# poke1024/vectorian

Measured on AMD Instinct MI355X. Metric: sentence-alignments/sec at d=300, |q|=10, |s|<=64; 1/2/4/8 GPU + %HBM roofline, higher is better.
Workload: dtype bf16

## Files before the change

### vectorian_amd/csrc/vk_common.hip.h

```cpp

#ifndef VK_COMMON_HIP_H
#define VK_COMMON_HIP_H

#include <hip/hip_runtime.h>
#include <stdint.h>
#include <stdlib.h>

#include "vk_device.h"

typedef __attribute__((ext_vector_type(8))) short bf16x8;
typedef __attribute__((ext_vector_type(4))) short bf16x4;
typedef __attribute__((ext_vector_type(4))) float f32x4;
typedef __attribute__((ext_vector_type(4))) int i32x4;
typedef __attribute__((ext_vector_type(2))) float f32x2;

#define VK_NEG_INF (-__builtin_inff())
#define VK_RUN 4
#ifdef VK_DBG_NOINLINE
#define VK_DP_INLINE __attribute__((noinline))
#else
#define VK_DP_INLINE __forceinline__
#endif


// ... 510 lines not shown

__device__ __forceinline__ const uint8_t *canon_row_ptr(const uint8_t *__restrict__ tile, int lane) { return tile + (lane & 15) * 16; }
__device__ __forceinline__ const uint8_t *canon_row_ptr_static(const uint8_t *__restrict__ etiles, int tile_bytes, int id) {
	return etiles + (int64_t)(id >> 4) * tile_bytes + (id & 15) * 16;
}

__device__ __forceinline__ float static_cell(float cosine, bool own, bool in_query, const vk_host::sim_ops &ops) {
	if (ops.n > 0 && in_query) cosine = vk_host::sim_ops_apply(cosine, ops);
	return own ? 1.0f : clip01(cosine);
}

__device__ __forceinline__ float static_table_cell(const float *__restrict__ table, int64_t table_stride, int id, int j) {
	return table[(int64_t)(j >> 4) * table_stride + (int64_t)id * 16 + (j & 15)];
}
__device__ __forceinline__ float static_cell(float cosine, bool own, bool in_query, const vk_host::sim_ops &ops, int sim_src,
	const float *__restrict__ table, int64_t table_stride, int id, int j) {
	if (sim_src != VK_SIMSRC_COSINE) return static_table_cell(table, table_stride, id, j);
	return static_cell(cosine, own, in_query, ops);
}

template <int NC>
__device__ __forceinline__ void static_sim_canon(const uint8_t *__restrict__ etiles, int tile_bytes, int id, const uint8_t *__restrict__ qtiles,
	int c0, int d, int prec, const int32_t *__restrict__ q_ids, int len_t, const vk_host::sim_ops &ops, int sim_src,
	const float *__restrict__ table, int64_t table_stride, float (&out)[NC]) {
	if (sim_src != VK_SIMSRC_COSINE) {
#pragma unroll
		for (int c = 0; c < NC; c++) out[c] = static_table_cell(table, table_stride, id, c0 + c);
		return;
	}
	sim_canon<NC>(etiles + (int64_t)(id >> 4) * tile_bytes, id & 15, qtiles + (int64_t)(c0 >> 4) * tile_bytes, c0 & 15, d, prec, out);
#pragma unroll
	for (int c = 0; c < NC; c++) out[c] = static_cell(out[c], q_ids && q_ids[c0 + c] == id, c0 + c < len_t, ops);
}

__device__ __forceinline__ float tag_weighted(float s, float w, int pos_s, int pos_t, float keep, float thr) {
	float wgt = w;
	if (pos_s != pos_t) wgt *= keep;
	const float sc = s * wgt;
	return sc <= thr ? 0.0f : sc;
}


__device__ __forceinline__ unsigned long long static_vocab_shared(int len_s, int len_t, const int32_t *__restrict__ tok,
	const int8_t *__restrict__ tag, const uint32_t *__restrict__ bits, const int32_t *qkey) {
	unsigned long long mask = 0;
	for (int u = 0; u < len_s; u++) {
		const int id = tok[u];
		if (!((bits[id >> 5] >> (id & 31)) & 1u)) continue;
		const int key = id * 256 + (tag[u] & 255);
		for (int j = 0; j < len_t; j++) mask |= qkey[j] == key ? 1ull << j : 0ull;
	}
	return (mask & (mask - 1)) ? mask : 0ull;
}

template <int NL, bool CANON = false, bool RESTORE = false>
__device__ __forceinline__ void static_vocab_fixup(float *__restrict__ S, int stride, int len_s, int len_t,
	const int32_t *__restrict__ tok, const int8_t *__restrict__ tag, const int8_t *__restrict__ pos,
	const float *__restrict__ table, int64_t table_stride, const uint32_t *__restrict__ bits, const int32_t *qkey,
	const float *tw, const int32_t *tpos, float keep, float thr, int l,
	const uint8_t *__restrict__ etiles = nullptr, int tile_bytes = 0, const uint8_t *__restrict__ qtiles = nullptr, int d = 0, int prec = 0,
	const int32_t *__restrict__ q_ids = nullptr, const vk_host::sim_ops &ops = vk_host::sim_ops{}, int sim_src = VK_SIMSRC_COSINE) {
	const unsigned long long mask = static_vocab_shared(len_s, len_t, tok, tag, bits, qkey);
	if (!mask) return;
	for (int u = l; u < len_s; u += NL) {
		const int id = tok[u];
		if (!((bits[id >> 5] >> (id & 31)) & 1u)) continue;
		const int key = id * 256 + (tag[u] & 255);
		int ft = -1;
		for (int j = len_t - 1; j >= 0; j--) ft = qkey[j] == key ? j : ft;
		if (ft < 0) continue;
		for (int j = 0; j < len_t; j++)
			if (((mask >> j) & 1ull) && qkey[j] > key) {
				float raw;
				if constexpr (CANON) {
					float v1[1];
					static_sim_canon<1>(etiles, tile_bytes, id, qtiles, j, d, prec, q_ids, len_t, ops, sim_src, table, table_stride, v1);
					raw = v1[0];
				} else raw = table[(int64_t)(j >> 4) * table_stride + (int64_t)id * 16 + (j & 15)];
				S[u * stride + j] = tag_weighted(raw, tw[RESTORE ? j : ft], pos[u], tpos[j], keep, thr);
			}
	}
}



struct DpArgs {
	int32_t locality;
	int32_t len_t;
	float gs, gt;
	float a_s, a_t;
	float open_s, open_t;
	const float *ws;
	const float *wt;
	const float *wt0;
	int32_t rwmd_symmetric, rwmd_normalize_bow, wmd_bound;
	float wrd_raw_total;
};

struct DecaySteps { float g1, g2, g4, g8; };

__device__ __forceinline__ DecaySteps decay_steps(float g, int v) {
	const float inf = __builtin_inff();
	return {v >= 1 ? g : inf, v >= 2 ? 2.0f * g : inf, v >= 4 ? 4.0f * g : inf, v >= 8 ? 8.0f * g : inf};
}

template <int LT>
__device__ __forceinline__ float decay_scan(float x, const DecaySteps &d) {
	x = fmaxf(x, dpp_zero<0x111>(x) - d.g1);
	if (LT > 2) x = fmaxf(x, dpp_zero<0x112>(x) - d.g2);
	if (LT > 4) x = fmaxf(x, dpp_zero<0x114>(x) - d.g4);
	if (LT > 8) x = fmaxf(x, dpp_zero<0x118>(x) - d.g8);
	return x;
}

template <int LT>
__device__ __forceinline__ float dp_linear(const float *__restrict__ S, int rowbase, int len, int maxlen, int v, const DpArgs &a) {
	const bool is_local = a.locality == VK_DEV_LOCAL;
	const bool is_global = a.locality == VK_DEV_GLOBAL;
	const float floor0 = is_local ? 0.0f : VK_NEG_INF;
	const float gsb = is_global ? a.gs : 0.0f;
	const float gs = a.gs, gt = a.gt;
	const bool last_col = v == a.len_t - 1;
	const float gt_v1 = gt * (float)(v + 1);

	const DecaySteps dt = decay_steps(gt, v);

	float h = is_global ? -gt_v1 : 0.0f;
	float best = 0.0f;
	for (int u = 1; u <= maxlen; u++) {
		const bool act = u <= len;
		const float s = S[(rowbase + (act ? u - 1 : 0)) * LT + v];
		const float bprev = -(gsb * (float)(u - 1));
		const float bcur = -(gsb * (float)u);
		const float diag = dpp_f<DPP_ROW_SHR1>(bprev, h);
		float c = fmaxf(diag + s, floor0);
		c = fmaxf(c, h - gs);
		float hn = decay_scan<LT>(c, dt);
		if (!is_local) hn = fmaxf(hn, bcur - gt_v1);
		h = act ? hn : h;
		if (is_local || last_col) best = fmaxf(best, h);
	}
	float m;
	if (is_local) m = v < a.len_t ? best : 0.0f;
	else if (is_global) m = last_col ? h : VK_NEG_INF;
	else m = v < a.len_t ? fmaxf(h, last_col ? best : 0.0f) : 0.0f;
	m = row_max_to_lane15(m);
	return (is_global) ? m : fmaxf(m, 0.0f);
}

template <int LT>
__device__ VK_DP_INLINE float dp_affine(const float *__restrict__ S, int rowbase, int len, int maxlen, int v, const DpArgs &a) {
	const bool is_local = a.locality == VK_DEV_LOCAL;
	const bool is_global = a.locality == VK_DEV_GLOBAL;
	const float floor0 = is_local ? 0.0f : VK_NEG_INF;
	const float bs = a.gs, bt = a.gt, open_s = a.open_s, open_t = a.open_t;
	const float a_s = a.a_s, a_t = a.a_t;
	const bool last_col = v == a.len_t - 1;

	float h = is_global ? -(a_t + bt * (float)(v + 1)) : 0.0f;
	float e = VK_NEG_INF;
	float best = 0.0f;
	const DecaySteps dt = decay_steps(bt, v);
	for (int u = 1; u <= maxlen; u++) {
		const bool act = u <= len;
		const float s = S[(rowbase + (act ? u - 1 : 0)) * LT + v];
		const float bprev = (is_global && u > 1) ? -(a_s + bs * (float)(u - 1)) : 0.0f;
		const float bcur = is_global ? -(a_s + bs * (float)u) : 0.0f;
		const float diag = dpp_f<DPP_ROW_SHR1>(bprev, h);
		const float en = fmaxf(h - open_s, e - bs);
		float c = fmaxf(fmaxf(diag + s, floor0), en);
		float f = VK_NEG_INF;
		float hc = c;
		if (a_t >= 0.0f) {
			f = decay_scan<LT>(dpp_f<DPP_ROW_SHR1>(bcur, c) - open_t, dt);
			hc = fmaxf(c, f);
		} else {
#pragma unroll
			for (int i = 0; i < LT; i++) {
				const float fl = fmaxf(dpp_f<DPP_ROW_SHR1>(bcur, hc) - open_t, dpp_f<DPP_ROW_SHR1>(VK_NEG_INF, f) - bt);
				f = fl;
				hc = fmaxf(c, f);
			}
		}
		if (act) { h = hc; e = en; }
		if (is_local || last_col) best = fmaxf(best, h);
	}
	float m;
	if (is_local) m = v < a.len_t ? best : 0.0f;
	else if (is_global) m = last_col ? h : VK_NEG_INF;
	else m = v < a.len_t ? fmaxf(h, last_col ? best : 0.0f) : 0.0f;
	m = row_max_to_lane15(m);
	return (is_global) ? m : fmaxf(m, 0.0f);
}

template <int LT>
__device__ __forceinline__ float dp_general(const float *__restrict__ S, float *__restrict__ Hh, int hstride,
	int rowbase, int len, int maxlen, int lane, const DpArgs &a) {

	const int v = lane & 15, sigma = lane >> 4;
	const bool is_local = a.locality == VK_DEV_LOCAL;
	const bool is_global = a.locality == VK_DEV_GLOBAL;
	const float floor0 = is_local ? 0.0f : VK_NEG_INF;
	const bool last_col = v == a.len_t - 1;
	float *hist = Hh + sigma * hstride * 16 + v;

	float wtl[LT];
#pragma unroll
	for (int p = 0; p < LT; p++) wtl[p] = (p <= v) ? a.wt[v + 1 - p] : __builtin_inff();

	float h = is_global ? -a.wt0[v + 1] : 0.0f;
	hist[0] = h;
	float best = 0.0f;
	for (int u = 1; u <= maxlen; u++) {
		const bool act = u <= len;
		const float s = S[(rowbase + (act ? u - 1 : 0)) * LT + v];
		const float bprev = is_global ? -a.ws[u - 1] : 0.0f;
		const float bcur = is_global ? -a.ws[u] : 0.0f;
		const float diag = dpp_f<DPP_ROW_SHR1>(bprev, h);
		float c = fmaxf(diag + s, floor0);
		for (int k = 1; k <= u; k++) c = fmaxf(c, hist[(u - k) * 16] - a.ws[k]);
		c = fmaxf(c, bcur - wtl[0]);
#pragma unroll
		for (int p = 1; p < LT; p++) {
			const float hp = __builtin_bit_cast(float,
				__builtin_amdgcn_ds_bpermute((sigma * 16 + p - 1) * 4, __builtin_bit_cast(int, c)));
			c = fmaxf(c, hp - wtl[p]);
		}
		if (act) { h = c; hist[u * 16] = c; }
		if (is_local || last_col) best = fmaxf(best, h);
	}
	float m;
	if (is_local) m = v < a.len_t ? best : 0.0f;
	else if (is_global) m = last_col ? h : VK_NEG_INF;
	else m = v < a.len_t ? fmaxf(h, last_col ? best : 0.0f) : 0.0f;
	m = row_max_to_lane15(m);
	return (is_global) ? m : fmaxf(m, 0.0f);
}

template <int LT, int MAXLEN, bool FRESH = true>
__device__ __forceinline__ float dp_general_reg(const float *__restrict__ S, int rowbase, int len, int maxlen, int v,
	const DpArgs &a, const float (&wsr)[MAXLEN + 1], const float (&wtr)[LT]) {

	int loc = a.locality, vsel = v;
	if constexpr (FRESH) {
		asm volatile("" : "+v"(loc));
		asm volatile("" : "+v"(vsel));
		loc = __builtin_amdgcn_readfirstlane(loc);
	}
	const bool is_local = loc == VK_DEV_LOCAL;
	const bool is_global = loc == VK_DEV_GLOBAL;
	const float floor0 = is_local ? 0.0f : VK_NEG_INF;
	const bool last_col = v == a.len_t - 1;
	const float wt_border = a.wt[v + 1];
	const float wt_border0 = a.wt0[v + 1];

	float wtv[16];
#pragma unroll
	for (int k = 1; k < LT; k++) wtv[k] = vsel >= k ? wtr[k] : __builtin_inff();

	float hreg[MAXLEN + 1];
	float h = is_global ? -wt_border0 : 0.0f;
	hreg[0] = h;
	float best = 0.0f;
#pragma unroll
	for (int u = 1; u <= MAXLEN; u++) {
		if (u <= maxlen) {
			const bool act = u <= len;
			const float s = S[(rowbase + (act ? u - 1 : 0)) * LT + v];
			const float bprev = is_global ? -wsr[u - 1] : 0.0f;
			const float bcur = is_global ? -wsr[u] : 0.0f;
			const float diag = dpp_f<DPP_ROW_SHR1>(bprev, hreg[u - 1]);
			float c = fmaxf(diag + s, floor0);
#pragma unroll
			for (int k = 1; k <= u; k++) c = fmaxf(c, hreg[u - k] - wsr[k]);
			float hc = fmaxf(c, bcur - wt_border);
			if (LT > 1) hc = fmaxf(hc, dpp_zero<0x111>(c) - wtv[1]);
			if (LT > 2) hc = fmaxf(hc, dpp_zero<0x112>(c) - wtv[2]);
			if (LT > 3) hc = fmaxf(hc, dpp_zero<0x113>(c) - wtv[3]);
			if (LT > 4) hc = fmaxf(hc, dpp_zero<0x114>(c) - wtv[4]);
			if (LT > 5) hc = fmaxf(hc, dpp_zero<0x115>(c) - wtv[5]);
			if (LT > 6) hc = fmaxf(hc, dpp_zero<0x116>(c) - wtv[6]);
			if (LT > 7) hc = fmaxf(hc, dpp_zero<0x117>(c) - wtv[7]);
			if (LT > 8) hc = fmaxf(hc, dpp_zero<0x118>(c) - wtv[8]);
			if (LT > 9) hc = fmaxf(hc, dpp_zero<0x119>(c) - wtv[9]);
			if (LT > 10) hc = fmaxf(hc, dpp_zero<0x11a>(c) - wtv[10]);
			if (LT > 11) hc = fmaxf(hc, dpp_zero<0x11b>(c) - wtv[11]);
			if (LT > 12) hc = fmaxf(hc, dpp_zero<0x11c>(c) - wtv[12]);
			if (LT > 13) hc = fmaxf(hc, dpp_zero<0x11d>(c) - wtv[13]);
			if (LT > 14) hc = fmaxf(hc, dpp_zero<0x11e>(c) - wtv[14]);
			if (LT > 15) hc = fmaxf(hc, dpp_zero<0x11f>(c) - wtv[15]);
			hreg[u] = hc;
			h = act ? hc : h;
			if (is_local || last_col) best = fmaxf(best, h);
		}
	}
	float m;
	if (is_local) m = v < a.len_t ? best : 0.0f;
	else if (is_global) m = last_col ? h : VK_NEG_INF;
	else m = v < a.len_t ? fmaxf(h, last_col ? best : 0.0f) : 0.0f;
	m = row_max_to_lane15(m);
	return (is_global) ? m : fmaxf(m, 0.0f);
}

template <int LT, int MAXLEN, int KT, bool FRESH = true>
__device__ __forceinline__ float dp_general_tail_reg(const float *__restrict__ S, int rowbase, int len, int maxlen, int v,
	const DpArgs &a, const float (&wsr)[KT + 2], const float (&wtr)[LT]) {
	static_assert(KT >= 1 && KT < MAXLEN, "the tail begins inside the table");
	int loc = a.locality, vsel = v;
	if constexpr (FRESH) {
		asm volatile("" : "+v"(loc));
		asm volatile("" : "+v"(vsel));
		loc = __builtin_amdgcn_readfirstlane(loc);
	}
	const bool is_local = loc == VK_DEV_LOCAL;
	const bool is_global = loc == VK_DEV_GLOBAL;
	const float floor0 = is_local ? 0.0f : VK_NEG_INF;
	const bool last_col = v == a.len_t - 1;
	const float wt_border = a.wt[v + 1];
	const float wt_border0 = a.wt0[v + 1];
	const float c_tail = wsr[KT + 1];

	float wtv[16];
#pragma unroll
	for (int k = 1; k < LT; k++) wtv[k] = vsel >= k ? wtr[k] : __builtin_inff();

	float hreg[MAXLEN + 1];
	float h = is_global ? -wt_border0 : 0.0f;
	hreg[0] = h;
	float R = h;
	float best = 0.0f;
#pragma unroll
	for (int u = 1; u <= MAXLEN; u++) {
		if (u <= maxlen) {
			const bool act = u <= len;
			const float s = S[(rowbase + (act ? u - 1 : 0)) * LT + v];
			const float bprev = is_global ? -wsr[u - 1 <= KT ? u - 1 : KT + 1] : 0.0f;
			const float bcur = is_global ? -wsr[u <= KT ? u : KT + 1] : 0.0f;
			const float diag = dpp_f<DPP_ROW_SHR1>(bprev, hreg[u - 1]);
			float c = fmaxf(diag + s, floor0);
#pragma unroll
			for (int k = 1; k <= (u < KT ? u : KT); k++) c = fmaxf(c, hreg[u - k] - wsr[k]);
			if (u > KT) {
				if (u > KT + 1) R = fmaxf(R, hreg[u - KT - 1]);
				c = fmaxf(c, R - c_tail);
			}
			float hc = fmaxf(c, bcur - wt_border);
			if (LT > 1) hc = fmaxf(hc, dpp_zero<0x111>(c) - wtv[1]);
			if (LT > 2) hc = fmaxf(hc, dpp_zero<0x112>(c) - wtv[2]);
			if (LT > 3) hc = fmaxf(hc, dpp_zero<0x113>(c) - wtv[3]);
			if (LT > 4) hc = fmaxf(hc, dpp_zero<0x114>(c) - wtv[4]);
			if (LT > 5) hc = fmaxf(hc, dpp_zero<0x115>(c) - wtv[5]);
			if (LT > 6) hc = fmaxf(hc, dpp_zero<0x116>(c) - wtv[6]);
			if (LT > 7) hc = fmaxf(hc, dpp_zero<0x117>(c) - wtv[7]);
			if (LT > 8) hc = fmaxf(hc, dpp_zero<0x118>(c) - wtv[8]);
			if (LT > 9) hc = fmaxf(hc, dpp_zero<0x119>(c) - wtv[9]);
			if (LT > 10) hc = fmaxf(hc, dpp_zero<0x11a>(c) - wtv[10]);
			if (LT > 11) hc = fmaxf(hc, dpp_zero<0x11b>(c) - wtv[11]);
			if (LT > 12) hc = fmaxf(hc, dpp_zero<0x11c>(c) - wtv[12]);
			if (LT > 13) hc = fmaxf(hc, dpp_zero<0x11d>(c) - wtv[13]);
			if (LT > 14) hc = fmaxf(hc, dpp_zero<0x11e>(c) - wtv[14]);
			if (LT > 15) hc = fmaxf(hc, dpp_zero<0x11f>(c) - wtv[15]);
			hreg[u] = hc;
			h = act ? hc : h;
			if (is_local || last_col) best = fmaxf(best, h);
		}
	}
	float m;
	if (is_local) m = v < a.len_t ? best : 0.0f;
	else if (is_global) m = last_col ? h : VK_NEG_INF;
	else m = v < a.len_t ? fmaxf(h, last_col ? best : 0.0f) : 0.0f;
	m = row_max_to_lane15(m);
	return (is_global) ? m : fmaxf(m, 0.0f);
}

template <int LT>
__device__ __forceinline__ float rwmd_rows(const float *__restrict__ S, int rowbase, int len, int maxlen, int v, const DpArgs &a) {
	const int len_t = a.len_t;
	const bool nbow = a.rwmd_normalize_bow != 0;
	const float w_t = nbow ? 1.0f / (float)len_t : 1.0f;
	const float w_s = nbow ? 1.0f / (float)(len > 0 ? len : 1) : 1.0f;
	const bool col_ok = v < len_t;
	float colmin = 3.402823466e+38F;
	float acc1 = 0.0f;
	for (int u = 1; u <= maxlen; u++) {
		const bool act = u <= len;
		const float s = S[(rowbase + (act ? u - 1 : 0)) * LT + v];
		const float dist = fmaxf(1.0f - s, 0.0f);
		if (act) colmin = fminf(colmin, dist);
		float m = col_ok ? dist : 3.402823466e+38F;
		m = fminf(m, dpp_f<DPP_ROW_SHR1>(m, m));
		m = fminf(m, dpp_f<DPP_ROW_SHR2>(m, m));
		m = fminf(m, dpp_f<DPP_ROW_SHR4>(m, m));
		m = fminf(m, dpp_f<DPP_ROW_SHR8>(m, m));
		if (act) acc1 += w_s * m;
	}
	const float x = col_ok ? w_t * colmin : 0.0f;
	float sum = x;
#pragma unroll
	for (int i = 1; i < LT; i++) {
		const float t = dpp_f<DPP_ROW_SHR1>(0.0f, sum);
		if (v == i) sum = t + x;
	}
	float acc0 = (v == len_t - 1) ? sum : VK_NEG_INF;
	acc0 = row_max_to_lane15(acc0);
	if (!nbow) {
		acc0 = acc0 / (float)len_t;
		acc1 = acc1 / (float)(len > 0 ? len : 1);
	}
	if (a.wmd_bound) {
		float lb;
		if (a.wmd_bound == 1) lb = fmaxf(acc0, acc1);
		else lb = len_t <= len ? acc0 : acc1;
		return fminf(1.0f - lb + 3e-5f, 1.0f);
	}
	float cost = 0.0f;
	if (a.rwmd_symmetric) {
		if (acc0 > cost) cost = acc0;
		if (acc1 > cost) cost = acc1;
	} else {
		cost = acc0;
	}
	const float max_cost = nbow ? 1.0f : (float)len_t;
	return (max_cost - cost) / max_cost;
}

template <int LT>
__device__ __forceinline__ float rwmd_fill_rows(const float *__restrict__ S, const float *__restrict__ smass, int rowbase, int len, int maxlen,
	int lane, const DpArgs &a, float q_mass) {
	const int v = lane & 15, sigma = lane >> 4;
	const int len_t = a.len_t;
	const bool nbow = a.rwmd_normalize_bow != 0;
	const bool col_ok = v < len_t;
	const float cap_s = nbow ? 1.0f / (float)(len > 0 ? len : 1) : 1.0f;
	const float INF = __builtin_inff();

	float rem = col_ok ? q_mass : 0.0f, cost0 = 0.0f, last_d = -1.0f;
	int last_i = -1;
	bool fin = !(rem > 0.0f) || len < 1;
	for (int round = 0; round < maxlen && __any(!fin); round++) {
		float bd = INF;
		int bi = -1;
		for (int u = 1; u <= maxlen; u++) {
			const bool act = u <= len;
			const float dist = fmaxf(1.0f - S[(rowbase + (act ? u - 1 : 0)) * LT + v], 0.0f);
			const bool later = dist > last_d || (dist == last_d && u - 1 > last_i);
			if (act && later && dist < bd) { bd = dist; bi = u - 1; }
		}
		if (!fin) {
			const float cap = (smass && bi >= 0) ? smass[bi] : cap_s;
			if (bi < 0) fin = true;
			else if (rem <= cap) { cost0 += rem * bd; fin = true; }
			else { rem -= cap; cost0 += cap * bd; last_d = bd; last_i = bi; }
		}
	}
	if (rem > 0.0f) cost0 += rem;
	float sum = cost0;
#pragma unroll
	for (int i = 1; i < LT; i++) {
		const float t = dpp_f<DPP_ROW_SHR1>(0.0f, sum);
		if (v == i) sum = t + cost0;
	}
	float acc0 = (v == len_t - 1) ? sum : VK_NEG_INF;
	acc0 = row_max_to_lane15(acc0);

	float acc1 = 0.0f;
	if (a.rwmd_symmetric) {
		for (int u = 1; u <= maxlen; u++) {
			const bool act = u <= len;
			const float dist = fmaxf(1.0f - S[(rowbase + (act ? u - 1 : 0)) * LT + v], 0.0f);
			float r1 = act ? (smass ? smass[u - 1] : cap_s) : 0.0f;
			float cost = 0.0f;
			bool used = !col_ok, done = !(r1 > 0.0f);
			for (int r = 0; r < LT && __any(!done); r++) {
				int key = used ? 0x7fffffff : ((__builtin_bit_cast(int, dist) & ~15) | v);
				key = min(key, __builtin_amdgcn_update_dpp(key, key, 0xB1, 0xf, 0xf, false));
				key = min(key, __builtin_amdgcn_update_dpp(key, key, 0x4E, 0xf, 0xf, false));
				key = min(key, __builtin_amdgcn_update_dpp(key, key, 0x141, 0xf, 0xf, false));
				key = min(key, __builtin_amdgcn_update_dpp(key, key, 0x140, 0xf, 0xf, false));
				const int tl = key & 15;
				const float td = __builtin_bit_cast(float, __builtin_amdgcn_ds_bpermute((sigma * 16 + tl) * 4, __builtin_bit_cast(int, dist)));
				const float tc = __builtin_bit_cast(float, __builtin_amdgcn_ds_bpermute((sigma * 16 + tl) * 4, __builtin_bit_cast(int, q_mass)));
				if (!done) {
					if (key == 0x7fffffff) done = true;
					else if (r1 <= tc) { cost += r1 * td; done = true; }
					else { r1 -= tc; cost += tc * td; }
				}
				if (v == tl) used = true;
			}
			if (r1 > 0.0f) cost += r1;
			acc1 += cost;
		}
	}
	if (!nbow) {
		acc0 = acc0 / (float)len_t;
		acc1 = acc1 / (float)(len > 0 ? len : 1);
	}
	float cost = acc0;
	if (a.rwmd_symmetric) { cost = 0.0f; if (acc0 > cost) cost = acc0; if (acc1 > cost) cost = acc1; }
	const float max_cost = nbow ? 1.0f : (float)len_t;
	return (max_cost - cost) / max_cost;
}

template <int LT>
__device__ __forceinline__ float wrd_bound_rows(const float *__restrict__ S, int rowbase, int len, int maxlen, int v,
	const DpArgs &a, const float *__restrict__ mag, const int32_t *__restrict__ ids, float q_mass) {
	const int len_t = a.len_t;
	const bool col_ok = v < len_t;
	float sum_s = 0.0f;
	float lb1n = 0.0f;
	const float BIG = 3.402823466e+38F;
	float d1 = BIG, d2 = BIG, d3 = BIG, d4 = BIG, c1 = 0.0f, c2 = 0.0f, c3 = 0.0f, c4 = 0.0f;
	const int lane_row = (int)(threadIdx.x & 48);
	for (int base = 0; base < maxlen; base += 64) {
		float mreg[4];
#pragma unroll
		for (int c = 0; c < 4; c++) {
			const int u0 = base + c * 16 + v;
			float mg = 0.0f;
			if (u0 < len) mg = mag ? (ids ? mag[ids[u0]] : mag[u0]) : 1.0f;
			mreg[c] = mg;
		}
#pragma unroll
		for (int c = 0; c < 4; c++) {
			const int u_end = maxlen < base + c * 16 + 16 ? maxlen : base + c * 16 + 16;
			for (int u = base + c * 16 + 1; u <= u_end; u++) {
				const bool act = u <= len;
				const float s = S[(rowbase + (act ? u - 1 : 0)) * LT + v];
				const float dist = fmaxf(1.0f - s, 0.0f);
				int mi = __builtin_bit_cast(int, col_ok ? dist : BIG);
				mi = min(mi, __builtin_amdgcn_update_dpp(mi, mi, DPP_ROW_SHR1, 0xf, 0xf, false));
				mi = min(mi, __builtin_amdgcn_update_dpp(mi, mi, DPP_ROW_SHR2, 0xf, 0xf, false));
				mi = min(mi, __builtin_amdgcn_update_dpp(mi, mi, DPP_ROW_SHR4, 0xf, 0xf, false));
				mi = min(mi, __builtin_amdgcn_update_dpp(mi, mi, DPP_ROW_SHR8, 0xf, 0xf, false));
				const float m = __builtin_bit_cast(float, mi);
				const float mg = __builtin_bit_cast(float, __builtin_amdgcn_ds_bpermute((lane_row | ((u - 1) & 15)) * 4, __builtin_bit_cast(int, mreg[c])));
				sum_s += mg;
				lb1n += mg * m;
				float nd = act ? dist : BIG, nc = mg;
				bool sw;
				sw = nd < d4; d4 = sw ? nd : d4; c4 = sw ? nc : c4;
				sw = d4 < d3; nd = d3; nc = c3; d3 = sw ? d4 : d3; c3 = sw ? c4 : c3; d4 = sw ? nd : d4; c4 = sw ? nc : c4;
				sw = d3 < d2; nd = d2; nc = c2; d2 = sw ? d3 : d2; c2 = sw ? c3 : c2; d3 = sw ? nd : d3; c3 = sw ? nc : c3;
				sw = d2 < d1; nd = d1; nc = c1; d1 = sw ? d2 : d1; c1 = sw ? c2 : c1; d2 = sw ? nd : d2; c2 = sw ? nc : c2;
			}
		}
	}
	const float lb1 = lb1n / sum_s * (1.0f - 2e-6f);
	const float scale = a.wrd_raw_total > 0.0f ? 1.0f : 1.0f / sum_s;
	float rem = col_ok ? q_mass : 0.0f, x = 0.0f, last = 0.0f;
	{
		float amt;
		if (d1 < BIG) { amt = fminf(rem, c1 * scale * (1.0f + 2e-6f)); x += amt * d1; rem -= amt; last = d1; }
		if (d2 < BIG) { amt = fminf(rem, c2 * scale * (1.0f + 2e-6f)); x += amt * d2; rem -= amt; last = d2; }
		if (d3 < BIG) { amt = fminf(rem, c3 * scale * (1.0f + 2e-6f)); x += amt * d3; rem -= amt; last = d3; }
		if (d4 < BIG) { amt = fminf(rem, c4 * scale * (1.0f + 2e-6f)); x += amt * d4; rem -= amt; last = d4; }
		x += fmaxf(rem, 0.0f) * last;
	}
	x += dpp_f<DPP_ROW_SHR1>(0.0f, x);
	x += dpp_f<DPP_ROW_SHR2>(0.0f, x);
	x += dpp_f<DPP_ROW_SHR4>(0.0f, x);
	x += dpp_f<DPP_ROW_SHR8>(0.0f, x);
	float lb;
	if (a.wrd_raw_total > 0.0f) {
		const float sum_t = a.wrd_raw_total;
		lb = (sum_t <= sum_s ? x / sum_t : lb1) * (1.0f - 2e-6f);
		if (!(sum_s > 0.0f)) lb = 0.0f;
	} else lb = fmaxf(x, lb1);
	return fminf(1.0f - lb + 3e-5f, 1.0f);
}

#endif
```

### vectorian_amd/csrc/vk_corpus.cpp

```cpp

#include "vk_internal.h"

std::string &vk_error_slot() {
	static thread_local std::string err;
	return err;
}

std::mutex &vk_ring_mutex() {
	static std::mutex mu;
	return mu;
}

void vk_devblock::release(void *p) {
	if (!p) return;
	{
		std::lock_guard<std::mutex> g(mu);
		ptrs.erase(std::remove(ptrs.begin(), ptrs.end(), p), ptrs.end());
	}
	(void)hipFree(p);
}

vk_devblock::~vk_devblock() {
	(void)hipSetDevice(device);
	for (void *p : ptrs) if (p) (void)hipFree(p);
// ... 314 lines not shown
	c->h_start = std::make_shared<std::vector<int32_t>>(st32);
	c->h_end = std::make_shared<std::vector<int32_t>>(en32);
	c->n_entries = n_entries;
	c->d_wide_order.reset(); c->d_xlong_order.reset(); c->d_apart_order.reset();
	c->n_wide_order = c->n_xlong_order = c->n_apart_order = -1;
	c->lq.order.reset(); c->lq.n_order = -1;
	c->n_long_groups = (int)long_groups.size();
	c->max_len = max_len;
	c->max_short_len = max_short;
	c->max_long_len = max_long;
	c->h_xlong = xlong_entries;
	c->h_apart = apart_entries;
	c->contiguous = contiguous;
	c->overlapping = false;
	for (int64_t s = 1; s < n_sentences && !c->overlapping; s++) c->overlapping = start[s] < end[s - 1] && end[s] > start[s];
	c->uniform_len = 0;
	if (n_sentences > 0 && contiguous) {
		const int64_t l0 = end[0] - start[0];
		bool uni = l0 > 0;
		for (int64_t s = 1; s < n_sentences && uni; s++) uni = (end[s] - start[s]) == l0;
		if (uni) c->uniform_len = (int)l0;
	}
	int mt = 1, mtok = 1, lt = 1, ltok = 1;
	size_t li = 0;
	for (int64_t g = 0; g * 4 < n_entries; g++) {
		const int64_t a = st32[(size_t)(g * 4)], b = en32[(size_t)std::min<int64_t>(g * 4 + 3, n_entries - 1)];
		const int tiles = (int)(((b + 15) >> 4) - (a >> 4));
		if (li < apart_groups.size() && apart_groups[li] == g) {
			li++;
			if (b - a <= VK_MAX_SENT_LEN) {
				lt = std::max(lt, tiles);
				ltok = std::max(ltok, (int)(b - a));
			}
		} else {
			mt = std::max(mt, tiles);
			mtok = std::max(mtok, (int)(b - a));
		}
	}
	int pt = 1, spt = 1;
	li = 0;
	for (int64_t g = 0; g * 2 < n_entries; g++) {
		const int64_t a = st32[(size_t)(g * 2)], b = en32[(size_t)std::min<int64_t>(g * 2 + 1, n_entries - 1)];
		const int tiles = (int)(((b + 15) >> 4) - (a >> 4));
		pt = std::max(pt, tiles);
		while (li < apart_groups.size() && apart_groups[li] < g / 2) li++;
		if (!(li < apart_groups.size() && apart_groups[li] == g / 2)) spt = std::max(spt, tiles);
	}
	c->max_pair_tiles = pt;
	c->max_short_pair_tiles = spt;
	c->max_group_tiles = mt;
	c->max_group_tokens = mtok;
	c->long_group_tiles = lt;
	c->long_group_tokens = ltok;
	c->have_sent = true;
	return VK_OK;
}

int vk_corpus_set_sentences(vk_corpus_t *c, const int64_t *sent_off, int64_t n_sentences) {
	if (!c || !sent_off) return fail(VK_ERR_INVALID, "null argument");
	if (c->finalized) return fail(VK_ERR_STATE, "corpus already finalized");
	if (n_sentences != c->desc.n_sentences) return fail(VK_ERR_INVALID, "sentence count differs from n_sentences");
	if (sent_off[0] != 0) return fail(VK_ERR_INVALID, "sentence spans must start at token 0 (document.h:151-168)");
	if (sent_off[n_sentences] != c->desc.n_tokens) return fail(VK_ERR_INVALID, "sentence spans must cover exactly n_tokens");
	for (int64_t s = 0; s < n_sentences; s++)
		if (sent_off[s + 1] < sent_off[s]) return fail(VK_ERR_INVALID, "sentence offsets must be non-decreasing");
	return set_slices_impl(c, sent_off, sent_off + 1, n_sentences, true);
}

int vk_corpus_set_slices(vk_corpus_t *c, const int64_t *start, const int64_t *end, int64_t n_sentences) {
	if (!c || !start || !end) return fail(VK_ERR_INVALID, "null argument");
	if (c->finalized) return fail(VK_ERR_STATE, "corpus already finalized");
	if (n_sentences != c->desc.n_sentences) return fail(VK_ERR_INVALID, "slice count differs from n_sentences");
	return set_slices_impl(c, start, end, n_sentences, false);
}

static void build_shadow(vk_corpus *c) {
	const int mode = bound_pass_mode();
	if (mode < 0 || (mode == 0 && c->desc.n_sentences < kBoundPassMinSentences)) return;
	if (c->max_len > VK_FAST_SENT_LEN || c->n_entries < 1) return;
	const vk_host::shadow_format f = vk_host::shadow_format_of(c->desc.d, c->nk32, c->tail, c->prec, c->desc.layout, bound_bits_wanted(mode));
	if (f.bits == 0) return;
	const size_t bytes = (size_t)c->n_tiles * f.tile_bytes();
	uint8_t *sh = nullptr;
	if (c->d_counter.reserve(4, &c->device_bytes) || alloc_shared(c, &sh, bytes)) { (void)hipGetLastError(); return; }
	uint32_t stats[4] = {0, 0, 1, 0};
	const bool ran = vk_launch_shadow(c->d_tiles, c->n_tiles, c->rows_total, c->tile_bytes, &f, sh, c->d_counter, c->stream) == hipSuccess
		&& hipMemcpyAsync(stats, c->d_counter, 16, hipMemcpyDeviceToHost, c->stream) == hipSuccess && hipStreamSynchronize(c->stream) == hipSuccess;
	if (!ran || stats[2] != 0) {
		(void)hipGetLastError();
		c->shared->release(sh);
		c->device_bytes -= (int64_t)bytes;
		return;
	}
	c->shadow = sh; c->shadow_format = f;
	memcpy(&c->shadow_n, &stats[0], 4);
	memcpy(&c->shadow_x, &stats[1], 4);
}

int vk_corpus_finalize(vk_corpus_t *c) {
	if (!c) return fail(VK_ERR_INVALID, "null argument");
	if (c->rows_appended != c->rows_total) return fail(VK_ERR_STATE, "not all vectors were appended");
	if (!c->have_sent) return fail(VK_ERR_STATE, "sentence spans were not set");
	if (c->desc.layout == VK_LAYOUT_STATIC && !c->have_ids) return fail(VK_ERR_STATE, "token ids were not set");
	VK_HIP(hipSetDevice(c->device));
	c->d_stage.reset();
	VK_HIP(hipStreamSynchronize(c->stream));
	build_shadow(c);
	c->finalized = true;
	return VK_OK;
}

int vk_corpus_set_sim_ops(vk_corpus_t *c, const int32_t *kinds, const float *args, int32_t n_ops) {
	if (!c || (n_ops > 0 && (!kinds || !args))) return fail(VK_ERR_INVALID, "null argument");
	int bad = -1;
	if (vk_host::sim_ops_check(kinds, args, n_ops, &bad) != VK_OK) {
		if (bad < 0) return fail(VK_ERR_INVALID, "n_ops must be 0 .. VK_MAX_SIM_OPS (8), got " + std::to_string(n_ops));
		return fail(VK_ERR_INVALID, "similarity operator " + std::to_string(bad) + ": unknown kind or an argument that is not finite");
	}
	if (n_ops > 0 && c->desc.layout != VK_LAYOUT_STATIC)
		return fail(VK_ERR_UNSUPPORTED, "similarity operators run over VK_LAYOUT_STATIC only: this corpus is VK_LAYOUT_CONTEXTUAL");
	vk_host::sim_ops ops{};
	ops.n = n_ops;
	for (int i = 0; i < n_ops; i++) { ops.kind[i] = kinds[i]; ops.arg[i] = args[i]; }
	c->sim_ops = ops;
	return VK_OK;
}

int vk_corpus_set_sim_source(vk_corpus_t *c, int32_t kind, float arg) {
	if (!c) return fail(VK_ERR_INVALID, "null argument");
	if (vk_host::sim_src_check(kind, arg) != VK_OK)
		return fail(VK_ERR_INVALID, kind == VK_SIMSRC_PNORM ? "VK_SIMSRC_PNORM: p must be finite and > 0" : "unknown similarity source " + std::to_string(kind));
	if (kind == VK_SIMSRC_COSINE) { c->sim_src = vk_host::sim_src{VK_SIMSRC_COSINE, 0.0f}; return VK_OK; }
	if (c->desc.layout != VK_LAYOUT_STATIC)
		return fail(VK_ERR_UNSUPPORTED, "similarity sources beside the cosine run over VK_LAYOUT_STATIC only: this corpus is VK_LAYOUT_CONTEXTUAL");
	if (c->desc.d > vk_host::kSimSrcMaxD)
		return fail(VK_ERR_UNSUPPORTED, "similarity sources beside the cosine: rows of at most " + std::to_string(vk_host::kSimSrcMaxD) + " features (the table kernel keeps a query tile in LDS)");
	if (!c->raw_rows) {
		if (c->rows_appended > 0 || c->finalized || c->is_view || c->shares_vectors)
			return fail(VK_ERR_STATE, "a similarity source beside the cosine is set before the first vk_corpus_append_vectors: it reads the unmodified rows, and they are gone");
		VK_HIP(hipSetDevice(c->device));
		const int raw_tile_bytes = (c->desc.d + 15) / 16 * 1024;
		const size_t bytes = (size_t)c->n_tiles * (size_t)raw_tile_bytes;
		auto rows = std::make_shared<vk_devbuf<uint8_t>>();
		if (int rc = rows->reserve(bytes, nullptr)) return rc;
		VK_HIP(hipMemsetAsync(*rows, 0, bytes, c->stream));
		VK_HIP(hipStreamSynchronize(c->stream));
		c->raw_rows = rows; c->raw_tile_bytes = raw_tile_bytes;
		c->device_bytes += (int64_t)bytes;
	}
	c->sim_src = vk_host::sim_src{kind, kind == VK_SIMSRC_PNORM ? arg : 0.0f};
	return VK_OK;
}

int vk_corpus_filter(vk_corpus_t *src, uint64_t pos_mask, uint64_t tag_mask, vk_corpus_t **out) {
	if (!src || !out) return fail(VK_ERR_INVALID, "null argument");
	if (!src->finalized) return fail(VK_ERR_STATE, "corpus not finalized");
	if (pos_mask && !src->d_pos) return fail(VK_ERR_STATE, "pos filter needs vk_corpus_set_token_pos");
	if (tag_mask && !src->d_tag) return fail(VK_ERR_STATE, "tag filter needs vk_corpus_set_token_tags");
	VK_HIP(hipSetDevice(src->device));
	hipStream_t st = src->stream;
	const int64_t n = src->desc.n_tokens, ne = src->n_entries, ns = src->desc.n_sentences;
	const bool is_static = src->desc.layout == VK_LAYOUT_STATIC;

	int32_t *keep = nullptr, *new_index = nullptr, *src_of = nullptr, *fs = nullptr, *fe = nullptr;
	void *temp = nullptr;
	vk_corpus *c = nullptr;
	int rc = VK_OK;
	auto body = [&]() -> int {
		VK_HIP(hipMalloc((void **)&keep, ((size_t)n + 1) * 4));
		VK_HIP(hipMalloc((void **)&new_index, ((size_t)n + 1) * 4));
		VK_HIP(hipMalloc((void **)&src_of, ((size_t)n + 1) * 4));
		VK_HIP(hipMalloc((void **)&fs, ((size_t)ne + 1) * 4));
		VK_HIP(hipMalloc((void **)&fe, ((size_t)ne + 1) * 4));
		size_t temp_bytes = 0;
		VK_HIP(vk_launch_filter_scan(nullptr, nullptr, 0, 0, n, keep, new_index, nullptr, &temp_bytes, st));
		VK_HIP(hipMalloc(&temp, temp_bytes ? temp_bytes : 16));
		VK_HIP(vk_launch_filter_scan(src->d_pos, src->d_tag, pos_mask, tag_mask, n, keep, new_index, temp, &temp_bytes, st));
		VK_HIP(vk_launch_filter_maps(keep, new_index, n, src_of, src->d_sent_start, src->d_sent_end, ne, fs, fe, st));
		int32_t n_kept32 = 0;
		std::vector<int32_t> hs((size_t)ne), he((size_t)ne);
		VK_HIP(hipMemcpyAsync(&n_kept32, new_index + n, 4, hipMemcpyDeviceToHost, st));
		if (ne > 0) {
			VK_HIP(hipMemcpyAsync(hs.data(), fs, (size_t)ne * 4, hipMemcpyDeviceToHost, st));
			VK_HIP(hipMemcpyAsync(he.data(), fe, (size_t)ne * 4, hipMemcpyDeviceToHost, st));
		}
		VK_HIP(hipStreamSynchronize(st));
		const int64_t n_kept = n_kept32;

		std::vector<int64_t> start((size_t)ns), end((size_t)ns);
		for (int64_t e = 0; e < ne; e++) {
			const int64_t sent = src->entry_sent.empty() ? e : src->entry_sent[(size_t)e];
			if (sent >= 0 && sent < ns) { start[(size_t)sent] = hs[(size_t)e]; end[(size_t)sent] = he[(size_t)e]; }
		}

		vk_corpus_desc desc = src->desc;
		desc.n_tokens = n_kept;
		if (is_static) {
			c = new vk_corpus();
			c->desc = desc; c->device = src->device;
			c->shared = std::make_shared<vk_devblock>();
			c->shared->device = src->device;
			c->d_pad = src->d_pad; c->nk32 = src->nk32; c->tail = src->tail; c->tile_bytes = src->tile_bytes; c->prec = src->prec;
			c->rows_total = c->rows_appended = src->rows_total; c->n_tiles = src->n_tiles;
			c->d_tiles = src->d_tiles; c->d_mag = src->d_mag; c->shares_vectors = true;
			c->vectors_of = src->shares_vectors ? src->vectors_of : src->shared;
			c->sim_ops = src->sim_ops;
			c->sim_src = src->sim_src; c->raw_rows = src->raw_rows; c->raw_tile_bytes = src->raw_tile_bytes;
			if (hipStreamCreateWithFlags(&c->stream, hipStreamNonBlocking) != hipSuccess) return fail(VK_ERR_HIP, "hipStreamCreate failed");
			for (auto &e : c->ev) if (hipEventCreate(&e) != hipSuccess) return fail(VK_ERR_HIP, "hipEventCreate failed");
			int r;
			if ((r = alloc_shared(c, &c->d_tok_id, (size_t)n_kept + 64))) return r;
			if ((r = reserve_query_workspaces(c))) return r;
			VK_HIP(hipMemsetAsync(c->d_tok_id, 0, ((size_t)n_kept + 64) * 4, st));
			VK_HIP(vk_launch_filter_gather(src->d_tok_id, c->d_tok_id, 4, src_of, n_kept, st));
			c->have_ids = true;
		} else {
			int r = vk_corpus_create(&desc, &c);
			if (r) return r;
			VK_HIP(hipStreamSynchronize(c->stream));
			VK_HIP(vk_launch_filter_rows(src->d_tiles, c->d_tiles, src_of, n_kept, src->tile_bytes, st));
			if (src->d_mag && c->d_mag) VK_HIP(vk_launch_filter_gather(src->d_mag, c->d_mag, 4, src_of, n_kept, st));
			c->rows_appended = c->rows_total;
		}
		for (int which = 0; which < 2; which++) {
			int8_t *from = which ? src->d_tag : src->d_pos;
			int8_t **to = which ? &c->d_tag : &c->d_pos;
			if (!from) continue;
			int r = alloc_shared(c, to, (size_t)n_kept + 64);
			if (r) return r;
			VK_HIP(hipMemsetAsync(*to, 0, (size_t)n_kept + 64, st));
			VK_HIP(vk_launch_filter_gather(from, *to, 1, src_of, n_kept, st));
		}
		VK_HIP(hipStreamSynchronize(st));
		if (is_static) {
			c->h_tok = std::make_shared<std::vector<int32_t>>((size_t)n_kept);
			if (n_kept > 0) VK_HIP(hipMemcpy(c->h_tok->data(), c->d_tok_id, (size_t)n_kept * 4, hipMemcpyDeviceToHost));
		}
		if (c->d_tag) {
			c->h_tag = std::make_shared<std::vector<int8_t>>((size_t)n_kept);
			if (n_kept > 0) VK_HIP(hipMemcpy(c->h_tag->data(), c->d_tag, (size_t)n_kept, hipMemcpyDeviceToHost));
		}
		int r = set_slices_impl(c, start.data(), end.data(), ns, src->contiguous);
		if (r) return r;
		c->finalized = true;
		return VK_OK;
	};
	rc = body();
	for (void *p : {(void *)keep, (void *)new_index, (void *)src_of, (void *)fs, (void *)fe, temp}) if (p) (void)hipFree(p);
	if (rc) { if (c) vk_corpus_free(c); return rc; }
	*out = c;
	return VK_OK;
}

int vk_last_scores(vk_corpus_t *c, float *scores, int64_t n) {
	if (!c || !scores) return fail(VK_ERR_INVALID, "null argument");
	if (!c->have_scores) return fail(VK_ERR_STATE, "no query has run on this corpus");
	if (n != c->desc.n_sentences) return fail(VK_ERR_INVALID, "n differs from n_sentences");
	VK_HIP(hipSetDevice(c->device));
	if (c->bp.pruned) {
		VK_HIP(vk_launch_score(&c->bp.full, c->bp.full_grid, c->bp.full_smem, c->stream));
		VK_HIP(hipStreamSynchronize(c->stream));
		c->bp.pruned = false;
	}
	if (c->entry_sent.empty()) {
		VK_HIP(hipMemcpy(scores, c->d_scores, (size_t)n * 4, hipMemcpyDeviceToHost));
		return VK_OK;
	}
	std::vector<float> rows((size_t)c->n_entries);
	VK_HIP(hipMemcpy(rows.data(), c->d_scores, rows.size() * 4, hipMemcpyDeviceToHost));
	for (int64_t e = 0; e < c->n_entries; e++)
		if (c->entry_sent[(size_t)e] >= 0) scores[c->entry_sent[(size_t)e]] = rows[(size_t)e];
	return VK_OK;
}

int vk_bound_pass_state(vk_corpus_t *c, float *bounds, int64_t n, int64_t *counters) {
	if (!c || !counters) return fail(VK_ERR_INVALID, "null argument");
	const int64_t v[7] = {c->bp.ran, c->bp.round1, c->bp.round2, c->bp.fell_back, c->bp.queries, c->bp.fallbacks, c->bp.survivors};
	memcpy(counters, v, sizeof v);
	if (!bounds) return VK_OK;
	if (!c->bp.ran) return fail(VK_ERR_STATE, "the last query ran no bound pass");
	if (n != c->desc.n_sentences) return fail(VK_ERR_INVALID, "n differs from n_sentences");
	VK_HIP(hipSetDevice(c->device));
	std::vector<float> rows((size_t)c->n_entries);
	VK_HIP(hipMemcpy(rows.data(), c->d_ub, rows.size() * 4, hipMemcpyDeviceToHost));
	for (int64_t e = 0; e < c->n_entries; e++) {
		const int64_t sent = c->entry_sent.empty() ? e : (int64_t)c->entry_sent[(size_t)e];
		if (sent >= 0) bounds[sent] = rows[(size_t)e];
	}
	return VK_OK;
}

int vk_bound_pass_bits(vk_corpus_t *c, int64_t *bits) {
	if (!c || !bits) return fail(VK_ERR_INVALID, "null argument");
	*bits = c->shadow ? c->shadow_format.bits : 0;
	return VK_OK;
}

int vk_bound_pass_tail(vk_corpus_t *c, int32_t *k) {
	if (!c || !k) return fail(VK_ERR_INVALID, "null argument");
	*k = c->bp.ran ? (int32_t)c->bp.tail_k : 0;
	return VK_OK;
}

int vk_bound_pass_shadow(vk_corpus_t *c, int64_t *format, float *nx, int64_t tile0, int64_t n, uint8_t *out) {
	if (!c || !format || !nx) return fail(VK_ERR_INVALID, "null argument");
	const vk_host::shadow_format &sf = c->shadow_format;
	const int64_t f[5] = {sf.bits, sf.steps, sf.live, sf.tile_bytes(), c->n_tiles};
	memset(format, 0, sizeof f);
	nx[0] = nx[1] = 0.0f;
	if (!c->shadow) return out ? fail(VK_ERR_STATE, "the corpus has no shadow") : VK_OK;
	memcpy(format, f, sizeof f);
	nx[0] = c->shadow_n; nx[1] = c->shadow_x;
	if (!out) return VK_OK;
	if (tile0 < 0 || n < 0 || tile0 > c->n_tiles || n > c->n_tiles - tile0) return fail(VK_ERR_INVALID, "tiles out of range");
	VK_HIP(hipSetDevice(c->device));
	VK_HIP(hipStreamSynchronize(c->stream));
	if (n > 0) VK_HIP(hipMemcpy(out, c->shadow + tile0 * sf.tile_bytes(), (size_t)n * sf.tile_bytes(), hipMemcpyDeviceToHost));
	return VK_OK;
}

int vk_batch_state(vk_corpus_t *c, int64_t *state) {
	if (!c || !state) return fail(VK_ERR_INVALID, "null argument");
	memcpy(state, c->batch_state, sizeof c->batch_state);
	return VK_OK;
}

int vk_query_route(vk_corpus_t *c, int64_t *state) {
	if (!c || !state) return fail(VK_ERR_INVALID, "null argument");
	memcpy(state, c->query_route, sizeof c->query_route);
	return VK_OK;
}

int vk_i8_tile_probe(const int8_t *q, const int8_t *x, int32_t *out) {
	if (!q || !x || !out) return fail(VK_ERR_INVALID, "null argument");
	vk_devbuf<uint8_t> buf;
	if (int rc = buf.reserve(4096, nullptr)) return rc;
	uint8_t *d = buf;
	VK_HIP(hipMemcpy(d, q, 1024, hipMemcpyHostToDevice));
	VK_HIP(hipMemcpy(d + 1024, x, 1024, hipMemcpyHostToDevice));
	VK_HIP(vk_launch_i8_probe((const int8_t *)d, (const int8_t *)d + 1024, (int32_t *)(d + 2048), nullptr));
	VK_HIP(hipDeviceSynchronize());
	VK_HIP(hipMemcpy(out, d + 2048, 1024, hipMemcpyDeviceToHost));
	return VK_OK;
}

int vk_i8_bound_tile_probe(const int8_t *q, const int8_t *x, int32_t nk64, int32_t live, int32_t *out) {
	if (!q || !x || !out) return fail(VK_ERR_INVALID, "null argument");
	if ((nk64 != 5 && nk64 != 12) || live < 1 || live > 4) return fail(VK_ERR_INVALID, "nk64 is 5 or 12, live 1 .. 4");
	const size_t tb = (size_t)nk64 * 1024;
	vk_devbuf<uint8_t> buf;
	if (int rc = buf.reserve(2 * tb + 1024, nullptr)) return rc;
	uint8_t *d = buf;
	std::vector<uint8_t> pk(2 * tb);
	for (int side = 0; side < 2; side++)
		for (int i = 0; i < 16; i++)
			vk_host::i8_put_row(pk.data() + side * tb, i, (const uint8_t *)(side ? x : q) + (size_t)i * nk64 * 64, nk64 * 64);
	VK_HIP(hipMemcpy(d, pk.data(), 2 * tb, hipMemcpyHostToDevice));
	VK_HIP(vk_launch_i8_bound_probe(d, d + tb, nk64, live, (int32_t *)(d + 2 * tb), nullptr));
	VK_HIP(hipDeviceSynchronize());
	VK_HIP(hipMemcpy(out, d + 2 * tb, 1024, hipMemcpyDeviceToHost));
	return VK_OK;
}

int vk_fp6_bound_tile_probe(const uint8_t *q, const uint8_t *x, int32_t live6, float *out) {
	if (!q || !x || !out) return fail(VK_ERR_INVALID, "null argument");
	if (live6 < 1 || live6 > 4) return fail(VK_ERR_INVALID, "live6 is 1 .. 4");
	const size_t xoff = VK_DEV_FP6_QTILE_BYTES, ooff = xoff + 5120;
	vk_devbuf<uint8_t> buf;
	if (int rc = buf.reserve(ooff + 1024, nullptr)) return rc;
	uint8_t *d = buf;
	std::vector<uint8_t> pk(ooff, 0);
	for (int i = 0; i < 16; i++) {
		vk_host::fp6_put_row(pk.data(), 4, i, q + (size_t)i * 384, 384);
		vk_host::fp6_put_row(pk.data() + xoff, live6, i, x + (size_t)i * 384, 256 + 32 * live6);
	}
	static_assert(VK_DEV_FP6_QTILE_BYTES % 128 == 0 && VK_DEV_FP6_TILE_BYTES(4) <= 5120, "the probe's buffer");
	VK_HIP(hipMemcpy(d, pk.data(), ooff, hipMemcpyHostToDevice));
	VK_HIP(vk_launch_fp6_bound_probe(d, d + xoff, live6, (float *)(d + ooff), nullptr));
	VK_HIP(hipDeviceSynchronize());
	VK_HIP(hipMemcpy(out, d + ooff, 1024, hipMemcpyDeviceToHost));
	return VK_OK;
}

int vk_fp6c_bound_tile_probe(const uint8_t *q, const uint8_t *x, int32_t d, int32_t fill, float *out) {
	if (!q || !x || !out) return fail(VK_ERR_INVALID, "null argument");
	if (d < 0 || d > 304) return fail(VK_ERR_INVALID, "d is 0 .. 304");
	const size_t xoff = VK_DEV_FP6_QTILE_BYTES, ooff = xoff + 5120;
	vk_devbuf<uint8_t> buf;
	if (int rc = buf.reserve(ooff + 1024, nullptr)) return rc;
	uint8_t *dv = buf;
	std::vector<uint8_t> pk(ooff, 0);
	for (int i = 0; i < 16; i++) {
		vk_host::fp6_put_row(pk.data(), 4, i, q + (size_t)i * 384, 384);
		vk_host::fp6c_put_row(pk.data() + xoff, i, x + (size_t)i * 384, d);
	}
	memset(pk.data() + xoff + VK_DEV_FP6C_TILE_BYTES, fill, 5120 - VK_DEV_FP6C_TILE_BYTES);
	VK_HIP(hipMemcpy(dv, pk.data(), ooff, hipMemcpyHostToDevice));
	VK_HIP(vk_launch_fp6c_bound_probe(dv, dv + xoff, (float *)(dv + ooff), nullptr));
	VK_HIP(hipDeviceSynchronize());
	VK_HIP(hipMemcpy(out, dv + ooff, 1024, hipMemcpyDeviceToHost));
	return VK_OK;
}

int vk_last_timings(const vk_corpus_t *c, vk_timings *t) {
	if (!c || !t) return fail(VK_ERR_INVALID, "null argument");
	*t = c->last;
	return VK_OK;
}

}
```

### vectorian_amd/csrc/vk_device.h

```cpp
#ifndef VK_DEVICE_H
#define VK_DEVICE_H

#include <hip/hip_runtime.h>
#include <stdint.h>

#include "vk_sim_ops_host.h"
#include "vk_sim_src_host.h"

#define VK_DEV_LOCAL 0
#define VK_DEV_GLOBAL 1
#define VK_DEV_SEMIGLOBAL 2

#define VK_DEV_LAYOUT_CONTEXTUAL 0
#define VK_DEV_LAYOUT_STATIC 1

#define VK_DEV_MAX_SENT_LEN 64
#define VK_DEV_MAX_LONG_LEN 512
#define VK_DEV_MAX_QUERY_LEN 16
#define VK_DEV_MAX_WIDE_QUERY_LEN 64
#define VK_DEV_BOUND_CONST_BYTES 256
#define VK_DEV_FP6_STEPS 3
#define VK_DEV_FP6_STEP_BYTES 1536
#define VK_DEV_FP6_QTILE_BYTES (VK_DEV_FP6_STEPS * VK_DEV_FP6_STEP_BYTES)
#define VK_DEV_FP6_TILE_BYTES(live6) ((VK_DEV_FP6_STEPS - 1) * VK_DEV_FP6_STEP_BYTES + 384 * (live6) + 128)
// ... 60 lines not shown

struct VkRwmdBatchParams {
	const uint8_t *tiles;
	int64_t n_tiles;
	int32_t tile_bytes, nk, half;
	const uint8_t *qtiles;
	int32_t n_qtiles, qpt;
	int32_t dense;
	int32_t late_mask;
	const int32_t *q_len;
	const float *q_inv_len;
	const float *q_param;
	int32_t n_queries;
	int32_t n_sent;
	int32_t tiles_per_sent;
	int32_t symmetric, nbow;
	const float *boost;
	float *scores;
	const int32_t *sent_len;
	const int32_t *sent_id;
	int64_t score_stride;
	const int32_t *tok_id;
	const int32_t *sent_start, *sent_end;
	const uint16_t *table;
	int64_t table_row;
	int32_t zero_row;
};

struct VkWrdParams {
	const uint8_t *tiles;
	const int32_t *tok_id;
	const float *table;
	int64_t table_stride;
	const int32_t *sent_start;
	const int32_t *sent_end;
	int32_t layout;
	int32_t nk32, tail, tile_bytes;
	int32_t prec;
	const uint8_t *qtile;
	int32_t nq;
	int32_t len_t;
	const float *mag;
	float qmass[VK_DEV_MAX_WIDE_QUERY_LEN];
	int32_t mass_mode;
	int32_t raw_masses;
	const int8_t *pos_s;
	float tw[VK_DEV_MAX_WIDE_QUERY_LEN];
	int32_t tpos[VK_DEV_MAX_WIDE_QUERY_LEN];
	float tw_keep, tw_threshold;
	float ref_total;
	const float *boost;
	const uint64_t *keys;
	float *raw_out;
	float *val_out;
	float *plan_out;
	float *rows_out;
	int32_t rows_len;
	const int8_t *tag_s;
	const uint32_t *qid_bits;
	int32_t qkey[VK_DEV_MAX_WIDE_QUERY_LEN];
	const int32_t *cand_query;
	int64_t qtile_stride;
	int32_t q_ids_stride;
	const int32_t *cand_len_t;
	const int32_t *group_list;
	int32_t n_list;
	int32_t n_entries;
	float *scores, *raw;
	float wrd_raw_total;
	int32_t wmd_bound;
	int32_t d;
	const int32_t *q_ids;
	uint8_t *scratch;
	int64_t scratch_stride;
	int32_t n_cand;
	vk_host::sim_ops sim_ops;
	int32_t sim_src;
};

struct VkFlowParams {
	const uint8_t *tiles;
	const int32_t *tok_id;
	const float *table;
	const int32_t *sent_start;
	const int32_t *sent_end;
	int32_t layout;
	int32_t nk32, tail, tile_bytes;
	int32_t prec;
	const uint8_t *qtile;
	int32_t len_t;
	int32_t locality;
	int32_t gap_mode;
	int32_t max_len;
	float gs, gt, a_s, a_t, open_s, open_t;
	const float *ws;
	const float *wt;
	const int8_t *pos_s;
	float tw[VK_DEV_MAX_QUERY_LEN];
	int32_t tpos[VK_DEV_MAX_QUERY_LEN];
	float tw_keep, tw_threshold;
	int32_t d;
	const int32_t *q_ids;
	const uint64_t *keys;
	float *raw_out;
	int16_t *mapping;
	float *edge_sim;
	vk_host::sim_ops sim_ops;
	int32_t sim_src;
};

struct VkScoreBatchParams {
	const uint8_t *tiles;
	const int32_t *sent_start;
	const int32_t *sent_end;
	int32_t n_sent;
	int32_t nk32, tail, tile_bytes;
	const uint8_t *qtiles;
	int32_t n_queries;
	int32_t n_strips;
	int32_t len_t[4];
	int32_t locality;
	int32_t gap_mode;
	int32_t rwmd_symmetric, rwmd_normalize_bow;
	float gs, gt, a_s, a_t, open_s, open_t;
	const float *ws;
	const float *wt;
	const float *wt0;
	const float *boost;
	float *scores;
	float *raw;
	int32_t lds_floats_per_wave;
	int32_t s_rows_per_wave;
	int32_t h_rows;
};

struct VkWideParams {
	const uint8_t *tiles;
	const int32_t *tok_id;
	const float *table;
	int64_t table_stride;
	const int32_t *sent_start;
	const int32_t *sent_end;
	int32_t n_sent;
	int32_t layout;
	int32_t nk32, tail, tile_bytes;
	int32_t prec;
	const uint8_t *qtile;
	int32_t nq, len_t;
	int32_t locality;
	int32_t gap_mode;
	int32_t max_len;
	int32_t rwmd_symmetric, rwmd_normalize_bow;
	float gs, gt, a_s, a_t, open_s, open_t;
	const float *ws;
	const float *wt;
	const float *wt0;
	const int8_t *pos_s;
	const int8_t *tag_s;
	const uint32_t *qid_bits;
	int32_t slices_overlap;
	int32_t qkey[VK_DEV_MAX_WIDE_QUERY_LEN];
	float tw[VK_DEV_MAX_WIDE_QUERY_LEN];
	int32_t tpos[VK_DEV_MAX_WIDE_QUERY_LEN];
	float tw_keep, tw_threshold;
	float ref_total;
	const float *mag;
	float qmass[VK_DEV_MAX_WIDE_QUERY_LEN];
	float wrd_raw_total;
	int32_t wmd_bound;
	const float *boost;
	float *scores;
	float *raw;
	int32_t d;
	const int32_t *q_ids;
	const uint64_t *keys;
	float *raw_out;
	int16_t *mapping;
	float *edge_sim;
	uint8_t *scratch;
	int64_t scratch_stride;
	const int32_t *order;
	int32_t n_order;
	const float *dp_rows;
	int32_t dp_rows_len;
	int32_t h_ring;
	int32_t ws_tail;
	vk_host::sim_ops sim_ops;
	int32_t sim_src;
};

struct VkLongqParams {
	const uint8_t *tiles;
	const int32_t *tok_id;
	const float *table;
	int64_t table_stride;
	const int32_t *sent_start;
	const int32_t *sent_end;
	int32_t n_sent;
	int32_t layout;
	int32_t nk32, tail, tile_bytes;
	int32_t prec;
	const uint8_t *qtile;
	int32_t nq, len_t;
	int32_t s_stride;
	int32_t locality;
	int32_t gap_mode;
	float gs, gt, a_s, a_t, open_s, open_t;
	const float *ws;
	const float *wt;
	int32_t wt_tail;
	const int8_t *pos_s;
	const float *tw;
	const int32_t *tpos;
	float tw_keep, tw_threshold;
	float ref_total;
	const float *boost;
	float *scores;
	float *raw;
	int32_t d;
	const int32_t *q_ids;
	const uint64_t *keys;
	int32_t n_keys;
	float *raw_out;
	int16_t *mapping;
	float *edge_sim;
	int32_t out_stride;
	uint8_t *scratch;
	int64_t scratch_stride;
	const int32_t *order;
	int32_t n_order;
	int64_t dm_off, su_off;
	vk_host::sim_ops sim_ops;
	int32_t sim_src;
};

struct VkSimSrcArgs {
	vk_host::sim_src src;
	const uint8_t *raw_tiles;
	int32_t raw_tile_bytes;
	int32_t d;
	const float *q_rows;
	const float *q_abs_sums;
};

#ifdef __cplusplus
namespace vk_host { struct shadow_format; }

extern "C" {
#endif
size_t vk_longq_scratch_bytes(int32_t len_t, int32_t gap_mode, int32_t flow, int32_t tagged);
size_t vk_longq_lds_bytes(int32_t len_t, int32_t max_len, int32_t flow);
int32_t vk_longq_blocks(int32_t len_t, int32_t max_len, int64_t n_sent, int32_t hm_in_lds);
int32_t vk_longq_hm_in_lds(int32_t len_t, int32_t max_len);
int32_t vk_longq_stride(int32_t max_len);
hipError_t vk_launch_longq(const VkLongqParams *p, int32_t flow_k, hipStream_t stream);
hipError_t vk_launch_longq_blocks(const VkLongqParams *p, int32_t max_len, int32_t flow_k, hipStream_t stream);
int32_t vk_longq_blocks_grid(int32_t len_t, int32_t max_len, int32_t gap_mode, int32_t flow_k, int64_t n_items);
hipError_t vk_launch_wide(const VkWideParams *p, int32_t flow_k, hipStream_t stream);
hipError_t vk_launch_doc(const VkWideParams *p, int32_t flow_k, hipStream_t stream);
size_t vk_doc_scratch_bytes(int32_t max_len, int32_t gap_mode);
hipError_t vk_launch_docw(const VkWideParams *p, int32_t flow_k, hipStream_t stream);
size_t vk_docw_scratch_bytes(int32_t max_len, int32_t nq);
hipError_t vk_launch_docg(const VkWideParams *p, int32_t flow_k, hipStream_t stream);
size_t vk_docg_scratch_bytes(int32_t max_len);
hipError_t vk_launch_submatch_bound(const float *raw, const float *boost, int64_t n, float total, float w, float m_star,
	float *scores, hipStream_t stream);
hipError_t vk_launch_mark(const uint64_t *keys, int32_t n, float *scores, hipStream_t stream);
hipError_t vk_launch_select_ge(const float *scores, int64_t n, float theta, float floor_excl, uint64_t *keys_out,
	uint32_t *counter, uint32_t cap, hipStream_t stream);
size_t vk_wide_lds_demand(int32_t max_len, int32_t nq, int32_t gap_mode, int32_t tagged, int32_t flow);
size_t vk_wide_scratch_bytes(int32_t max_len, int32_t nq, int32_t gap_mode, int32_t flow, int32_t ring);
int32_t vk_wide_gs_blocks(int32_t max_len, int32_t nq, int32_t gap_mode, int32_t flow_k, int64_t n_sent, int32_t ring);
int32_t vk_wide_ring_rows(int32_t nq, int32_t gap_mode, int32_t ws_tail);
hipError_t vk_launch_shadow(const uint8_t *tiles, int64_t n_tiles, int64_t rows_total, int32_t tile_bytes, const vk_host::shadow_format *f,
	uint8_t *shadow, uint32_t *stats, hipStream_t stream);
hipError_t vk_launch_i8_bound_probe(const uint8_t *qtile8, const uint8_t *tile8, int32_t nk64, int32_t live, int32_t *out, hipStream_t stream);
hipError_t vk_launch_i8_probe(const int8_t *q, const int8_t *x, int32_t *out, hipStream_t stream);
hipError_t vk_launch_fp6_bound_probe(const uint8_t *qtile6, const uint8_t *tile6, int32_t live6, float *out, hipStream_t stream);
hipError_t vk_launch_fp6c_bound_probe(const uint8_t *qtile6, const uint8_t *tile6c, float *out, hipStream_t stream);
hipError_t vk_launch_select_ge_key(const float *scores, int64_t n, const uint64_t *theta_key, float floor_excl, uint64_t *keys_out,
	uint32_t *counter, uint32_t cap, hipStream_t stream);
hipError_t vk_launch_rekey(const uint64_t *keys, int32_t n, const float *scores, float floor_excl, uint64_t *out, hipStream_t stream);
hipError_t vk_launch_topk_unsorted(const uint64_t *in, int32_t n, int32_t k, uint64_t *out, hipStream_t stream);
hipError_t vk_launch_key_groups(const uint64_t *keys, int32_t n, int32_t *groups, hipStream_t stream);
hipError_t vk_launch_pack(const void *in, int32_t dtype_bf16, int64_t n_rows, int32_t d, int32_t d_pad, int64_t row0,
	uint8_t *tiles, float *mag_out, int32_t normalize, int32_t prec, hipStream_t stream);
size_t vk_score32_lds_bytes(int32_t nk32, int32_t tail, int32_t max_pair_tiles, int32_t len_t, int32_t gap_mode, int32_t waves);
int32_t vk_score32_waves(int32_t nk32, int32_t tail, int32_t max_pair_tiles, int32_t len_t, int32_t gap_mode);
hipError_t vk_launch_score32(const VkWideParams *p, int32_t max_pair_tiles, hipStream_t stream);
hipError_t vk_launch_filter_scan(const int8_t *pos, const int8_t *tag, uint64_t pos_mask, uint64_t tag_mask, int64_t n,
	int32_t *keep, int32_t *new_index, void *temp, size_t *temp_bytes, hipStream_t stream);
hipError_t vk_launch_filter_maps(const int32_t *keep, const int32_t *new_index, int64_t n, int32_t *src_of,
	const int32_t *start, const int32_t *end, int64_t n_entries, int32_t *out_start, int32_t *out_end, hipStream_t stream);
hipError_t vk_launch_filter_rows(const uint8_t *src, uint8_t *dst, const int32_t *src_of, int64_t n_kept, int32_t tile_bytes,
	hipStream_t stream);
hipError_t vk_launch_filter_gather(const void *src, void *dst, int32_t elem_bytes, const int32_t *src_of, int64_t n_kept,
	hipStream_t stream);
hipError_t vk_launch_table(const uint8_t *etiles, const uint8_t *qtile, int32_t n_tiles, int32_t nk32, int32_t tail,
	int32_t tile_bytes, float *table, const int32_t *q_ids, int32_t len_t, int32_t V, int32_t prec, const vk_host::sim_ops *ops,
	const VkSimSrcArgs *src, hipStream_t stream);
hipError_t vk_launch_score(const VkScoreParams *p, int32_t grid, size_t smem_bytes, hipStream_t stream);
int32_t vk_score_m8t_tail_k(void);
int32_t vk_score_m7t_tail_k(void);
hipError_t vk_launch_span(const VkScoreParams *p, hipStream_t stream);
hipError_t vk_launch_score_batch(const VkScoreBatchParams *p, int32_t lt, size_t smem, hipStream_t stream);
hipError_t vk_launch_topk_scores(const float *scores, int64_t n, float min_score, int32_t k, uint64_t *out,
	int32_t *n_blocks_out, hipStream_t stream);
hipError_t vk_launch_topk_keys(const uint64_t *in, int64_t n, int32_t k, uint64_t *out, int32_t *n_blocks_out,
	hipStream_t stream);
hipError_t vk_launch_topk_wave(const float *scores, const uint64_t *keys_in, int64_t n, float min_score, int32_t k,
	int64_t per_wave, uint64_t *out, int64_t *n_waves_out, hipStream_t stream);
hipError_t vk_launch_flow(const VkFlowParams *p, int32_t k, hipStream_t stream);
hipError_t vk_launch_sort_all(const float *scores, int64_t n, float min_score, uint64_t *keys_a, uint64_t *keys_b, void *temp, size_t *temp_bytes,
	uint64_t **sorted_out, hipStream_t stream);
hipError_t vk_launch_rwmd_batch(const VkRwmdBatchParams *p, hipStream_t stream);
hipError_t vk_launch_rwmd_batch32(const VkRwmdBatchParams *p, hipStream_t stream);
hipError_t vk_launch_batch_pack(const uint8_t *src_tiles, uint8_t *dst_tiles, const int32_t *ids, const int32_t *sent_start, const int32_t *sent_end,
	int64_t n, int32_t tps, int32_t tile_bytes, hipStream_t stream);
int vk_rwmd_batch_supported(int32_t nk, int32_t half);
hipError_t vk_launch_table_batch(const uint8_t *etiles, int64_t n_vtiles, int32_t tile_bytes, int32_t nk16, const uint8_t *qtiles, int32_t n_qtiles,
	uint16_t *table, int32_t V, const vk_host::sim_ops *ops, const uint32_t *live, hipStream_t stream);
hipError_t vk_launch_table_batch_fix(uint16_t *table, const int64_t *offsets, int32_t n, hipStream_t stream);
hipError_t vk_launch_rwmd_static32(const VkRwmdBatchParams *p, int32_t w64, hipStream_t stream);
hipError_t vk_launch_topk_wave_batch(const float *scores, const uint64_t *keys_in, int64_t n, float min_score, int32_t k,
	int64_t per_wave, int32_t n_queries, int64_t in_stride, int64_t out_stride, uint64_t *out, int64_t *n_waves_out, hipStream_t stream);
hipError_t vk_launch_wrd_exact(const VkWrdParams *p, int32_t n_cand, float *scores_to_mark, hipStream_t stream);
hipError_t vk_launch_rows(const VkWrdParams *p, int32_t n_cand, hipStream_t stream);
hipError_t vk_launch_canon_rows(const VkWrdParams *p, int32_t n_cand, int32_t max_tiles, hipStream_t stream);
hipError_t vk_launch_wrd_exact_long(const VkWrdParams *p, int32_t n_cand, hipStream_t stream);
int vk_wrd_long_blocks(void);
size_t vk_wrd_long_scratch_bytes(void);
hipError_t vk_launch_long_rwmd_fill(const VkWideParams *p, const int32_t *group_list, int32_t n_list, int32_t n_entries, hipStream_t stream);
hipError_t vk_launch_long_bound(const VkWrdParams *p, hipStream_t stream);
#ifdef __cplusplus
}
#endif

#endif
```

### vectorian_amd/csrc/vk_internal.h

```cpp
#ifndef VK_INTERNAL_H
#define VK_INTERNAL_H

#include "../../include/vectorian_hip.h"
#include "vk_device.h"
#include "vk_devbuf.h"
#include "vk_guard.h"
#include "vk_result_host.h"
#include "vk_bound_host.h"
#include "vk_route_host.h"
#include "vk_sim_ops_host.h"

#include <algorithm>
#include <atomic>
#include <cmath>
#include <cstdio>
#include <cstring>
#include <memory>
#include <mutex>
#include <string>
#include <vector>

std::string &vk_error_slot();

namespace {

int fail(int code, const std::string &msg) {
	vk_error_slot() = msg;
	return code;
}

#define VK_HIP(call) \
	do { \
		hipError_t e_ = (call); \
		if (e_ != hipSuccess) { \
			char buf_[512]; \
			snprintf(buf_, sizeof buf_, "%s failed: %s (%s:%d)", #call, hipGetErrorString(e_), __FILE__, __LINE__); \
			return fail(VK_ERR_HIP, buf_); \
		} \
	} while (0)

uint16_t f32_to_bf16(float x) {
	uint32_t u;
	memcpy(&u, &x, 4);
	if ((u & 0x7fffffffu) > 0x7f800000u) return (uint16_t)((u >> 16) | 0x0040u);
	u += 0x7fffu + ((u >> 16) & 1u);
	return (uint16_t)(u >> 16);
}

float bf16_to_f32(uint16_t b) {
	uint32_t u = ((uint32_t)b) << 16;
	float f;
	memcpy(&f, &u, 4);
	return f;
}

using vk_host::gap_cost;

constexpr int kTopkChunk = 2048;
constexpr int kGapTable = 640;
constexpr int64_t kStageBytes = 64ll << 20;
constexpr int64_t kBoundPassMinSentences = 1000000;
constexpr int64_t kBoundRound2Floor = 1024;
inline int bound_pass_mode() {
	const char *e = getenv("VK_BOUND_PASS");
	return !e ? 0 : !strcmp(e, "off") ? -1 : !strcmp(e, "force") ? 1 : 0;
}
inline int bound_bits_wanted(int mode) {
	const char *e = getenv("VK_BOUND_BITS");
	if (e && !strcmp(e, "6c")) return vk_host::bits6_compact;
	if (e && !strcmp(e, "6")) return 6;
	if (e && !strcmp(e, "8")) return 8;
	return mode > 0 ? 8 : vk_host::bits6_compact;
}
inline bool bound_tail_wanted(int mode) { return vk_host::bound_tail_choice(getenv("VK_BOUND_TAIL"), mode); }

}

struct vk_devblock {
	int device = 0;
	std::mutex mu;
	std::vector<void *> ptrs;
	void add(void *p) { std::lock_guard<std::mutex> g(mu); ptrs.push_back(p); }
	void release(void *p);
	~vk_devblock();
};

std::mutex &vk_ring_mutex();

struct vk_corpus_shape {
	vk_corpus_desc desc{};
	int device = 0;
	int d_pad = 0, nk32 = 0, tail = 0, tile_bytes = 0;
	int prec = 0;
	int64_t rows_total = 0, rows_appended = 0, n_tiles = 0;
	uint8_t *d_tiles = nullptr;
	float *d_mag = nullptr;
	int32_t *d_tok_id = nullptr;
	int8_t *d_pos = nullptr;
	int8_t *d_tag = nullptr;
	int32_t *d_sent_start = nullptr, *d_sent_end = nullptr;
	std::shared_ptr<std::vector<int32_t>> h_start, h_end, h_tok;
	std::shared_ptr<std::vector<int8_t>> h_tag;
	bool contiguous = false;
	bool overlapping = false;
	bool have_ids = false, have_sent = false;
	int max_len = 0, max_group_tiles = 0, max_group_tokens = 0;
	int max_pair_tiles = 0;
	int max_short_pair_tiles = 0;
	int64_t n_entries = 0;
	std::vector<int32_t> entry_sent;
	int32_t *d_long_groups = nullptr;
	int n_long_groups = 0, max_short_len = 0, long_group_tiles = 0, long_group_tokens = 0;
	int max_long_len = 0;
	std::shared_ptr<std::vector<int32_t>> h_apart;
	std::shared_ptr<std::vector<int32_t>> h_xlong;
	int uniform_len = 0;
	bool shares_vectors = false;
	std::shared_ptr<vk_devblock> shared, vectors_of;
	const uint8_t *shadow = nullptr;
	vk_host::shadow_format shadow_format;
	float shadow_n = 0.0f, shadow_x = 0.0f;
	vk_host::sim_ops sim_ops{};
	vk_host::sim_src sim_src{};
	std::shared_ptr<vk_devbuf<uint8_t>> raw_rows;
	int raw_tile_bytes = 0;
};

enum vk_batch_state_index {
	VK_BS_ROUTE,
	VK_BS_QB_MAX, VK_BS_LT, VK_BS_GAP_MODE,
	VK_BS_STAT, VK_BS_STAT_UNIFORM32, VK_BS_UNIFORM16, VK_BS_B32, VK_BS_R32, VK_BS_GRAN,
	VK_BS_WIDE32, VK_BS_DENSE, VK_BS_QPT, VK_BS_N_QTILES, VK_BS_UNIFORM_LEN, VK_BS_LATE_MASK,
	VK_BS_COUNT
};

enum vk_query_route_index {
	VK_QR_PLAN, VK_QR_GAP_MODE, VK_QR_WIDE_GAP_MODE, VK_QR_SCORE32_GAP_MODE, VK_QR_WAVE_TILES,
	VK_QR_PASS_SHORT, VK_QR_PASS_MID, VK_QR_PASS_XLONG, VK_QR_LIST, VK_QR_RING_ROWS, VK_QR_FLOW, VK_QR_OSTRIDE, VK_QR_RAW, VK_QR_SPAN_SKIP_RAW,
	VK_QR_COUNT
};

struct vk_corpus : vk_corpus_shape {
	hipStream_t stream = nullptr;
	bool finalized = false;
	std::vector<int32_t> sent_entry;
	int64_t device_bytes = 0;
	vk_devbuf<uint8_t> d_bq; vk_devbuf<int32_t> d_bqlen; vk_devbuf<float> d_bscores; vk_devbuf<uint64_t> d_bkeys[2];
	vk_devbuf<float> d_braw;
	vk_devbuf<uint8_t> d_stage;
	vk_devbuf<uint8_t> d_qtile;
	vk_devbuf<float> d_ws, d_wt;
	vk_devbuf<int32_t> d_qids;
	vk_devbuf<float> d_table;
	vk_devbuf<float> d_qraw;
	vk_devbuf<float> d_scores, d_raw, d_boost;
	vk_devbuf<uint64_t> d_keys[2];
	vk_devbuf<float> d_out_raw, d_out_sim;
	vk_devbuf<int16_t> d_out_map;
	vk_devbuf<float> d_wrd_raw, d_wrd_val;
	vk_devbuf<uint32_t> d_counter;
	vk_devbuf<float> d_rows_out, d_plan_out;
	vk_devbuf<uint8_t> d_bqt; vk_devbuf<uint64_t> d_bcand; vk_devbuf<int32_t> d_bcandq; vk_devbuf<float> d_brows;
	vk_devbuf<float, true> h_brows;
	vk_devbuf<uint32_t> d_qbits;
	vk_devbuf<uint8_t> d_wrdl_scratch;
	vk_devbuf<uint8_t> d_wide_scratch;
	vk_devbuf<int32_t> d_apart_order; int32_t n_apart_order = -1;
	vk_devbuf<int32_t> d_xlong_order; int32_t n_xlong_order = -1;
	vk_devbuf<int32_t> d_wide_order; int32_t n_wide_order = -1;
	int rows_w = 0;
	struct batch_bucket { vk_devbuf<uint8_t> tiles; vk_devbuf<int32_t> len, id; int64_t n = 0; };
	batch_bucket bl[4];
	bool bl_built = false;
	int64_t bl_empty = 0;
	vk_devbuf<uint8_t> d_qtile8; vk_devbuf<float> d_ub; vk_devbuf<int32_t> d_bound_groups; vk_devbuf<uint64_t> d_bound_keys;
	struct bound_state {
		bool pruned = false;
		VkScoreParams full{}; int full_grid = 0; size_t full_smem = 0;
		int64_t ran = 0, round1 = 0, round2 = 0, fell_back = 0;
		int64_t tail_k = 0;
		int64_t queries = 0, fallbacks = 0, survivors = 0;
		vk_host::bound_backoff backoff;
	} bp;
	vk_devbuf<int32_t> d_sb_id[2]; int64_t sb_n[2] = {0, 0}; bool sb_built = false; int64_t sb_empty = 0;
	vk_devbuf<uint16_t> d_btable;
	vk_devbuf<int64_t> d_bfix;
	vk_devbuf<uint32_t> d_blive;
	vk_devbuf<int32_t> d_bqids;
	vk_devbuf<uint64_t> d_sort[2]; vk_devbuf<uint8_t> d_sort_temp;
	int64_t batch_state[VK_BS_COUNT] = {};
	int64_t query_route[VK_QR_COUNT] = {};
	hipEvent_t ev[7] = {nullptr, nullptr, nullptr, nullptr, nullptr, nullptr, nullptr};
	vk_timings last{};
	bool have_scores = false;
	bool is_view = false;
	struct longq_bufs {
		vk_devbuf<uint8_t> qt;
		vk_devbuf<float> fl;
		vk_devbuf<int32_t> il;
		vk_devbuf<float> table;
		vk_devbuf<uint8_t> scratch, fscratch;
		vk_devbuf<uint8_t> bscratch;
		vk_devbuf<int32_t> order; int32_t n_order = -1;
		vk_devbuf<float> raw, sim;
		vk_devbuf<int16_t> map;
	} lq;
	vk_corpus *peer = nullptr;
	std::atomic<bool> ev2_recorded{false};
};

namespace {

template <typename T> int alloc_shared(vk_corpus *c, T **p, size_t n) {
	VK_HIP(hipMalloc((void **)p, n ? n * sizeof(T) : 16));
	c->device_bytes += (int64_t)(n * sizeof(T));
	c->shared->add((void *)*p);
	return VK_OK;
}

}

int vk_wait_peer_turn(vk_corpus *c, hipStream_t st);
int vk_validate_query(const vk_corpus *c, const vk_query_desc *q, const vk_topk_out *out);
int vk_longq_query(vk_corpus *c, const vk_query_desc *q, vk_topk_out *out, vk_host_keep &keep);
void vk_pack_query(const vk_corpus *c, const vk_query_desc *q, std::vector<uint8_t> &tile, float *mags, std::vector<uint8_t> *bound_tile = nullptr);

namespace {

template <typename P> void corpus_fields(P &p, const vk_corpus *c) {
	p.tiles = c->d_tiles; p.sent_start = c->d_sent_start; p.sent_end = c->d_sent_end;
	p.nk32 = c->nk32; p.tail = c->tail; p.tile_bytes = c->tile_bytes;
}
template <typename P> auto sim_ops_field(P &p, const vk_corpus *c, int) -> decltype((void)p.sim_ops) { p.sim_ops = c->sim_ops; p.sim_src = c->sim_src.kind; }
template <typename P> void sim_ops_field(P &, const vk_corpus *, long) {}
template <typename P> void corpus_fields_ids(P &p, const vk_corpus *c) {
	corpus_fields(p, c);
	sim_ops_field(p, c, 0);
	p.tok_id = c->d_tok_id; p.prec = c->prec;
	p.layout = c->desc.layout == VK_LAYOUT_STATIC ? VK_DEV_LAYOUT_STATIC : VK_DEV_LAYOUT_CONTEXTUAL;
}
template <typename P, typename G> void gap_fields(P &p, const G &g) {
	p.gs = g.gs; p.gt = g.gt; p.a_s = g.a_s; p.a_t = g.a_t; p.open_s = g.open_s; p.open_t = g.open_t;
}

inline float ref_total_of(const vk_query_desc *q) {
	if (!q->tag_weights) return (float)q->len_t;
	float total = 0.0f;
	for (int j = 0; j < q->len_t; j++) total += q->tag_weights[j];
	return total;
}
template <typename P> void tag_weight_fields(P &p, const vk_corpus *c, const vk_query_desc *q, int cols) {
	const bool tagged = q->tag_weights != nullptr;
	for (int j = 0; j < cols; j++) {
		p.tw[j] = (tagged && j < q->len_t) ? q->tag_weights[j] : 0.0f;
		p.tpos[j] = (tagged && j < q->len_t) ? (int32_t)q->q_pos[j] : -1;
	}
	p.ref_total = ref_total_of(q);
	if (!tagged) return;
	p.pos_s = c->d_pos; p.tw_keep = 1.0f - q->pos_mismatch_penalty; p.tw_threshold = q->similarity_threshold;
}

void state_timings(vk_corpus *c, bool flow, int scored = 2) {
	float ms = 0;
	vk_timings t{};
	if (hipEventElapsedTime(&ms, c->ev[0], c->ev[5]) == hipSuccess) t.prepare_ms = ms;
	if (hipEventElapsedTime(&ms, c->ev[5], c->ev[1]) == hipSuccess) t.queue_ms = ms;
	if (hipEventElapsedTime(&ms, c->ev[1], c->ev[scored]) == hipSuccess) t.score_ms = ms;
	if (hipEventElapsedTime(&ms, c->ev[scored], c->ev[3]) == hipSuccess) t.topk_ms = ms;
	if (flow && hipEventElapsedTime(&ms, c->ev[3], c->ev[4]) == hipSuccess) t.flow_ms = ms;
	if (hipEventElapsedTime(&ms, c->ev[0], c->ev[4]) == hipSuccess) t.total_ms = ms - t.queue_ms;
	c->last = t;
}

int select_waves(vk_corpus *c, float floor, int kk, hipStream_t st, const uint64_t **d_sel) {
	int64_t nw = 0;
	int cur = 0;
	VK_HIP(vk_launch_topk_wave(c->d_scores, nullptr, c->n_entries, floor, kk, 4096, c->d_keys[0], &nw, st));
	while (nw > 1) {
		const int64_t nkeys = nw * kk;
		const int64_t per_wave = nkeys <= 16384 ? nkeys : 4096;
		VK_HIP(vk_launch_topk_wave(nullptr, c->d_keys[cur], nkeys, 0.0f, kk, per_wave, c->d_keys[1 - cur], &nw, st));
		cur = 1 - cur;
	}
	*d_sel = c->d_keys[cur];
	return VK_OK;
}
int select_blocks(vk_corpus *c, float floor, int kk, hipStream_t st, const uint64_t **d_sel, const float *scores = nullptr) {
	int nb = 0, cur = 0;
	VK_HIP(vk_launch_topk_scores(scores ? scores : (const float *)c->d_scores, c->n_entries, floor, kk, c->d_keys[0], &nb, st));
	while (nb > 1) {
		VK_HIP(vk_launch_topk_keys(c->d_keys[cur], (int64_t)nb * kk, kk, c->d_keys[1 - cur], &nb, st));
		cur = 1 - cur;
	}
	*d_sel = c->d_keys[cur];
	return VK_OK;
}

int upload_boost(vk_corpus *c, const float *boost, vk_host_keep &keep, hipStream_t st, bool *nonneg = nullptr) {
	const int64_t n = c->n_entries;
	if (nonneg) {
		float least = 0.0f;
		bool nan = false;
		for (int64_t s = 0; s < c->desc.n_sentences; s++) { least = std::min(least, boost[s]); nan = nan || boost[s] != boost[s]; }
		*nonneg = !(least < 0.0f) && !nan;
	}
	if (int rc = c->d_boost.reserve((size_t)n + 8, &c->device_bytes)) return rc;
	if (!c->entry_sent.empty()) {
		std::vector<float> &rows = keep.vec<float>((size_t)n);
		for (int64_t e = 0; e < n; e++) rows[(size_t)e] = c->entry_sent[(size_t)e] >= 0 ? boost[c->entry_sent[(size_t)e]] : 1.0f;
		boost = rows.data();
	}
	VK_HIP(hipMemcpyAsync(c->d_boost, boost, (size_t)n * 4, hipMemcpyHostToDevice, st));
	return VK_OK;
}

constexpr size_t vk_source_tile_floats(int d) { return 16 * (size_t)d + 16; }
int upload_source_query(vk_corpus *c, const vk_query_desc *q, vk_host_keep &keep, hipStream_t st) {
	const int d = c->desc.d, nq = (q->len_t + 15) / 16;
	const size_t per = vk_source_tile_floats(d);
	std::vector<float> &rows = keep.vec<float>(per * (size_t)nq);
	std::fill(rows.begin(), rows.end(), 0.0f);
	for (int i = 0; i < q->len_t; i++) {
		float *row = rows.data() + (size_t)(i >> 4) * per + (size_t)(i & 15) * d;
		for (int k = 0; k < d; k++)
			row[k] = q->q_dtype == VK_F32 ? ((const float *)q->q_vectors)[(size_t)i * d + k] : bf16_to_f32(((const uint16_t *)q->q_vectors)[(size_t)i * d + k]);
		rows[(size_t)(i >> 4) * per + 16 * (size_t)d + (size_t)(i & 15)] = vk_host::sim_src_abs_sum(row, d);
	}
	if (int rc = c->d_qraw.reserve(rows.size(), &c->device_bytes)) return rc;
	VK_HIP(hipMemcpyAsync(c->d_qraw, rows.data(), rows.size() * 4, hipMemcpyHostToDevice, st));
	return VK_OK;
}
VkSimSrcArgs source_table_args(const vk_corpus *c, int t) {
	VkSimSrcArgs a{};
	a.src = c->sim_src; a.raw_tiles = c->raw_rows ? (const uint8_t *)*c->raw_rows : nullptr; a.raw_tile_bytes = c->raw_tile_bytes; a.d = c->desc.d;
	a.q_rows = (const float *)c->d_qraw + (size_t)t * vk_source_tile_floats(c->desc.d);
	a.q_abs_sums = a.q_rows + 16 * (size_t)c->desc.d;
	return a;
}

int64_t row_of_sentence(vk_corpus *c, int64_t s) {
	if (c->entry_sent.empty()) return s;
	if (c->sent_entry.empty()) {
		c->sent_entry.assign((size_t)c->desc.n_sentences, -1);
		for (int64_t e = 0; e < c->n_entries; e++) if (c->entry_sent[(size_t)e] >= 0) c->sent_entry[(size_t)c->entry_sent[(size_t)e]] = (int32_t)e;
	}
	return (int64_t)c->sent_entry[(size_t)s];
}

int launch_wrd_exact_both(vk_corpus *c, VkWrdParams &w, int count, float *scores_to_mark, bool long_too, hipStream_t st) {
	VK_HIP(vk_launch_wrd_exact(&w, count, scores_to_mark, st));
	if (long_too) {
		if (w.nq > 1)
			if (int rc = c->d_wrdl_scratch.reserve((size_t)vk_wrd_long_blocks() * vk_wrd_long_scratch_bytes(), &c->device_bytes)) return rc;
		w.scratch = c->d_wrdl_scratch; w.scratch_stride = (int64_t)vk_wrd_long_scratch_bytes();
		VK_HIP(vk_launch_wrd_exact_long(&w, count, st));
	}
	return VK_OK;
}

}

#endif
```

### vectorian_amd/csrc/vk_query.cpp

```cpp

#include "vk_internal.h"
#include "vk_guard.h"
#include "vk_transport_host.h"

static constexpr int kCanonMargin = 8;
static const vk_host::route_fits kRouteFits{vk_score32_waves, vk_wide_ring_rows, vk_wide_lds_demand};
static bool exact_transport(const vk_query_desc *q) { return vk_host::exact_transport(q->algorithm, q->wmd_full != 0); }
static vk_host::route_facts route_facts_of(const vk_corpus *c, const vk_query_desc *q, const vk_topk_out *out) {
	vk_host::route_facts f;
	f.layout = c->desc.layout; f.prec = c->prec; f.nk32 = c->nk32; f.tail = c->tail;
	f.max_len = c->max_len; f.max_short_len = c->max_short_len; f.n_long_groups = c->n_long_groups;
	f.has_apart = c->h_apart && !c->h_apart->empty(); f.has_xlong = c->h_xlong && !c->h_xlong->empty();
	f.max_pair_tiles = c->max_pair_tiles; f.max_short_pair_tiles = c->max_short_pair_tiles; f.uniform_len = c->uniform_len;
	f.has_pos = c->d_pos != nullptr; f.has_tags = c->d_tag != nullptr; f.n_sentences = c->desc.n_sentences;
	f.algorithm = q->algorithm; f.wmd_full = q->wmd_full != 0; f.rwmd_injective = q->rwmd_injective != 0; f.len_t = q->len_t;
	if (q->algorithm == VK_ALG_ALIGN) {
		f.gaps = vk_host::classify_gaps(q->gap_s, q->gap_t);
		if (f.gaps.gap_mode == 2 && q->gap_s.kind >= VK_GAP_LINEAR && q->gap_s.kind <= VK_GAP_TABLE) f.ws_tail = vk_host::ws_tail_of(q->gap_s, c->max_len);
	}
	f.submatch = q->submatch_weight > 0.0f; f.tagged = q->tag_weights != nullptr; f.has_q_tags = q->q_tags != nullptr; f.has_q_ids = q->q_token_ids != nullptr;
	f.only = q->only_slices != nullptr; f.want_flow = q->want_flow != 0; f.locality = q->locality;
	f.sim_rows = out->sim_rows != nullptr; f.raw_score = out->raw_score != nullptr; f.boost = q->boost != nullptr;
	const int k = q->max_matches;
	const bool restated = (q->want_flow && q->algorithm == VK_ALG_ALIGN) || (q->algorithm == VK_ALG_RWMD && !q->wmd_full && q->want_flow && out->sim_rows);
	f.kk = f.only ? q->n_only : (int)std::min<int64_t>(!restated ? k : (k <= VK_MAX_MATCHES ? std::min(k + kCanonMargin, VK_MAX_MATCHES) : k + kCanonMargin), std::max<int64_t>(c->n_entries, 1));
	return f;
}

int vk_validate_query(const vk_corpus *c, const vk_query_desc *q, const vk_topk_out *out) {
	if (!c || !q || !out) return fail(VK_ERR_INVALID, "null argument");
	if (!c->finalized) return fail(VK_ERR_STATE, "corpus not finalized");
	if (q->len_t < 1) return fail(VK_ERR_INVALID, "empty query");
	if (q->len_t > VK_MAX_LONG_QUERY_LEN) return fail(VK_ERR_UNSUPPORTED, "query longer than VK_MAX_LONG_QUERY_LEN (512) tokens");
	if (q->len_t > VK_MAX_QUERY_LEN) {
		if (q->algorithm != VK_ALG_ALIGN) return fail(VK_ERR_UNSUPPORTED, "queries of more than VK_MAX_QUERY_LEN (64) tokens: alignments only (the transports keep a lane per query token)");
		if (c->max_len > VK_MAX_SENT_LEN) return fail(VK_ERR_UNSUPPORTED, "queries of more than 64 tokens over a corpus that holds a slice of more than VK_MAX_SENT_LEN (512) tokens: the state of such a slice does not fit a workgroup's LDS");
		if (q->submatch_weight != 0.0f) return fail(VK_ERR_UNSUPPORTED, "queries of more than 64 tokens with a submatch weight");
		if (out->sim_rows) return fail(VK_ERR_UNSUPPORTED, "queries of more than 64 tokens: similarity rows of the winners are not returned");
		if (q->max_matches > VK_MAX_MATCHES) return fail(VK_ERR_UNSUPPORTED, "queries of more than 64 tokens: max_matches <= VK_MAX_MATCHES");
	}
	if (q->len_t <= VK_MAX_QUERY_LEN) {
		const vk_host::query_route r = vk_host::route_query(route_facts_of(c, q, out), vk_host::route_switches{}, kRouteFits);
		if (r.status != VK_OK && !r.fits32) return fail(r.status, r.message);
	}
	if (c->max_len > VK_MAX_SENT_LEN && q->algorithm != VK_ALG_ALIGN) {
		const bool relaxed_11 = q->algorithm == VK_ALG_RWMD && !q->wmd_full && q->rwmd_injective;
		if (!relaxed_11)
			return fail(VK_ERR_UNSUPPORTED, "slices of more than VK_MAX_SENT_LEN (512) tokens: alignments and the relaxed 1:1 word mover's distance only (the 1:n form and the exact transports keep a slice's bag of words in LDS)");
		if (c->desc.layout == VK_LAYOUT_STATIC && q->tag_weights && q->q_tags && q->q_token_ids && c->d_tag)
			return fail(VK_ERR_UNSUPPORTED, "slices of more than VK_MAX_SENT_LEN (512) tokens: tag-weighted vocabulary transports keyed by (id, tag) rewrite cells of a slice's rows in LDS");
	}
	if (!q->q_vectors) return fail(VK_ERR_INVALID, "q_vectors is null");
	if (q->q_dtype != VK_F32 && q->q_dtype != VK_BF16) return fail(VK_ERR_INVALID, "bad q_dtype");
	if (q->max_matches < 1 || q->max_matches > VK_MAX_MATCHES_SORTED) return fail(VK_ERR_INVALID, "max_matches out of range");
	if (q->max_matches > VK_MAX_MATCHES && !q->only_slices && (q->algorithm != VK_ALG_ALIGN || q->submatch_weight != 0.0f || out->sim_rows))
		return fail(VK_ERR_UNSUPPORTED, "max_matches beyond VK_MAX_MATCHES (1024): alignments without a submatch weight only");
	if (out->capacity < q->max_matches) return fail(VK_ERR_INVALID, "output capacity smaller than max_matches");
	if (!out->score || !out->sentence) return fail(VK_ERR_INVALID, "output arrays missing");
	if (out->sim_rows && out->rows_per_winner != 0 && (out->rows_per_winner < VK_FAST_SENT_LEN || out->rows_per_winner % 64 != 0 || out->rows_per_winner > VK_MAX_DOC_LEN + 1))
		return fail(VK_ERR_INVALID, "rows_per_winner must be 0 or a multiple of 64 (64 .. VK_MAX_DOC_LEN + 1)");
	if (!(q->submatch_weight >= 0.0f)) return fail(VK_ERR_INVALID, "submatch_weight must be >= 0 (pow of a zero base, metric/alignment.h:97-99)");
	if (q->only_slices) {
		if (q->n_only < 1 || q->n_only > VK_MAX_MATCHES || q->n_only > out->capacity) return fail(VK_ERR_INVALID, "only_slices: n_only out of range (1 .. min(VK_MAX_MATCHES, capacity))");
		const bool relaxed = q->algorithm == VK_ALG_RWMD && !q->wmd_full && out->sim_rows != nullptr;
		const bool exact = exact_transport(q);
		if (!(q->algorithm == VK_ALG_ALIGN || relaxed || exact) || !q->want_flow || (q->submatch_weight != 0.0f && q->algorithm != VK_ALG_ALIGN))
			return fail(VK_ERR_UNSUPPORTED, "only_slices states alignments, relaxed WMD with sim_rows, or exact transports, with want_flow (and submatch_weight = 0 for the transports)");
		for (int i = 0; i < q->n_only; i++)
			if (q->only_slices[i] < 0 || q->only_slices[i] >= c->desc.n_sentences) return fail(VK_ERR_INVALID, "only_slices: slice index out of range");
	}
	if (q->bidirectional) return fail(VK_ERR_UNSUPPORTED, "bidirectional is not implemented (unused upstream, query.cpp:81-83)");
	int rc = VK_OK;
	const auto tag_weights = [&]() -> int {
		if (!q->tag_weights) return VK_OK;
		if (!q->q_pos) return fail(VK_ERR_INVALID, "tag-weighted query without q_pos");
		if (!c->d_pos) return fail(VK_ERR_STATE, "tag-weighted query needs vk_corpus_set_token_pos");
		if (q->similarity_threshold < 0.0f) return fail(VK_ERR_INVALID, "similarity_threshold must be >= 0 (slice/static.h:209)");
		return VK_OK;
	};
	const auto flow_arrays = [&]() -> int {
		return (q->want_flow && (!out->mapping || !out->edge_sim)) ? fail(VK_ERR_INVALID, "want_flow needs mapping and edge_sim arrays") : VK_OK;
	};
	if (q->algorithm == VK_ALG_ALIGN) {
		if (q->locality < VK_LOCAL || q->locality > VK_SEMIGLOBAL) return fail(VK_ERR_INVALID, "bad locality");
		for (const vk_gap *g : {&q->gap_s, &q->gap_t}) {
			if (g->kind < VK_GAP_LINEAR || g->kind > VK_GAP_TABLE) return fail(VK_ERR_INVALID, "bad gap kind");
			if (g->kind == VK_GAP_TABLE && (!g->table || g->n_table < 1)) return fail(VK_ERR_INVALID, "gap table missing");
		}
		if (q->gap_s.kind == VK_GAP_TABLE && q->gap_s.n_table <= c->max_len) return fail(VK_ERR_INVALID, "gap_s table shorter than the longest sentence");
		if (q->gap_t.kind == VK_GAP_TABLE && q->gap_t.n_table <= q->len_t) return fail(VK_ERR_INVALID, "gap_t table shorter than the query");
		if ((rc = flow_arrays())) return rc;
		if ((rc = tag_weights())) return rc;
	} else if (q->algorithm == VK_ALG_RWMD) {
		if ((rc = tag_weights())) return rc;
		if (q->tag_weights) {
			if (q->q_tags && c->desc.layout == VK_LAYOUT_STATIC) {
				if (c->desc.vocab_size > (1 << 23)) return fail(VK_ERR_UNSUPPORTED, "tag-weighted transport with q_tags over the static layout: vocabularies of more than 2^23 entries overflow the (id, tag) keys");
				for (int j = 0; j < q->len_t; j++) {
					if (q->q_tags[j] < 0) return fail(VK_ERR_INVALID, "q_tags: tag codes must be 0 .. 127");
					if (q->q_token_ids && q->q_token_ids[j] >= (1 << 23)) return fail(VK_ERR_UNSUPPORTED, "q_token_ids: ids of 2^23 and more overflow the (id, tag) keys");
				}
			}
			if (q->q_tags && !q->rwmd_injective && !q->wmd_full && c->desc.layout == VK_LAYOUT_STATIC && !c->d_tag)
				return fail(VK_ERR_STATE, "tag-weighted 1:n RWMD over the static layout with q_tags needs vk_corpus_set_token_tags (its vocabulary is keyed by (token, tag), bow.h:150-176)");
		}
		if (q->rwmd_symmetric && !q->rwmd_normalize_bow)
			return fail(VK_ERR_INVALID, "cannot run symmetric mode WMD with bow (needs nbow)");
		if (q->wmd_full) {
			if (q->rwmd_injective) return fail(VK_ERR_INVALID, "non-relaxed WMD with injective mapping is not supported");
			if (q->rwmd_symmetric) return fail(VK_ERR_INVALID, "non-relaxed WMD with symmetric computation is not supported");
		}
		if ((rc = flow_arrays())) return rc;
	} else if (q->algorithm == VK_ALG_WRD) {
		if ((rc = tag_weights())) return rc;
		if (!c->d_mag) return fail(VK_ERR_STATE, "VK_ALG_WRD needs a corpus created with keep_magnitudes = 1");
		if ((rc = flow_arrays())) return rc;
	} else {
		return fail(VK_ERR_INVALID, "bad algorithm");
	}
	return VK_OK;
}

void vk_pack_query(const vk_corpus *c, const vk_query_desc *q, std::vector<uint8_t> &tile, float *mags, std::vector<uint8_t> *bound_tile) {
	const int d = c->desc.d;
	tile.assign((size_t)c->tile_bytes * (size_t)((q->len_t + 15) / 16), 0);
	std::vector<float> row((size_t)d);
	for (int i = 0; i < q->len_t; i++) {
		for (int k = 0; k < d; k++)
			row[(size_t)k] = q->q_dtype == VK_F32 ? ((const float *)q->q_vectors)[(size_t)i * d + k]
			                                       : bf16_to_f32(((const uint16_t *)q->q_vectors)[(size_t)i * d + k]);
		double acc = 0.0;
		for (int k = 0; k < d; k++) acc += (double)row[(size_t)k] * (double)row[(size_t)k];
		float m = (float)std::sqrt(acc);
		if (m != m) m = 0.0f;
		mags[i] = m;
		if (q->q_normalize) {
			for (int k = 0; k < d; k++) {
				float v = row[(size_t)k] / m;
				if (v != v) v = 0.0f;
				row[(size_t)k] = v;
			}
		}
		for (int k = 0; k < d; k++) {
			if (c->prec) {
				const size_t off = (size_t)(i >> 4) * c->tile_bytes + (size_t)(k >> 4) * 1024 + (size_t)((k & 3) * 16 + (i & 15)) * 16 + (size_t)((k & 15) >> 2) * 4;
				memcpy(&tile[off], &row[(size_t)k], 4);
				continue;
			}
			const uint16_t b = f32_to_bf16(row[(size_t)k]);
			const int t = k >> 5, g = (k & 31) >> 3, j = k & 7;
			const size_t off = (size_t)(i >> 4) * c->tile_bytes + (size_t)t * 1024 + (size_t)(g * 16 + (i & 15)) * 16 + (size_t)j * 2;
			memcpy(&tile[off], &b, 2);
		}
	}
	if (!bound_tile || !c->shadow || c->prec || q->len_t > VK_FAST_QUERY_LEN) return;
	std::vector<float> stored((size_t)q->len_t * d);
	for (int i = 0; i < q->len_t; i++)
		for (int k = 0; k < d; k++) {
			uint16_t b;
			memcpy(&b, &tile[(size_t)(k >> 5) * 1024 + (size_t)(((k & 31) >> 3) * 16 + i) * 16 + (size_t)(k & 7) * 2], 2);
			stored[(size_t)i * d + k] = bf16_to_f32(b);
		}
	vk_host::pack_bound_query(c->shadow_format, stored.data(), q->len_t, c->shadow_n, c->shadow_x, *bound_tile);
}

static int score_bounded(vk_corpus *c, const VkScoreParams &p, int grid, size_t smem, size_t smem_bound, size_t smem_list, int kk, float sel_floor,
	const vk_gap &gap_s, bool tail, vk_host_keep &keep, hipStream_t st, const uint64_t **d_sel) {
	*d_sel = nullptr;
	const int64_t n = c->n_entries;
	vk_corpus::bound_state &b = c->bp;
	const int64_t most = std::max<int64_t>(n / 16, kBoundRound2Floor);
	const int M = kk <= 32 ? 64 : kk <= 256 ? 512 : VK_MAX_MATCHES;
	int rc;
	if ((rc = c->d_ub.reserve((size_t)n + 8, &c->device_bytes))) return rc;
	if ((rc = c->d_bound_groups.reserve((size_t)std::max<int64_t>(most, kTopkChunk), &c->device_bytes))) return rc;
	if ((rc = c->d_bound_keys.reserve((size_t)2 * kTopkChunk, &c->device_bytes))) return rc;
	if ((rc = c->d_counter.reserve(4, &c->device_bytes))) return rc;
	VkScoreParams pb = p;
	const vk_host::shadow_format &sf = c->shadow_format;
	pb.tiles = c->shadow; pb.nk32 = sf.steps; pb.tail = 0; pb.tile_bytes = sf.tile_bytes(); pb.bound_bits = sf.bits; pb.bound_live = sf.live; pb.bound_compact = sf.compact;
	pb.q_mode3 = 0; pb.q_lds = 0; pb.qtile = c->d_qtile8; pb.scores = c->d_ub; pb.raw = nullptr;
	b.tail_k = 0;
	if (tail && (p.gap_mode == 3 || p.gap_mode == 6)) {
		const int rows = p.gap_mode == 3 ? 32 : 64, K = sf.bits == 6 ? vk_score_m8t_tail_k() : vk_score_m7t_tail_k();
		float w[65];
		for (int j = 0; j <= rows; j++) w[j] = gap_cost(gap_s, j);
		pb.gap_mode = p.gap_mode == 3 ? 8 : 9;
		pb.bound_tail_cost = vk_host::bound_tail_cost(w, K, rows);
		b.tail_k = K;
	}
	VK_HIP(vk_launch_score(&pb, grid, smem_bound, st));
	VK_HIP(hipEventRecord(c->ev[2], st));
	c->ev2_recorded = true;
	b.ran = 1; b.queries++;
	VK_HIP(hipMemsetD32Async(static_cast<hipDeviceptr_t>(c->d_scores), (int)0xff800000u, (size_t)n, st));
	if (p.raw) VK_HIP(hipMemsetD32Async(reinterpret_cast<hipDeviceptr_t>(p.raw), (int)0xff800000u, (size_t)n, st));
	VkScoreParams pl = p;
	pl.group_list = c->d_bound_groups;
	const uint64_t *d_first = nullptr;
	if ((rc = select_blocks(c, sel_floor, M, st, &d_first, c->d_ub))) return rc;
	VK_HIP(vk_launch_key_groups(d_first, M, c->d_bound_groups, st));
	pl.n_list = M;
	VK_HIP(vk_launch_score(&pl, M, smem_list, st));
	uint64_t *d_exact = c->d_bound_keys, *d_best = c->d_bound_keys + kTopkChunk;
	VK_HIP(vk_launch_rekey(d_first, M, c->d_scores, sel_floor, d_exact, st));
	VK_HIP(vk_launch_topk_unsorted(d_exact, M, kk, d_best, st));
	VK_HIP(vk_launch_select_ge_key(c->d_ub, n, d_best + (kk - 1), sel_floor, c->d_keys[0], c->d_counter, (uint32_t)most, st));
	uint32_t &count = *keep.array<uint32_t>(1);
	VK_HIP(hipMemcpyAsync(&count, c->d_counter, 4, hipMemcpyDeviceToHost, st));
	VK_HIP(hipStreamSynchronize(st));
	b.round1 = M;
	bool fell = false;
	if ((int64_t)count > most) {
		fell = true;
		VK_HIP(vk_launch_score(&p, grid, smem, st));
	} else if (count > 0) {
		VK_HIP(vk_launch_key_groups(c->d_keys[0], (int32_t)count, c->d_bound_groups, st));
		pl.n_list = (int32_t)count;
		VK_HIP(vk_launch_score(&pl, (int32_t)count, smem_list, st));
	}
	if (!fell && count <= (uint32_t)kTopkChunk) {
		VK_HIP(vk_launch_rekey(c->d_keys[0], (int32_t)count, c->d_scores, sel_floor, d_exact, st));
		VK_HIP(vk_launch_topk_unsorted(d_exact, (int32_t)count, kk, d_best, st));
		*d_sel = d_best;
	}
	b.round2 = count;
	if (!fell) b.survivors += count;
	b.fell_back = fell ? 1 : 0;
	if (fell) b.fallbacks++;
	if (bound_pass_mode() == 0) b.backoff.record(fell);
	b.pruned = !fell;
	b.full = p; b.full_grid = grid; b.full_smem = smem;
	return VK_OK;
}

static int query_body(vk_corpus_t *c, const vk_query_desc *q, vk_topk_out *out, vk_host_keep &keep) {
	int rc = VK_OK;
	VK_HIP(hipSetDevice(c->device));
	c->bp.pruned = false; c->bp.ran = c->bp.round1 = c->bp.round2 = c->bp.fell_back = c->bp.tail_k = 0;
	for (int64_t &x : c->query_route) x = -1;
	if (q->len_t > VK_MAX_QUERY_LEN) return vk_longq_query(c, q, out, keep);
	hipStream_t st = c->stream;
	const int64_t n = c->n_entries;
	const int k = q->max_matches;
	const bool only = q->only_slices != nullptr;
	out->n_out = 0;
	c->have_scores = false;
	if (n == 0) return VK_OK;
	const vk_host::route_switches sw = vk_host::read_route_switches();
	vk_host::route_facts facts = route_facts_of(c, q, out);
	const int bound_mode = bound_pass_mode();
	facts.bound_pass = c->shadow && bound_mode >= 0 && (bound_mode > 0 || c->desc.n_sentences >= kBoundPassMinSentences) && vk_host::bound_pass_takes(facts) &&
		(bound_mode != 0 || c->bp.backoff.take());
	const vk_host::query_route r = vk_host::route_query(facts, sw, kRouteFits);
	if (r.status != VK_OK) return fail(r.status, r.message);
	const int64_t route_state[VK_QR_COUNT] = {r.plan, r.gap_mode, r.wide_gap_mode, r.score32_gap_mode, r.wave_tiles, r.pass[vk_host::CLASS_SHORT],
		r.pass[vk_host::CLASS_MID], r.pass[vk_host::CLASS_XLONG], r.list, r.ring_rows, r.flow, r.ostride, r.raw, r.span_skip_raw};
	memcpy(c->query_route, route_state, sizeof route_state);
	const bool wide_query = q->len_t > VK_FAST_QUERY_LEN;
	const bool xlong = c->max_len > VK_MAX_SENT_LEN;
	const bool wide_family = r.flow != vk_host::FLOW_NARROW;
	auto sentence_of = [c](int64_t row) { return c->entry_sent.empty() ? row : (int64_t)c->entry_sent[(size_t)row]; };
	const bool is_static_l = c->desc.layout == VK_LAYOUT_STATIC;
	auto fill_transport = [&](VkWrdParams &w) {
		corpus_fields_ids(w, c);
		w.table = c->d_table; w.table_stride = (int64_t)c->n_tiles * 16 * 16;
		w.qtile = c->d_qtile; w.nq = (q->len_t + 15) / 16; w.len_t = q->len_t; w.mag = c->d_mag;
		w.d = c->desc.d; w.q_ids = is_static_l ? (int32_t *)c->d_qids : nullptr;
		tag_weight_fields(w, c, q, VK_MAX_QUERY_LEN);
		if (q->tag_weights) {
			if (is_static_l && q->algorithm == VK_ALG_RWMD && q->q_tags && q->q_token_ids && c->d_tag && c->d_qbits) {
				w.tag_s = c->d_tag; w.qid_bits = c->d_qbits;
				for (int j = 0; j < VK_MAX_QUERY_LEN; j++)
					w.qkey[j] = (j < q->len_t && q->q_token_ids[j] >= 0 && q->q_token_ids[j] < c->desc.vocab_size) ? q->q_token_ids[j] * 256 + ((int32_t)q->q_tags[j] & 255) : -1;
			}
		}
	};
	auto transport_flows = [&](const std::vector<int64_t> &rows_idx, bool exact, const float *qmass, int mass_mode, int raw_masses, float *rows_dst = nullptr) -> int {
		if (!q->want_flow || !out->sim_rows || rows_idx.empty()) return VK_OK;
		if (!rows_dst) rows_dst = out->sim_rows;
		const int nqw = (q->len_t + 15) / 16, W = 16 * nqw;
		const int R = out->rows_per_winner > 0 ? out->rows_per_winner : VK_FAST_SENT_LEN;
		if (R % 64 != 0 || R > VK_MAX_DOC_LEN + 1 || (exact && R > VK_MAX_SENT_LEN))
			return fail(VK_ERR_INVALID, "rows_per_winner must be a multiple of 64, at most VK_MAX_SENT_LEN (rows without plans: VK_MAX_DOC_LEN + 1)");
		int rc2;
		const int cnt = (int)rows_idx.size();
		const size_t need = (size_t)cnt * R * W;
		if ((rc2 = c->d_rows_out.reserve(need, &c->device_bytes))) return rc2;
		if ((rc2 = c->d_plan_out.reserve(need, &c->device_bytes))) return rc2;
		if ((rc2 = c->d_wrd_raw.reserve((size_t)VK_MAX_MATCHES, &c->device_bytes))) return rc2;
		if ((rc2 = c->d_wrd_val.reserve((size_t)VK_MAX_MATCHES, &c->device_bytes))) return rc2;
		std::vector<uint64_t> &hk = keep.vec<uint64_t>((size_t)cnt);
		for (int i = 0; i < cnt; i++) hk[(size_t)i] = vk_host::key_of_row(rows_idx[(size_t)i]);
		VK_HIP(hipMemcpyAsync(c->d_keys[1], hk.data(), hk.size() * 8, hipMemcpyHostToDevice, c->stream));
		VkWrdParams w{};
		fill_transport(w);
		w.keys = c->d_keys[1]; w.rows_out = c->d_rows_out; w.rows_len = R;
		if (R > VK_MAX_SENT_LEN) {
			VK_HIP(hipMemsetAsync(c->d_rows_out, 0, need * 4, c->stream));
			VK_HIP(vk_launch_canon_rows(&w, cnt, (c->max_len + 15) / 16 + 1, c->stream));
		} else VK_HIP(vk_launch_rows(&w, cnt, c->stream));
		VK_HIP(hipMemcpyAsync(rows_dst, c->d_rows_out, need * 4, hipMemcpyDeviceToHost, c->stream));
		if (exact && out->plan) {
			w.mass_mode = mass_mode; w.raw_masses = raw_masses;
			memcpy(w.qmass, qmass, sizeof w.qmass);
			w.raw_out = c->d_wrd_raw; w.val_out = c->d_wrd_val; w.plan_out = c->d_plan_out;
			VK_HIP(hipMemsetAsync(c->d_plan_out, 0, need * 4, c->stream));
			if ((rc2 = launch_wrd_exact_both(c, w, cnt, nullptr, R > VK_FAST_SENT_LEN && c->max_len > VK_FAST_SENT_LEN, c->stream))) return rc2;
			VK_HIP(hipMemcpyAsync(out->plan, c->d_plan_out, need * 4, hipMemcpyDeviceToHost, c->stream));
		}
		VK_HIP(hipStreamSynchronize(c->stream));
		return VK_OK;
	};

	VK_HIP(hipEventRecord(c->ev[0], st));
	std::vector<uint8_t> &qtile = keep.vec<uint8_t>();
	float qmags[VK_MAX_QUERY_LEN] = {0};
	const int nq = (q->len_t + 15) / 16;
	bool bound_ok = r.plan == vk_host::PLAN_BOUNDED;
	std::vector<uint8_t> &qtile8 = keep.vec<uint8_t>();
	vk_pack_query(c, q, qtile, qmags, bound_ok ? &qtile8 : nullptr);
	VK_HIP(hipMemcpyAsync(c->d_qtile, qtile.data(), qtile.size(), hipMemcpyHostToDevice, st));
	bound_ok = bound_ok && !qtile8.empty();
	if (bound_ok) {
		if ((rc = c->d_qtile8.reserve(qtile8.size(), &c->device_bytes))) return rc;
		VK_HIP(hipMemcpyAsync(c->d_qtile8, qtile8.data(), qtile8.size(), hipMemcpyHostToDevice, st));
	}

	VkScoreParams p{};
	float qmass_all[VK_MAX_QUERY_LEN] = {0};
	const size_t n_ws = std::max<size_t>((size_t)kGapTable, (size_t)c->max_len + 2);
	std::vector<float> &ws = keep.vec<float>(n_ws);
	float *wt = keep.array<float>(160);
	const bool is_align = q->algorithm == VK_ALG_ALIGN;
	if (q->algorithm == VK_ALG_WRD) {
		float sum_t = 0.0f;
		for (int j = 0; j < q->len_t; j++) sum_t += qmags[j];
		const bool rawm = !q->wrd_normalize_magnitudes;
		for (int j = 0; j < VK_MAX_QUERY_LEN; j++) qmass_all[j] = j < q->len_t ? (rawm ? qmags[j] : qmags[j] / sum_t) : 0.0f;
		memcpy(p.qmass, qmass_all, sizeof p.qmass);
		p.wrd_raw_total = rawm ? sum_t : 0.0f;
		p.mag = c->d_mag;
	} else if (q->algorithm == VK_ALG_RWMD) {
		p.rwmd_symmetric = q->rwmd_symmetric;
		p.rwmd_normalize_bow = q->rwmd_normalize_bow;
		if (q->wmd_full) {
			p.wmd_bound = q->rwmd_normalize_bow ? 1 : 2;
			for (int j = 0; j < q->len_t; j++) qmass_all[j] = q->rwmd_normalize_bow ? 1.0f / (float)q->len_t : 1.0f;
		}
		else if (!q->rwmd_injective) {
			const bool ids = c->desc.layout == VK_LAYOUT_STATIC && q->q_token_ids;
			for (int j = 0; j < VK_MAX_QUERY_LEN; j++) {
				float mass = 0.0f;
				if (j < q->len_t) {
					int cnt = 1;
					bool first = true;
					const bool tagged = q->tag_weights && q->q_tags;
					if (ids && q->q_token_ids[j] >= 0)
						for (int i = 0; i < q->len_t; i++)
							if (i != j && q->q_token_ids[i] == q->q_token_ids[j] && (!tagged || q->q_tags[i] == q->q_tags[j])) { cnt++; if (i < j) first = false; }
					mass = first ? (q->rwmd_normalize_bow ? (float)cnt / (float)q->len_t : (float)cnt) : 0.0f;
				}
				qmass_all[j] = mass;
			}
			memcpy(p.qmass, qmass_all, sizeof p.qmass);
			if (ids && q->tag_weights && q->q_tags) p.tag_s = c->d_tag;
		}
	} else gap_fields(p, facts.gaps);
	p.gap_mode = r.gap_mode;
	for (size_t i = 0; i < n_ws; i++) ws[i] = (is_align && (int64_t)i <= c->max_len) ? gap_cost(q->gap_s, (int)i) : 0.0f;
	if ((rc = c->d_ws.reserve(n_ws, &c->device_bytes))) return rc;
	vk_host::wt_with_closure(wt, q->gap_t, q->len_t, is_align);
	VK_HIP(hipMemcpyAsync(c->d_ws, ws.data(), n_ws * sizeof(float), hipMemcpyHostToDevice, st));
	VK_HIP(hipMemcpyAsync(c->d_wt, wt, 160 * sizeof(float), hipMemcpyHostToDevice, st));

	bool boost_nonneg = true;
	if (q->boost && (rc = upload_boost(c, q->boost, keep, st, bound_ok ? &boost_nonneg : nullptr))) return rc;
	bound_ok = bound_ok && boost_nonneg;

	const bool is_static = c->desc.layout == VK_LAYOUT_STATIC;
	const int64_t table_stride = (int64_t)c->n_tiles * 16 * 16;
	if (is_static) {
		int32_t *ids = keep.array<int32_t>(80);
		for (int j = 0; j < 80; j++) ids[j] = (q->q_token_ids && j < q->len_t) ? q->q_token_ids[j] : -1;
		VK_HIP(hipMemcpyAsync(c->d_qids, ids, 80 * sizeof(int32_t), hipMemcpyHostToDevice, st));
		const bool sourced = c->sim_src.kind != VK_SIMSRC_COSINE;
		if (sourced && (rc = upload_source_query(c, q, keep, st))) return rc;
		for (int t = 0; t < nq && (!only || sourced); t++) {
			const VkSimSrcArgs sa = source_table_args(c, t);
			VK_HIP(vk_launch_table(c->d_tiles, c->d_qtile + (size_t)t * c->tile_bytes, (int32_t)c->n_tiles, c->nk32, c->tail, c->tile_bytes,
				c->d_table + t * table_stride, q->q_token_ids ? c->d_qids + t * 16 : nullptr, std::min(16, q->len_t - t * 16), c->desc.vocab_size, c->prec, &c->sim_ops,
				sourced ? &sa : nullptr, st));
		}
	}

	const bool do_flow = q->want_flow && is_align;
	const bool canon_tr = q->algorithm == VK_ALG_RWMD && !q->wmd_full && q->want_flow && out->sim_rows != nullptr;
	const int kk = facts.kk;
	const float sel_floor = (do_flow || canon_tr) ? q->min_score - 1e-5f * std::max(1.0f, std::fabs(q->min_score)) : q->min_score;

	VK_HIP(hipEventRecord(c->ev[5], st));
	if ((rc = vk_wait_peer_turn(c, st))) return rc;
	VK_HIP(hipEventRecord(c->ev[1], st));
	corpus_fields_ids(p, c);
	p.table = c->d_table; p.n_sent = (int32_t)n;
	p.qtile = c->d_qtile; p.len_t = q->len_t; p.locality = q->locality;
	p.ws = c->d_ws; p.wt = c->d_wt + 80; p.wt0 = c->d_wt;
	p.boost = q->boost ? (float *)c->d_boost : nullptr;
	p.scores = c->d_scores; p.raw = c->d_raw;
	tag_weight_fields(p, c, q, VK_FAST_QUERY_LEN);
	int32_t qkey_all[VK_MAX_QUERY_LEN];
	for (int j = 0; j < VK_MAX_QUERY_LEN; j++) qkey_all[j] = -1;
	const bool vocab_fix = is_static && q->algorithm == VK_ALG_RWMD && q->tag_weights && q->q_tags && q->q_token_ids && c->d_tag && c->d_pos;
	if (vocab_fix) {
		const size_t words = ((size_t)c->desc.vocab_size + 31) / 32 + 1;
		if ((rc = c->d_qbits.reserve(words, &c->device_bytes))) return rc;
		std::vector<uint32_t> &bits = keep.vec<uint32_t>(words, 0u);
		for (int j = 0; j < q->len_t; j++) {
			const int32_t id = q->q_token_ids[j];
			if (id < 0 || id >= c->desc.vocab_size) continue;
			bits[(size_t)id >> 5] |= 1u << (id & 31);
			qkey_all[j] = id * 256 + ((int32_t)q->q_tags[j] & 255);
		}
		VK_HIP(hipMemcpyAsync(c->d_qbits, bits.data(), words * 4, hipMemcpyHostToDevice, st));
		VK_HIP(hipStreamSynchronize(st));
		p.qid_bits = c->d_qbits; p.tag_s = c->d_tag; p.slices_overlap = c->overlapping ? 1 : 0;
		for (int j = 0; j < VK_FAST_QUERY_LEN; j++) p.qkey[j] = qkey_all[j];
	}
	bool bounded = false;
	const uint64_t *d_sel_bounded = nullptr;
	VkWideParams wp{};
	auto wide_order = [&](vk_host::route_list list) -> int {
		const bool all = list == vk_host::LIST_ALL, apart = list == vk_host::LIST_APART;
		vk_devbuf<int32_t> &d_ord = all ? c->d_wide_order : apart ? c->d_apart_order : c->d_xlong_order;
		int32_t &n_ord = all ? c->n_wide_order : apart ? c->n_apart_order : c->n_xlong_order;
		if (n_ord < 0) {
			std::vector<int32_t> ord;
			if (all) { for (int64_t e = 0; e < n; e++) if ((*c->h_end)[(size_t)e] > (*c->h_start)[(size_t)e]) ord.push_back((int32_t)e); }
			else if (apart && c->h_apart) ord = *c->h_apart;
			else if (!apart && c->h_xlong) ord = *c->h_xlong;
			std::stable_sort(ord.begin(), ord.end(), [&](int32_t a, int32_t b) {
				return (*c->h_end)[(size_t)a] - (*c->h_start)[(size_t)a] > (*c->h_end)[(size_t)b] - (*c->h_start)[(size_t)b]; });
			int rcw;
			if ((rcw = d_ord.reserve(ord.size() + 1, &c->device_bytes))) return rcw;
			VK_HIP(hipMemcpy(d_ord, ord.data(), ord.size() * 4, hipMemcpyHostToDevice));
			n_ord = (int32_t)ord.size();
		}
		wp.order = d_ord; wp.n_order = n_ord;
		if (all) {
			VK_HIP(hipMemsetD32Async(static_cast<hipDeviceptr_t>(c->d_scores), (int)0xff800000u, (size_t)n, st));
			if (wp.raw) VK_HIP(hipMemsetD32Async(reinterpret_cast<hipDeviceptr_t>(wp.raw), (int)0xff800000u, (size_t)n, st));
		}
		return VK_OK;
	};
	auto wide_state = [&](int flow_k) -> int {
		const bool flow = flow_k > 0;
		const vk_host::route_list list = flow ? vk_host::LIST_NONE : r.list;
		wp.scratch = nullptr; wp.scratch_stride = 0; wp.h_ring = 0; wp.order = nullptr; wp.n_order = 0;
		if (flow ? r.wide_lds_flow : r.wide_lds_score)
			return list == vk_host::LIST_APART || list == vk_host::LIST_XLONG ? wide_order(list) : VK_OK;
		wp.h_ring = r.ring_rows;
		size_t per = vk_wide_scratch_bytes(c->max_len, nq, wp.gap_mode, flow, wp.h_ring);
		if (flow && r.flow == vk_host::FLOW_DOC) per = std::max(per, vk_doc_scratch_bytes(c->max_len, wp.gap_mode));
		if (flow && r.flow == vk_host::FLOW_DOCW) per = std::max(per, vk_docw_scratch_bytes(c->max_len, nq));
		if (flow && r.flow == vk_host::FLOW_DOCG) per = std::max(per, vk_docg_scratch_bytes(c->max_len));
		const size_t blocks = (size_t)vk_wide_gs_blocks(c->max_len, nq, wp.gap_mode, flow_k, n, wp.h_ring);
		const size_t need = per * blocks;
		if (need > ((size_t)16 << 30)) return fail(VK_ERR_UNSUPPORTED, "traceback state of this many slices this long exceeds 16 GiB of scratch");
		if (int rcw = c->d_wide_scratch.reserve(need, &c->device_bytes)) return rcw;
		wp.scratch = c->d_wide_scratch; wp.scratch_stride = (int64_t)per;
		return list != vk_host::LIST_NONE ? wide_order(list) : VK_OK;
	};
	auto list_pass = [&]() -> int {
		const vk_host::route_pass pass = r.wide_pass;
		if (int rcw = (pass == vk_host::PASS_WIDE || pass == vk_host::PASS_DOC) ? wide_state(0) : wide_order(r.list)) return rcw;
		if (wp.order && wp.n_order == 0) return VK_OK;
		if (pass == vk_host::PASS_DOCW) VK_HIP(vk_launch_docw(&wp, 0, st));
		else if (pass == vk_host::PASS_DOCG) VK_HIP(vk_launch_docg(&wp, 0, st));
		else if (pass == vk_host::PASS_DOC) VK_HIP(vk_launch_doc(&wp, 0, st));
		else VK_HIP(vk_launch_wide(&wp, 0, st));
		return VK_OK;
	};
	if (wide_family || r.list != vk_host::LIST_NONE) {
		corpus_fields_ids(wp, c);
		wp.table = c->d_table; wp.table_stride = table_stride; wp.n_sent = (int32_t)n;
		wp.qtile = c->d_qtile; wp.nq = nq; wp.len_t = q->len_t; wp.locality = q->locality; wp.max_len = c->max_len;
		wp.gap_mode = r.wide_gap_mode;
		wp.rwmd_symmetric = p.rwmd_symmetric; wp.rwmd_normalize_bow = p.rwmd_normalize_bow;
		gap_fields(wp, p);
		wp.ws = c->d_ws; wp.wt = c->d_wt; wp.wt0 = c->d_wt;
		wp.ws_tail = facts.ws_tail;
		tag_weight_fields(wp, c, q, VK_MAX_QUERY_LEN);
		wp.tag_s = p.tag_s; wp.qid_bits = p.qid_bits; wp.slices_overlap = p.slices_overlap; memcpy(wp.qkey, qkey_all, sizeof wp.qkey);
		wp.boost = p.boost; wp.scores = c->d_scores; wp.raw = r.raw ? (float *)c->d_raw : nullptr;
		wp.d = c->desc.d; wp.q_ids = is_static ? (int32_t *)c->d_qids : nullptr;
	}
	if (r.plan == vk_host::PLAN_MULTI_BLOCK) {
		const bool exact = exact_transport(q);
		if (exact || r.score32_gap_mode == 7) memcpy(wp.qmass, qmass_all, sizeof wp.qmass);
		if (exact) {
			wp.mag = q->algorithm == VK_ALG_WRD ? c->d_mag : nullptr;
			wp.wrd_raw_total = p.wrd_raw_total; wp.wmd_bound = q->algorithm == VK_ALG_WRD ? 0 : p.wmd_bound;
		}
		wp.gap_mode = r.score32_gap_mode;
		if (r.wide_gap_mode == 2) wp.wt = c->d_wt + 80;
		VK_HIP(vk_launch_score32(&wp, r.wave_tiles, st));
		if (r.pass[vk_host::CLASS_MID] == vk_host::PASS_LONG_RWMD_FILL) VK_HIP(vk_launch_long_rwmd_fill(&wp, c->d_long_groups, c->n_long_groups, (int32_t)n, st));
		else if (r.pass[vk_host::CLASS_MID] == vk_host::PASS_LONG_BOUND) {
			VkWrdParams lw{};
			fill_transport(lw);
			lw.mag = q->algorithm == VK_ALG_WRD ? c->d_mag : nullptr;
			memcpy(lw.qmass, qmass_all, sizeof lw.qmass);
			lw.wrd_raw_total = p.wrd_raw_total; lw.wmd_bound = wp.wmd_bound;
			lw.group_list = c->d_long_groups; lw.n_list = c->n_long_groups; lw.n_entries = (int32_t)n;
			lw.scores = c->d_scores; lw.raw = c->d_raw; lw.boost = p.boost;
			VK_HIP(vk_launch_long_bound(&lw, st));
		}
		wp.gap_mode = r.wide_gap_mode;
		wp.wt = c->d_wt;
		if (r.wide_pass != vk_host::PASS_NONE && (rc = list_pass())) return rc;
	} else if (r.plan == vk_host::PLAN_DOCW_ALL || r.plan == vk_host::PLAN_DOCG_ALL || r.plan == vk_host::PLAN_WIDE_ALL) {
		if ((rc = list_pass())) return rc;
	} else if (r.plan == vk_host::PLAN_SPAN) {
		VkScoreParams ps = p;
		if (r.span_skip_raw) ps.raw = nullptr;
		VK_HIP(vk_launch_span(&ps, st));
	} else if (!wide_query) {
	p.max_short_len = VK_FAST_SENT_LEN;
	if (!r.raw) p.raw = nullptr;
	p.s_rows_per_wave = is_static ? (c->max_group_tokens + 15) / 16 * 16 : c->max_group_tiles * 16;
	p.h_rows = c->max_short_len + 1;
	const int lt = q->len_t <= 4 ? 4 : q->len_t <= 8 ? 8 : q->len_t <= 12 ? 12 : 16;
	int lds_floats = p.s_rows_per_wave * lt + 16;
	if (p.gap_mode == 2) lds_floats += 4 * p.h_rows * 16;
	p.m_rows = (c->max_short_len + 4) / 4 * 4;
	if (p.gap_mode == 7) lds_floats += 4 * p.m_rows;
	p.lds_floats_per_wave = lds_floats;
	size_t smem = (size_t)lds_floats * 4 * 4;
	const bool reg_history = p.gap_mode == 3 || p.gap_mode == 6;
	if (!is_static && c->prec == 0 && c->nk32 == 10 && c->tail == 1)
		p.q_mode3 = sw.qlds ? 1 : sw.qreg ? 0 : (reg_history ? 1 : 0);
	if (!is_static && c->prec == 1 && c->nk32 == 19 && !sw.no_f32_special) p.q_mode3 = 1;
// ... 520 lines not shown
```

### vectorian_amd/csrc/vk_score.hip.h

```cpp
#ifndef VK_SCORE_HIP_H
#define VK_SCORE_HIP_H

#include <type_traits>
#include "vk_common.hip.h"


#ifdef VK_SCORE_VGPRS
#define VK_SCORE_KERNEL_ATTR __attribute__((amdgpu_num_vgpr(VK_SCORE_VGPRS)))
#else
#define VK_SCORE_KERNEL_ATTR
#endif

template <int MODE, int NK32, bool TAIL, int GAP, int LT>
__global__ __launch_bounds__(256) VK_SCORE_KERNEL_ATTR void vk_score_kernel(VkScoreParams p) {
	extern __shared__ float4 vk_smem4[];
	float *smem = reinterpret_cast<float *>(vk_smem4);
	const int lane = threadIdx.x & 63, wv = threadIdx.x >> 6;
	const int nwaves = blockDim.x >> 6;
	const uint8_t *qlds = reinterpret_cast<const uint8_t *>(smem);
	if constexpr (MODE == 3 || MODE == 4) {
		for (int i = threadIdx.x; i < NK32 * 64; i += blockDim.x)
			vk_smem4[i] = *reinterpret_cast<const float4 *>(p.qtile + i * 16);
		__syncthreads();
		smem += NK32 * 256;
	}
	if constexpr (MODE == 7) {
		for (int i = threadIdx.x; i < NK32 * 64 + 12; i += blockDim.x)
			vk_smem4[i] = *reinterpret_cast<const float4 *>(p.qtile + i * 16);
		__syncthreads();
		smem += NK32 * 256 + VK_DEV_BOUND_CONST_BYTES / 4;
	}
	if constexpr (MODE == 8 || MODE == 9) {
		for (int i = threadIdx.x; i < VK_DEV_FP6_QTILE_BYTES / 16 + 12; i += blockDim.x)
			vk_smem4[i] = *reinterpret_cast<const float4 *>(p.qtile + i * 16);
		__syncthreads();
		smem += (VK_DEV_FP6_QTILE_BYTES + VK_DEV_BOUND_CONST_BYTES) / 4;
	}
	if constexpr (MODE == 1 || MODE == 5 || MODE == 6) {
		if (p.q_lds > 0) {
			for (int i = threadIdx.x; i * 16 < p.q_lds; i += blockDim.x)
				vk_smem4[i] = i * 16 < p.tile_bytes ? *reinterpret_cast<const float4 *>(p.qtile + i * 16) : float4{0.0f, 0.0f, 0.0f, 0.0f};
			__syncthreads();
			smem += p.q_lds / 4;
		}
	}
	float *S = smem + wv * p.lds_floats_per_wave;
	float *Hh = S + p.s_rows_per_wave * LT + 16;
	const int sigma = lane >> 4, v = lane & 15;

	QFrag<NK32, TAIL> qf;
	if constexpr (MODE == 0) load_qfrag<NK32, TAIL>(qf, p.qtile, lane);

	DpArgs a;
	a.locality = p.locality; a.len_t = p.len_t;
	a.gs = p.gs; a.gt = p.gt; a.a_s = p.a_s; a.a_t = p.a_t; a.open_s = p.open_s; a.open_t = p.open_t;
	a.ws = p.ws; a.wt = p.wt; a.wt0 = p.wt0;
	a.rwmd_symmetric = p.rwmd_symmetric; a.rwmd_normalize_bow = p.rwmd_normalize_bow; a.wmd_bound = p.wmd_bound;
	a.wrd_raw_total = p.wrd_raw_total;
	const float inv_ref = p.ref_total;
	constexpr bool TAGS = MODE != 7 && MODE != 8 && MODE != 9;
	float twl[4] = {1.0f, 1.0f, 1.0f, 1.0f};
	int tposl[4] = {0, 0, 0, 0};
	if (TAGS && p.pos_s) {
		const int cbase = (MODE == 2) ? (lane & 3) * 4 : (lane >> 4) * 4;
#pragma unroll
		for (int r = 0; r < 4; r++) { twl[r] = p.tw[cbase + r]; tposl[r] = p.tpos[cbase + r]; }
	}

	constexpr bool FLAT = GAP == 8 || GAP == 9;
	static_assert(!FLAT || MODE == 7 || MODE == 8 || MODE == 9, "a flat-tailed table gives a bound, not a score");
	constexpr int WSN = FLAT ? VK_BOUND_TAIL_K + 2 : GAP == 6 ? 65 : 33;
	float wsr[WSN], wtr[LT];
	if (GAP == 3 || GAP == 6 || FLAT) {
#pragma unroll
		for (int k = 0; k < (FLAT ? WSN - 1 : WSN); k++) wsr[k] = p.ws[k];
		if (FLAT) wsr[WSN - 1] = p.bound_tail_cost;
#pragma unroll
		for (int k = 0; k < LT; k++) wtr[k] = p.wt[k];
	}

	const int n_groups = p.group_list ? p.n_list : (p.n_sent + 3) >> 2;
	const int run = p.group_list ? 1 : VK_RUN;
	const int n_runs = (n_groups + run - 1) / run;
	for (int ri = blockIdx.x * nwaves + wv; ri < n_runs; ri += gridDim.x * nwaves) {
	int prev_tile = -1, prev_row = 0;
	for (int gg = 0; gg < run; gg++) {
		const int gi = ri * run + gg;
		if (gi >= n_groups) break;
		const int grp = p.group_list ? p.group_list[gi] : gi;
		const int s_idx = grp * 4 + sigma;
		const int i0 = s_idx < p.n_sent ? s_idx : p.n_sent;
		const int t_a = p.sent_start[i0], t_b = p.sent_end[i0];
		const int len = t_b - t_a;
		const int g_a = __builtin_amdgcn_readlane(t_a, 0);
		const int g_b = __builtin_amdgcn_readlane(t_b, 48);
		int maxlen = __builtin_amdgcn_readlane(len, 0);
		maxlen = max(maxlen, __builtin_amdgcn_readlane(len, 16));
		maxlen = max(maxlen, __builtin_amdgcn_readlane(len, 32));
		maxlen = max(maxlen, __builtin_amdgcn_readlane(len, 48));
		if (!p.group_list && maxlen > p.max_short_len) { prev_tile = -1; continue; }

		int rowbase;
		if (MODE == 2) {
			const int ntok = g_b - g_a;
			for (int it0 = 0; it0 * 16 < ntok; it0 += 4) {
				int id[4];
				float4 val[4];
#pragma unroll
				for (int q4 = 0; q4 < 4; q4++) {
					const int tk = (it0 + q4) * 16 + (lane >> 2);
					id[q4] = p.tok_id[g_a + (tk < ntok ? tk : 0)];
				}
#pragma unroll
				for (int q4 = 0; q4 < 4; q4++)
					val[q4] = *reinterpret_cast<const float4 *>(p.table + (int64_t)id[q4] * 16 + (lane & 3) * 4);
#pragma unroll
				for (int q4 = 0; q4 < 4; q4++) {
					const int tk = (it0 + q4) * 16 + (lane >> 2);
					if (tk < ntok) {
						float4 vq = val[q4];
						if (p.pos_s) {
							const int ps = p.pos_s[g_a + tk];
							vq.x = tag_weighted(vq.x, twl[0], ps, tposl[0], p.tw_keep, p.tw_threshold);
							vq.y = tag_weighted(vq.y, twl[1], ps, tposl[1], p.tw_keep, p.tw_threshold);
							vq.z = tag_weighted(vq.z, twl[2], ps, tposl[2], p.tw_keep, p.tw_threshold);
							vq.w = tag_weighted(vq.w, twl[3], ps, tposl[3], p.tw_keep, p.tw_threshold);
						}
						if ((lane & 3) * 4 < LT) *reinterpret_cast<float4 *>(S + tk * LT + (lane & 3) * 4) = vq;
					}
				}
			}
			rowbase = t_a - g_a;
		} else {
			const int tile0 = g_a >> 4;
			const int ntiles = ((g_b + 15) >> 4) - tile0;
			const uint8_t *tp = p.tiles + (int64_t)tile0 * p.tile_bytes;
			int ti0 = 0;
			if (ntiles > 0 && tile0 == prev_tile) {
				if (prev_row != 0) {
					float4 keep = {0.0f, 0.0f, 0.0f, 0.0f};
					if (lane < 4 * LT) keep = reinterpret_cast<const float4 *>(S)[prev_row * 4 * LT + lane];
					wave_lds_fence();
					if (lane < 4 * LT) reinterpret_cast<float4 *>(S)[lane] = keep;
				}
				ti0 = 1;
				tp += p.tile_bytes;
			}
			if (ntiles > 0) { prev_tile = tile0 + ntiles - 1; prev_row = ntiles - 1; }
			if constexpr (MODE == 8 || MODE == 9) {
				constexpr int T = GAP == 6 ? 1 : GAP == 8 ? VK_FP6_TILES_TAIL : GAP == 9 ? VK_FP6_TILES_TAIL64 : VK_FP6_TILES;
				const auto tiles = [&](auto tc, int ti) {
					constexpr int N = decltype(tc)::value;
					f32x4 ub[N];
					sim_tiles_fp6<N, MODE == 9>(ub, qlds, tp, p.tile_bytes, lane, p.bound_live);
#pragma unroll
					for (int i = 0; i < N; i++)
						if ((lane >> 4) * 4 < LT) *reinterpret_cast<f32x4 *>(S + ((ti + i) * 16 + (lane & 15)) * LT + (lane >> 4) * 4) = ub[i];
					tp += (int64_t)N * p.tile_bytes;
				};
				int ti = ti0;
				for (; ti + T <= ntiles; ti += T) tiles(std::integral_constant<int, T>{}, ti);
				if constexpr (T > 1)
					for (; ti < ntiles; ti++) tiles(std::integral_constant<int, 1>{}, ti);
			} else
			for (int ti = ti0; ti < ntiles; ti++) {
				f32x4 acc;
				if constexpr (MODE == 0) acc = sim_tile<NK32, TAIL>(qf, tp, lane);
				else if constexpr (MODE == 3) acc = sim_tile_qlds<NK32, TAIL>(qlds, tp, lane);
				else if constexpr (MODE == 4) acc = sim_tile_f32_qlds<NK32>(qlds, tp, lane);
				else if constexpr (MODE == 7) acc = sim_tile_i8<NK32>(qlds, tp, lane, p.bound_live);
				else {
					constexpr bool DEEP = MODE == 5 || MODE == 6;
					constexpr int PREC = MODE == 6 ? 1 : 0;
					if (p.q_lds > 0) acc = sim_tile_generic<DEEP, PREC>(qlds, tp, p.nk32, p.tail, lane);
					else acc = sim_tile_generic<DEEP, PREC>(p.qtile, tp, p.nk32, p.tail, lane);
				}
				if (TAGS && p.pos_s) {
					const int ps = p.pos_s[(tile0 + ti) * 16 + (lane & 15)];
#pragma unroll
					for (int r = 0; r < 4; r++) acc[r] = tag_weighted(acc[r], twl[r], ps, tposl[r], p.tw_keep, p.tw_threshold);
				}
				if ((lane >> 4) * 4 < LT) *reinterpret_cast<f32x4 *>(S + (ti * 16 + (lane & 15)) * LT + (lane >> 4) * 4) = acc;
				tp += p.tile_bytes;
			}
			rowbase = t_a - tile0 * 16;
		}
		wave_lds_fence();
		int turns = 1;
		bool rewrite = false;
		if constexpr (MODE == 2 && (GAP == 4 || GAP == 7)) {
			if (p.qid_bits) {
				rewrite = len > 0 && static_vocab_shared(len, p.len_t, p.tok_id + t_a, p.tag_s + t_a, p.qid_bits, p.qkey) != 0;
				if (p.slices_overlap && __builtin_amdgcn_ballot_w64(rewrite) != 0) turns = 4;
				else if (rewrite) static_vocab_fixup<16>(S + rowbase * LT, LT, len, p.len_t, p.tok_id + t_a, p.tag_s + t_a, p.pos_s + t_a, p.table, 0,
					p.qid_bits, p.qkey, p.tw, p.tpos, p.tw_keep, p.tw_threshold, v);
				wave_lds_fence();
			}
		}

		const int lenc = len > 0 ? len : 0;
		const int rb = len > 0 ? rowbase : 0;
		auto evaluate = [&]() -> float {
		float raw;
		if constexpr (GAP == 0) raw = dp_linear<LT>(S, rb, lenc, maxlen, v, a);
		else if constexpr (GAP == 1) raw = dp_affine<LT>(S, rb, lenc, maxlen, v, a);
		else if constexpr (GAP == 2) raw = dp_general<LT>(S, Hh, p.h_rows, rb, lenc, maxlen, lane, a);
		else if constexpr (GAP == 3) raw = dp_general_reg<LT, 32>(S, rb, lenc, maxlen, v, a, wsr, wtr);
		else if constexpr (GAP == 6) raw = dp_general_reg<LT, 64, MODE != 7>(S, rb, lenc, maxlen, v, a, wsr, wtr);
		else if constexpr (GAP == 8) raw = dp_general_tail_reg<LT, 32, VK_BOUND_TAIL_K>(S, rb, lenc, maxlen, v, a, wsr, wtr);
		else if constexpr (GAP == 9) raw = dp_general_tail_reg<LT, 64, VK_BOUND_TAIL_K, MODE != 7>(S, rb, lenc, maxlen, v, a, wsr, wtr);
		else if constexpr (GAP == 4) {
			if (a.wmd_bound == 1) raw = wrd_bound_rows<LT>(S, rb, lenc, maxlen, v, a, nullptr, nullptr, 1.0f / (float)a.len_t);
			else raw = rwmd_rows<LT>(S, rb, lenc, maxlen, v, a);
		}
		else if constexpr (GAP == 7) {
			float *sm = nullptr;
			if (MODE == 2) {
				sm = Hh + sigma * p.m_rows;
				const float wsum = p.rwmd_normalize_bow ? (float)(lenc > 0 ? lenc : 1) : 1.0f;
				for (int u = v; u < lenc; u += 16) {
					const int id = p.tok_id[t_a + u];
					int cnt = 0;
					bool first = true;
					for (int i = 0; i < lenc; i++) {
						const bool same = p.tok_id[t_a + i] == id && (!p.tag_s || p.tag_s[t_a + i] == p.tag_s[t_a + u]);
						cnt += same ? 1 : 0;
						first = first && !(same && i < u);
					}
					sm[u] = first ? (float)cnt / wsum : 0.0f;
				}
				wave_lds_fence();
			}
			raw = rwmd_fill_rows<LT>(S, sm, rb, lenc, maxlen, lane, a, p.qmass[v]);
		}
		else if constexpr (MODE == 2) raw = wrd_bound_rows<LT>(S, rb, lenc, maxlen, v, a, p.mag, p.tok_id + (len > 0 ? t_a : 0), p.qmass[v]);
		else raw = wrd_bound_rows<LT>(S, rb, lenc, maxlen, v, a, p.mag + (len > 0 ? t_a : 0), nullptr, p.qmass[v]);
		return raw;
		};
		float raw = 0.0f;
		if constexpr (MODE == 2 && (GAP == 4 || GAP == 7)) {
			if (turns > 1) {
				for (int turn = 0; turn < 4; turn++) {
					const bool mine = sigma == turn;
					if (mine && rewrite) static_vocab_fixup<16>(S + rowbase * LT, LT, len, p.len_t, p.tok_id + t_a, p.tag_s + t_a, p.pos_s + t_a, p.table, 0,
						p.qid_bits, p.qkey, p.tw, p.tpos, p.tw_keep, p.tw_threshold, v);
					wave_lds_fence();
					const float r = evaluate();
					if (mine) raw = r;
					wave_lds_fence();
					if (mine && rewrite) static_vocab_fixup<16, false, true>(S + rowbase * LT, LT, len, p.len_t, p.tok_id + t_a, p.tag_s + t_a, p.pos_s + t_a, p.table, 0,
						p.qid_bits, p.qkey, p.tw, p.tpos, p.tw_keep, p.tw_threshold, v);
					wave_lds_fence();
				}
			} else raw = evaluate();
		} else raw = evaluate();

		if (v == 15 && s_idx < p.n_sent) {
			float val = VK_NEG_INF, r = VK_NEG_INF;
			if (len >= 1) {
				const float boost = p.boost ? p.boost[s_idx] : 1.0f;
				r = raw;
				val = (raw / inv_ref) * boost;
			}
			p.scores[s_idx] = val;
			if (p.raw) p.raw[s_idx] = r;
		}
		wave_lds_fence();
	}
	}
}

template <typename K>
static hipError_t launch_sized(K kernel, const VkScoreParams &p, int want_blocks, size_t smem, hipStream_t stream) {
	int occ = 0;
	const int threads = p.group_list ? 64 : 256;
	hipError_t e;
	if (smem > 64 * 1024) {
		e = hipFuncSetAttribute(reinterpret_cast<const void *>(kernel), hipFuncAttributeMaxDynamicSharedMemorySize, (int)smem);
		if (e != hipSuccess) return e;
	}
	e = hipOccupancyMaxActiveBlocksPerMultiprocessor(&occ, kernel, threads, smem);
	if (e != hipSuccess) return e;
	if (occ < 1) occ = 1;
	const int real_occ = occ;
	const bool bound_pass = p.gap_mode == 5 || (p.gap_mode == 4 && p.wmd_bound == 1);
	const bool dp_bound = p.layout == VK_DEV_LAYOUT_STATIC || (p.nk32 <= 3 && p.bound_bits == 0);
	const int stream_cap = ((p.bound_bits == 0 && p.nk32 >= 5 && p.nk32 <= 7) || p.bound_bits == 6) ? 4 : 3;
	if (occ > stream_cap && !dp_bound && !bound_pass) occ = stream_cap;
	if (p.nk32 == 24 && p.tail == 0 && p.prec == 0 && p.layout != VK_DEV_LAYOUT_STATIC && !bound_pass) occ = 1;
	const char *ov = getenv("VK_BLOCKS_PER_CU");
	if (ov && atoi(ov) > 0) occ = atoi(ov) < real_occ ? atoi(ov) : real_occ;
	int dev = 0, cus = 256;
	if (hipGetDevice(&dev) == hipSuccess) (void)hipDeviceGetAttribute(&cus, hipDeviceAttributeMultiprocessorCount, dev);
	const int grid = want_blocks < cus * occ ? want_blocks : cus * occ;
	kernel<<<grid, threads, smem, stream>>>(p);
	return hipGetLastError();
}

template <int MODE, int NK32, bool TAIL, int GAP>
static hipError_t launch_score_lt(const VkScoreParams &p, int grid, size_t smem, hipStream_t stream) {
	const int lt = p.len_t <= 4 ? 4 : p.len_t <= 8 ? 8 : p.len_t <= 12 ? 12 : 16;
	switch (lt) {
	case 4: return launch_sized(vk_score_kernel<MODE, NK32, TAIL, GAP, 4>, p, grid, smem, stream);
	case 8: return launch_sized(vk_score_kernel<MODE, NK32, TAIL, GAP, 8>, p, grid, smem, stream);
	case 12: return launch_sized(vk_score_kernel<MODE, NK32, TAIL, GAP, 12>, p, grid, smem, stream);
	default: return launch_sized(vk_score_kernel<MODE, NK32, TAIL, GAP, 16>, p, grid, smem, stream);
	}
}

template <int MODE, int NK32, bool TAIL>
static hipError_t launch_score_gap(const VkScoreParams &p, int grid, size_t smem, hipStream_t stream) {
	switch (p.gap_mode) {
	case 0: return launch_score_lt<MODE, NK32, TAIL, 0>(p, grid, smem, stream);
	case 1: return launch_score_lt<MODE, NK32, TAIL, 1>(p, grid, smem, stream);
	case 3: return launch_score_lt<MODE, NK32, TAIL, 3>(p, grid, smem, stream);
	case 4: return launch_score_lt<MODE, NK32, TAIL, 4>(p, grid, smem, stream);
	case 5: return launch_score_lt<MODE, NK32, TAIL, 5>(p, grid, smem, stream);
	case 6: return launch_score_lt<MODE, NK32, TAIL, 6>(p, grid, smem, stream);
	case 7: return launch_score_lt<MODE, NK32, TAIL, 7>(p, grid, smem, stream);
	default: return launch_score_lt<MODE, NK32, TAIL, 2>(p, grid, smem, stream);
	}
}

#endif
```

### vectorian_amd/csrc/vk_score_m9t.hip

```cpp
#define VK_SCORE_VGPRS 104
#include "vk_score.hip.h"

extern "C" hipError_t vk_launch_score_m9t(const VkScoreParams *p, int32_t grid, size_t smem_bytes, hipStream_t stream) {
	switch (p->gap_mode) {
	case 8: return launch_score_lt<9, VK_DEV_FP6_STEPS, false, 8>(*p, grid, smem_bytes, stream);
	case 9: return launch_score_lt<9, VK_DEV_FP6_STEPS, false, 9>(*p, grid, smem_bytes, stream);
	default: return hipErrorInvalidValue;
	}
}
```

Before: 840.6 million.

## Add specialized local-alignment bound kernel with exact query width and full-length DP

Adds a kernel for the FP6 bound pass with flat tail, used when the locality is local. It is templated on the exact query length, so the in-row DPP max chain covers only the real query columns and the locality checks become compile-time constants. When every sentence in a wave has length 32, a dedicated DP path batches the score loads eight at a time and drops the active-length masks. The shared score-kernel body moves into an include file so both kernels can reuse it. The launcher gains a fixed blocks-per-CU cap and an environment switch to fall back to the generic path; the cost is many more kernel instantiations.

```diff
diff --git a/vectorian_amd/csrc/vk_common.hip.h b/vectorian_amd/csrc/vk_common.hip.h
--- a/vectorian_amd/csrc/vk_common.hip.h
+++ b/vectorian_amd/csrc/vk_common.hip.h
@@ -836,15 +836,18 @@
 	return (is_global) ? m : fmaxf(m, 0.0f);
 }
 
-template <int LT, int MAXLEN, int KT, bool FRESH = true>
+#define VK_DP_LOC_RUNTIME (-1)
+template <int LT, int MAXLEN, int KT, bool FRESH = true, int LOC = VK_DP_LOC_RUNTIME, int LQ = LT>
 __device__ __forceinline__ float dp_general_tail_reg(const float *__restrict__ S, int rowbase, int len, int maxlen, int v,
 	const DpArgs &a, const float (&wsr)[KT + 2], const float (&wtr)[LT]) {
 	static_assert(KT >= 1 && KT < MAXLEN, "the tail begins inside the table");
-	int loc = a.locality, vsel = v;
+	static_assert(LQ >= 1 && LQ <= LT, "the in-row columns are columns of the strip");
+	static_assert(LOC == VK_DP_LOC_RUNTIME || LOC == VK_DEV_LOCAL, "the one compile-time locality is local");
+	int loc = LOC == VK_DP_LOC_RUNTIME ? a.locality : LOC, vsel = v;
 	if constexpr (FRESH) {
-		asm volatile("" : "+v"(loc));
+		if constexpr (LOC == VK_DP_LOC_RUNTIME) asm volatile("" : "+v"(loc));
 		asm volatile("" : "+v"(vsel));
-		loc = __builtin_amdgcn_readfirstlane(loc);
+		if constexpr (LOC == VK_DP_LOC_RUNTIME) loc = __builtin_amdgcn_readfirstlane(loc);
 	}
 	const bool is_local = loc == VK_DEV_LOCAL;
 	const bool is_global = loc == VK_DEV_GLOBAL;
@@ -856,7 +859,7 @@
 
 	float wtv[16];
 #pragma unroll
-	for (int k = 1; k < LT; k++) wtv[k] = vsel >= k ? wtr[k] : __builtin_inff();
+	for (int k = 1; k < LQ; k++) wtv[k] = vsel >= k ? wtr[k] : __builtin_inff();
 
 	float hreg[MAXLEN + 1];
 	float h = is_global ? -wt_border0 : 0.0f;
@@ -879,21 +882,21 @@
 				c = fmaxf(c, R - c_tail);
 			}
 			float hc = fmaxf(c, bcur - wt_border);
-			if (LT > 1) hc = fmaxf(hc, dpp_zero<0x111>(c) - wtv[1]);
-			if (LT > 2) hc = fmaxf(hc, dpp_zero<0x112>(c) - wtv[2]);
-			if (LT > 3) hc = fmaxf(hc, dpp_zero<0x113>(c) - wtv[3]);
-			if (LT > 4) hc = fmaxf(hc, dpp_zero<0x114>(c) - wtv[4]);
-			if (LT > 5) hc = fmaxf(hc, dpp_zero<0x115>(c) - wtv[5]);
-			if (LT > 6) hc = fmaxf(hc, dpp_zero<0x116>(c) - wtv[6]);
-			if (LT > 7) hc = fmaxf(hc, dpp_zero<0x117>(c) - wtv[7]);
-			if (LT > 8) hc = fmaxf(hc, dpp_zero<0x118>(c) - wtv[8]);
-			if (LT > 9) hc = fmaxf(hc, dpp_zero<0x119>(c) - wtv[9]);
-			if (LT > 10) hc = fmaxf(hc, dpp_zero<0x11a>(c) - wtv[10]);
-			if (LT > 11) hc = fmaxf(hc, dpp_zero<0x11b>(c) - wtv[11]);
-			if (LT > 12) hc = fmaxf(hc, dpp_zero<0x11c>(c) - wtv[12]);
-			if (LT > 13) hc = fmaxf(hc, dpp_zero<0x11d>(c) - wtv[13]);
-			if (LT > 14) hc = fmaxf(hc, dpp_zero<0x11e>(c) - wtv[14]);
-			if (LT > 15) hc = fmaxf(hc, dpp_zero<0x11f>(c) - wtv[15]);
+			if (LQ > 1) hc = fmaxf(hc, dpp_zero<0x111>(c) - wtv[1]);
+			if (LQ > 2) hc = fmaxf(hc, dpp_zero<0x112>(c) - wtv[2]);
+			if (LQ > 3) hc = fmaxf(hc, dpp_zero<0x113>(c) - wtv[3]);
+			if (LQ > 4) hc = fmaxf(hc, dpp_zero<0x114>(c) - wtv[4]);
+			if (LQ > 5) hc = fmaxf(hc, dpp_zero<0x115>(c) - wtv[5]);
+			if (LQ > 6) hc = fmaxf(hc, dpp_zero<0x116>(c) - wtv[6]);
+			if (LQ > 7) hc = fmaxf(hc, dpp_zero<0x117>(c) - wtv[7]);
+			if (LQ > 8) hc = fmaxf(hc, dpp_zero<0x118>(c) - wtv[8]);
+			if (LQ > 9) hc = fmaxf(hc, dpp_zero<0x119>(c) - wtv[9]);
+			if (LQ > 10) hc = fmaxf(hc, dpp_zero<0x11a>(c) - wtv[10]);
+			if (LQ > 11) hc = fmaxf(hc, dpp_zero<0x11b>(c) - wtv[11]);
+			if (LQ > 12) hc = fmaxf(hc, dpp_zero<0x11c>(c) - wtv[12]);
+			if (LQ > 13) hc = fmaxf(hc, dpp_zero<0x11d>(c) - wtv[13]);
+			if (LQ > 14) hc = fmaxf(hc, dpp_zero<0x11e>(c) - wtv[14]);
+			if (LQ > 15) hc = fmaxf(hc, dpp_zero<0x11f>(c) - wtv[15]);
 			hreg[u] = hc;
 			h = act ? hc : h;
 			if (is_local || last_col) best = fmaxf(best, h);
@@ -905,6 +908,66 @@
 	else m = v < a.len_t ? fmaxf(h, last_col ? best : 0.0f) : 0.0f;
 	m = row_max_to_lane15(m);
 	return (is_global) ? m : fmaxf(m, 0.0f);
+}
+
+template <int LT, int LQ, int KT>
+__device__ __forceinline__ float dp_tail_local_full(const float *__restrict__ S, int rowbase, int v, const DpArgs &a,
+	const float (&wsr)[KT + 2], const float (&wtr)[LT]) {
+	static_assert(KT >= 1 && KT < 32, "the tail begins inside the table");
+	static_assert(LQ >= 1 && LQ <= LT, "the in-row columns are columns of the strip");
+	constexpr int BATCH = 8;
+	int vsel = v;
+	asm volatile("" : "+v"(vsel));
+	const float border = 0.0f - a.wt[v + 1];
+	const float c_tail = wsr[KT + 1];
+
+	float wtv[16];
+#pragma unroll
+	for (int k = 1; k < LQ; k++) wtv[k] = vsel >= k ? wtr[k] : __builtin_inff();
+
+	const float *row = S + rowbase * LT + v;
+	float hreg[33];
+	float sv[BATCH];
+	hreg[0] = 0.0f;
+	float R = 0.0f;
+	float best = 0.0f;
+#pragma unroll
+	for (int u = 1; u <= 32; u++) {
+		if ((u - 1) % BATCH == 0) {
+			__builtin_amdgcn_sched_barrier(0);
+#pragma unroll
+			for (int i = 0; i < BATCH; i++) sv[i] = row[(u - 1 + i) * LT];
+			__builtin_amdgcn_sched_barrier(0);
+		}
+		float c = fmaxf(dpp_zero<0x111>(hreg[u - 1]) + sv[(u - 1) % BATCH], 0.0f);
+#pragma unroll
+		for (int k = 1; k <= (u < KT ? u : KT); k++) c = fmaxf(c, hreg[u - k] - wsr[k]);
+		if (u > KT) {
+			if (u > KT + 1) R = fmaxf(R, hreg[u - KT - 1]);
+			c = fmaxf(c, R - c_tail);
+		}
+		float hc = fmaxf(c, border);
+		if (LQ > 1) hc = fmaxf(hc, dpp_zero<0x111>(c) - wtv[1]);
+		if (LQ > 2) hc = fmaxf(hc, dpp_zero<0x112>(c) - wtv[2]);
+		if (LQ > 3) hc = fmaxf(hc, dpp_zero<0x113>(c) - wtv[3]);
+		if (LQ > 4) hc = fmaxf(hc, dpp_zero<0x114>(c) - wtv[4]);
+		if (LQ > 5) hc = fmaxf(hc, dpp_zero<0x115>(c) - wtv[5]);
+		if (LQ > 6) hc = fmaxf(hc, dpp_zero<0x116>(c) - wtv[6]);
+		if (LQ > 7) hc = fmaxf(hc, dpp_zero<0x117>(c) - wtv[7]);
+		if (LQ > 8) hc = fmaxf(hc, dpp_zero<0x118>(c) - wtv[8]);
+		if (LQ > 9) hc = fmaxf(hc, dpp_zero<0x119>(c) - wtv[9]);
+		if (LQ > 10) hc = fmaxf(hc, dpp_zero<0x11a>(c) - wtv[10]);
+		if (LQ > 11) hc = fmaxf(hc, dpp_zero<0x11b>(c) - wtv[11]);
+		if (LQ > 12) hc = fmaxf(hc, dpp_zero<0x11c>(c) - wtv[12]);
+		if (LQ > 13) hc = fmaxf(hc, dpp_zero<0x11d>(c) - wtv[13]);
+		if (LQ > 14) hc = fmaxf(hc, dpp_zero<0x11e>(c) - wtv[14]);
+		if (LQ > 15) hc = fmaxf(hc, dpp_zero<0x11f>(c) - wtv[15]);
+		hreg[u] = hc;
+		best = fmaxf(best, hc);
+	}
+	float m = v < a.len_t ? best : 0.0f;
+	m = row_max_to_lane15(m);
+	return fmaxf(m, 0.0f);
 }
 
 template <int LT>
diff --git a/vectorian_amd/csrc/vk_corpus.cpp b/vectorian_amd/csrc/vk_corpus.cpp
--- a/vectorian_amd/csrc/vk_corpus.cpp
+++ b/vectorian_amd/csrc/vk_corpus.cpp
@@ -640,6 +640,12 @@
 	return VK_OK;
 }
 
+int vk_bound_pass_dp(vk_corpus_t *c, int32_t *out) {
+	if (!c || !out) return fail(VK_ERR_INVALID, "null argument");
+	*out = c->bp.ran ? (int32_t)c->bp.fast_dp : 0;
+	return VK_OK;
+}
+
 int vk_bound_pass_shadow(vk_corpus_t *c, int64_t *format, float *nx, int64_t tile0, int64_t n, uint8_t *out) {
 	if (!c || !format || !nx) return fail(VK_ERR_INVALID, "null argument");
 	const vk_host::shadow_format &sf = c->shadow_format;
diff --git a/vectorian_amd/csrc/vk_device.h b/vectorian_amd/csrc/vk_device.h
--- a/vectorian_amd/csrc/vk_device.h
+++ b/vectorian_amd/csrc/vk_device.h
@@ -386,6 +386,8 @@
 hipError_t vk_launch_score(const VkScoreParams *p, int32_t grid, size_t smem_bytes, hipStream_t stream);
 int32_t vk_score_m8t_tail_k(void);
 int32_t vk_score_m7t_tail_k(void);
+int32_t vk_score_m9f_takes(const VkScoreParams *p);
+hipError_t vk_launch_score_m9f(const VkScoreParams *p, int32_t grid, size_t smem_bytes, hipStream_t stream);
 hipError_t vk_launch_span(const VkScoreParams *p, hipStream_t stream);
 hipError_t vk_launch_score_batch(const VkScoreBatchParams *p, int32_t lt, size_t smem, hipStream_t stream);
 hipError_t vk_launch_topk_scores(const float *scores, int64_t n, float min_score, int32_t k, uint64_t *out,
diff --git a/vectorian_amd/csrc/vk_internal.h b/vectorian_amd/csrc/vk_internal.h
--- a/vectorian_amd/csrc/vk_internal.h
+++ b/vectorian_amd/csrc/vk_internal.h
@@ -179,6 +179,7 @@
 		VkScoreParams full{}; int full_grid = 0; size_t full_smem = 0;
 		int64_t ran = 0, round1 = 0, round2 = 0, fell_back = 0;
 		int64_t tail_k = 0;
+		int64_t fast_dp = 0;
 		int64_t queries = 0, fallbacks = 0, survivors = 0;
 		vk_host::bound_backoff backoff;
 	} bp;
diff --git a/vectorian_amd/csrc/vk_query.cpp b/vectorian_amd/csrc/vk_query.cpp
--- a/vectorian_amd/csrc/vk_query.cpp
+++ b/vectorian_amd/csrc/vk_query.cpp
@@ -189,6 +189,7 @@
 		pb.bound_tail_cost = vk_host::bound_tail_cost(w, K, rows);
 		b.tail_k = K;
 	}
+	b.fast_dp = sf.bits == 6 && sf.compact && vk_score_m9f_takes(&pb) ? 1 : 0;
 	VK_HIP(vk_launch_score(&pb, grid, smem_bound, st));
 	VK_HIP(hipEventRecord(c->ev[2], st));
 	c->ev2_recorded = true;
@@ -237,7 +238,7 @@
 static int query_body(vk_corpus_t *c, const vk_query_desc *q, vk_topk_out *out, vk_host_keep &keep) {
 	int rc = VK_OK;
 	VK_HIP(hipSetDevice(c->device));
-	c->bp.pruned = false; c->bp.ran = c->bp.round1 = c->bp.round2 = c->bp.fell_back = c->bp.tail_k = 0;
+	c->bp.pruned = false; c->bp.ran = c->bp.round1 = c->bp.round2 = c->bp.fell_back = c->bp.tail_k = c->bp.fast_dp = 0;
 	for (int64_t &x : c->query_route) x = -1;
 	if (q->len_t > VK_MAX_QUERY_LEN) return vk_longq_query(c, q, out, keep);
 	hipStream_t st = c->stream;
diff --git a/vectorian_amd/csrc/vk_score.hip.h b/vectorian_amd/csrc/vk_score.hip.h
--- a/vectorian_amd/csrc/vk_score.hip.h
+++ b/vectorian_amd/csrc/vk_score.hip.h
@@ -13,265 +13,12 @@
 
 template <int MODE, int NK32, bool TAIL, int GAP, int LT>
 __global__ __launch_bounds__(256) VK_SCORE_KERNEL_ATTR void vk_score_kernel(VkScoreParams p) {
-	extern __shared__ float4 vk_smem4[];
-	float *smem = reinterpret_cast<float *>(vk_smem4);
-	const int lane = threadIdx.x & 63, wv = threadIdx.x >> 6;
-	const int nwaves = blockDim.x >> 6;
-	const uint8_t *qlds = reinterpret_cast<const uint8_t *>(smem);
-	if constexpr (MODE == 3 || MODE == 4) {
-		for (int i = threadIdx.x; i < NK32 * 64; i += blockDim.x)
-			vk_smem4[i] = *reinterpret_cast<const float4 *>(p.qtile + i * 16);
-		__syncthreads();
-		smem += NK32 * 256;
-	}
-	if constexpr (MODE == 7) {
-		for (int i = threadIdx.x; i < NK32 * 64 + 12; i += blockDim.x)
-			vk_smem4[i] = *reinterpret_cast<const float4 *>(p.qtile + i * 16);
-		__syncthreads();
-		smem += NK32 * 256 + VK_DEV_BOUND_CONST_BYTES / 4;
-	}
-	if constexpr (MODE == 8 || MODE == 9) {
-		for (int i = threadIdx.x; i < VK_DEV_FP6_QTILE_BYTES / 16 + 12; i += blockDim.x)
-			vk_smem4[i] = *reinterpret_cast<const float4 *>(p.qtile + i * 16);
-		__syncthreads();
-		smem += (VK_DEV_FP6_QTILE_BYTES + VK_DEV_BOUND_CONST_BYTES) / 4;
-	}
-	if constexpr (MODE == 1 || MODE == 5 || MODE == 6) {
-		if (p.q_lds > 0) {
-			for (int i = threadIdx.x; i * 16 < p.q_lds; i += blockDim.x)
-				vk_smem4[i] = i * 16 < p.tile_bytes ? *reinterpret_cast<const float4 *>(p.qtile + i * 16) : float4{0.0f, 0.0f, 0.0f, 0.0f};
-			__syncthreads();
-			smem += p.q_lds / 4;
-		}
-	}
-	float *S = smem + wv * p.lds_floats_per_wave;
-	float *Hh = S + p.s_rows_per_wave * LT + 16;
-	const int sigma = lane >> 4, v = lane & 15;
-
-	QFrag<NK32, TAIL> qf;
-	if constexpr (MODE == 0) load_qfrag<NK32, TAIL>(qf, p.qtile, lane);
-
-	DpArgs a;
-	a.locality = p.locality; a.len_t = p.len_t;
-	a.gs = p.gs; a.gt = p.gt; a.a_s = p.a_s; a.a_t = p.a_t; a.open_s = p.open_s; a.open_t = p.open_t;
-	a.ws = p.ws; a.wt = p.wt; a.wt0 = p.wt0;
-	a.rwmd_symmetric = p.rwmd_symmetric; a.rwmd_normalize_bow = p.rwmd_normalize_bow; a.wmd_bound = p.wmd_bound;
-	a.wrd_raw_total = p.wrd_raw_total;
-	const float inv_ref = p.ref_total;
-	constexpr bool TAGS = MODE != 7 && MODE != 8 && MODE != 9;
-	float twl[4] = {1.0f, 1.0f, 1.0f, 1.0f};
-	int tposl[4] = {0, 0, 0, 0};
-	if (TAGS && p.pos_s) {
-		const int cbase = (MODE == 2) ? (lane & 3) * 4 : (lane >> 4) * 4;
-#pragma unroll
-		for (int r = 0; r < 4; r++) { twl[r] = p.tw[cbase + r]; tposl[r] = p.tpos[cbase + r]; }
-	}
-
-	constexpr bool FLAT = GAP == 8 || GAP == 9;
-	static_assert(!FLAT || MODE == 7 || MODE == 8 || MODE == 9, "a flat-tailed table gives a bound, not a score");
-	constexpr int WSN = FLAT ? VK_BOUND_TAIL_K + 2 : GAP == 6 ? 65 : 33;
-	float wsr[WSN], wtr[LT];
-	if (GAP == 3 || GAP == 6 || FLAT) {
-#pragma unroll
-		for (int k = 0; k < (FLAT ? WSN - 1 : WSN); k++) wsr[k] = p.ws[k];
-		if (FLAT) wsr[WSN - 1] = p.bound_tail_cost;
-#pragma unroll
-		for (int k = 0; k < LT; k++) wtr[k] = p.wt[k];
-	}
-
-	const int n_groups = p.group_list ? p.n_list : (p.n_sent + 3) >> 2;
-	const int run = p.group_list ? 1 : VK_RUN;
-	const int n_runs = (n_groups + run - 1) / run;
-	for (int ri = blockIdx.x * nwaves + wv; ri < n_runs; ri += gridDim.x * nwaves) {
-	int prev_tile = -1, prev_row = 0;
-	for (int gg = 0; gg < run; gg++) {
-		const int gi = ri * run + gg;
-		if (gi >= n_groups) break;
-		const int grp = p.group_list ? p.group_list[gi] : gi;
-		const int s_idx = grp * 4 + sigma;
-		const int i0 = s_idx < p.n_sent ? s_idx : p.n_sent;
-		const int t_a = p.sent_start[i0], t_b = p.sent_end[i0];
-		const int len = t_b - t_a;
-		const int g_a = __builtin_amdgcn_readlane(t_a, 0);
-		const int g_b = __builtin_amdgcn_readlane(t_b, 48);
-		int maxlen = __builtin_amdgcn_readlane(len, 0);
-		maxlen = max(maxlen, __builtin_amdgcn_readlane(len, 16));
-		maxlen = max(maxlen, __builtin_amdgcn_readlane(len, 32));
-		maxlen = max(maxlen, __builtin_amdgcn_readlane(len, 48));
-		if (!p.group_list && maxlen > p.max_short_len) { prev_tile = -1; continue; }
-
-		int rowbase;
-		if (MODE == 2) {
-			const int ntok = g_b - g_a;
-			for (int it0 = 0; it0 * 16 < ntok; it0 += 4) {
-				int id[4];
-				float4 val[4];
-#pragma unroll
-				for (int q4 = 0; q4 < 4; q4++) {
-					const int tk = (it0 + q4) * 16 + (lane >> 2);
-					id[q4] = p.tok_id[g_a + (tk < ntok ? tk : 0)];
-				}
-#pragma unroll
-				for (int q4 = 0; q4 < 4; q4++)
-					val[q4] = *reinterpret_cast<const float4 *>(p.table + (int64_t)id[q4] * 16 + (lane & 3) * 4);
-#pragma unroll
-				for (int q4 = 0; q4 < 4; q4++) {
-					const int tk = (it0 + q4) * 16 + (lane >> 2);
-					if (tk < ntok) {
-						float4 vq = val[q4];
-						if (p.pos_s) {
-							const int ps = p.pos_s[g_a + tk];
-							vq.x = tag_weighted(vq.x, twl[0], ps, tposl[0], p.tw_keep, p.tw_threshold);
-							vq.y = tag_weighted(vq.y, twl[1], ps, tposl[1], p.tw_keep, p.tw_threshold);
-							vq.z = tag_weighted(vq.z, twl[2], ps, tposl[2], p.tw_keep, p.tw_threshold);
-							vq.w = tag_weighted(vq.w, twl[3], ps, tposl[3], p.tw_keep, p.tw_threshold);
-						}
-						if ((lane & 3) * 4 < LT) *reinterpret_cast<float4 *>(S + tk * LT + (lane & 3) * 4) = vq;
-					}
-				}
-			}
-			rowbase = t_a - g_a;
-		} else {
-			const int tile0 = g_a >> 4;
-			const int ntiles = ((g_b + 15) >> 4) - tile0;
-			const uint8_t *tp = p.tiles + (int64_t)tile0 * p.tile_bytes;
-			int ti0 = 0;
-			if (ntiles > 0 && tile0 == prev_tile) {
-				if (prev_row != 0) {
-					float4 keep = {0.0f, 0.0f, 0.0f, 0.0f};
-					if (lane < 4 * LT) keep = reinterpret_cast<const float4 *>(S)[prev_row * 4 * LT + lane];
-					wave_lds_fence();
-					if (lane < 4 * LT) reinterpret_cast<float4 *>(S)[lane] = keep;
-				}
-				ti0 = 1;
-				tp += p.tile_bytes;
-			}
-			if (ntiles > 0) { prev_tile = tile0 + ntiles - 1; prev_row = ntiles - 1; }
-			if constexpr (MODE == 8 || MODE == 9) {
-				constexpr int T = GAP == 6 ? 1 : GAP == 8 ? VK_FP6_TILES_TAIL : GAP == 9 ? VK_FP6_TILES_TAIL64 : VK_FP6_TILES;
-				const auto tiles = [&](auto tc, int ti) {
-					constexpr int N = decltype(tc)::value;
-					f32x4 ub[N];
-					sim_tiles_fp6<N, MODE == 9>(ub, qlds, tp, p.tile_bytes, lane, p.bound_live);
-#pragma unroll
-					for (int i = 0; i < N; i++)
-						if ((lane >> 4) * 4 < LT) *reinterpret_cast<f32x4 *>(S + ((ti + i) * 16 + (lane & 15)) * LT + (lane >> 4) * 4) = ub[i];
-					tp += (int64_t)N * p.tile_bytes;
-				};
-				int ti = ti0;
-				for (; ti + T <= ntiles; ti += T) tiles(std::integral_constant<int, T>{}, ti);
-				if constexpr (T > 1)
-					for (; ti < ntiles; ti++) tiles(std::integral_constant<int, 1>{}, ti);
-			} else
-			for (int ti = ti0; ti < ntiles; ti++) {
-				f32x4 acc;
-				if constexpr (MODE == 0) acc = sim_tile<NK32, TAIL>(qf, tp, lane);
-				else if constexpr (MODE == 3) acc = sim_tile_qlds<NK32, TAIL>(qlds, tp, lane);
-				else if constexpr (MODE == 4) acc = sim_tile_f32_qlds<NK32>(qlds, tp, lane);
-				else if constexpr (MODE == 7) acc = sim_tile_i8<NK32>(qlds, tp, lane, p.bound_live);
-				else {
-					constexpr bool DEEP = MODE == 5 || MODE == 6;
-					constexpr int PREC = MODE == 6 ? 1 : 0;
-					if (p.q_lds > 0) acc = sim_tile_generic<DEEP, PREC>(qlds, tp, p.nk32, p.tail, lane);
-					else acc = sim_tile_generic<DEEP, PREC>(p.qtile, tp, p.nk32, p.tail, lane);
-				}
-				if (TAGS && p.pos_s) {
-					const int ps = p.pos_s[(tile0 + ti) * 16 + (lane & 15)];
-#pragma unroll
-					for (int r = 0; r < 4; r++) acc[r] = tag_weighted(acc[r], twl[r], ps, tposl[r], p.tw_keep, p.tw_threshold);
-				}
-				if ((lane >> 4) * 4 < LT) *reinterpret_cast<f32x4 *>(S + (ti * 16 + (lane & 15)) * LT + (lane >> 4) * 4) = acc;
-				tp += p.tile_bytes;
-			}
-			rowbase = t_a - tile0 * 16;
-		}
-		wave_lds_fence();
-		int turns = 1;
-		bool rewrite = false;
-		if constexpr (MODE == 2 && (GAP == 4 || GAP == 7)) {
-			if (p.qid_bits) {
-				rewrite = len > 0 && static_vocab_shared(len, p.len_t, p.tok_id + t_a, p.tag_s + t_a, p.qid_bits, p.qkey) != 0;
-				if (p.slices_overlap && __builtin_amdgcn_ballot_w64(rewrite) != 0) turns = 4;
-				else if (rewrite) static_vocab_fixup<16>(S + rowbase * LT, LT, len, p.len_t, p.tok_id + t_a, p.tag_s + t_a, p.pos_s + t_a, p.table, 0,
-					p.qid_bits, p.qkey, p.tw, p.tpos, p.tw_keep, p.tw_threshold, v);
-				wave_lds_fence();
-			}
-		}
-
-		const int lenc = len > 0 ? len : 0;
-		const int rb = len > 0 ? rowbase : 0;
-		auto evaluate = [&]() -> float {
-		float raw;
-		if constexpr (GAP == 0) raw = dp_linear<LT>(S, rb, lenc, maxlen, v, a);
-		else if constexpr (GAP == 1) raw = dp_affine<LT>(S, rb, lenc, maxlen, v, a);
-		else if constexpr (GAP == 2) raw = dp_general<LT>(S, Hh, p.h_rows, rb, lenc, maxlen, lane, a);
-		else if constexpr (GAP == 3) raw = dp_general_reg<LT, 32>(S, rb, lenc, maxlen, v, a, wsr, wtr);
-		else if constexpr (GAP == 6) raw = dp_general_reg<LT, 64, MODE != 7>(S, rb, lenc, maxlen, v, a, wsr, wtr);
-		else if constexpr (GAP == 8) raw = dp_general_tail_reg<LT, 32, VK_BOUND_TAIL_K>(S, rb, lenc, maxlen, v, a, wsr, wtr);
-		else if constexpr (GAP == 9) raw = dp_general_tail_reg<LT, 64, VK_BOUND_TAIL_K, MODE != 7>(S, rb, lenc, maxlen, v, a, wsr, wtr);
-		else if constexpr (GAP == 4) {
-			if (a.wmd_bound == 1) raw = wrd_bound_rows<LT>(S, rb, lenc, maxlen, v, a, nullptr, nullptr, 1.0f / (float)a.len_t);
-			else raw = rwmd_rows<LT>(S, rb, lenc, maxlen, v, a);
-		}
-		else if constexpr (GAP == 7) {
-			float *sm = nullptr;
-			if (MODE == 2) {
-				sm = Hh + sigma * p.m_rows;
-				const float wsum = p.rwmd_normalize_bow ? (float)(lenc > 0 ? lenc : 1) : 1.0f;
-				for (int u = v; u < lenc; u += 16) {
-					const int id = p.tok_id[t_a + u];
-					int cnt = 0;
-					bool first = true;
-					for (int i = 0; i < lenc; i++) {
-						const bool same = p.tok_id[t_a + i] == id && (!p.tag_s || p.tag_s[t_a + i] == p.tag_s[t_a + u]);
-						cnt += same ? 1 : 0;
-						first = first && !(same && i < u);
-					}
-					sm[u] = first ? (float)cnt / wsum : 0.0f;
-				}
-				wave_lds_fence();
-			}
-			raw = rwmd_fill_rows<LT>(S, sm, rb, lenc, maxlen, lane, a, p.qmass[v]);
-		}
-		else if constexpr (MODE == 2) raw = wrd_bound_rows<LT>(S, rb, lenc, maxlen, v, a, p.mag, p.tok_id + (len > 0 ? t_a : 0), p.qmass[v]);
-		else raw = wrd_bound_rows<LT>(S, rb, lenc, maxlen, v, a, p.mag + (len > 0 ? t_a : 0), nullptr, p.qmass[v]);
-		return raw;
-		};
-		float raw = 0.0f;
-		if constexpr (MODE == 2 && (GAP == 4 || GAP == 7)) {
-			if (turns > 1) {
-				for (int turn = 0; turn < 4; turn++) {
-					const bool mine = sigma == turn;
-					if (mine && rewrite) static_vocab_fixup<16>(S + rowbase * LT, LT, len, p.len_t, p.tok_id + t_a, p.tag_s + t_a, p.pos_s + t_a, p.table, 0,
-						p.qid_bits, p.qkey, p.tw, p.tpos, p.tw_keep, p.tw_threshold, v);
-					wave_lds_fence();
-					const float r = evaluate();
-					if (mine) raw = r;
-					wave_lds_fence();
-					if (mine && rewrite) static_vocab_fixup<16, false, true>(S + rowbase * LT, LT, len, p.len_t, p.tok_id + t_a, p.tag_s + t_a, p.pos_s + t_a, p.table, 0,
-						p.qid_bits, p.qkey, p.tw, p.tpos, p.tw_keep, p.tw_threshold, v);
-					wave_lds_fence();
-				}
-			} else raw = evaluate();
-		} else raw = evaluate();
-
-		if (v == 15 && s_idx < p.n_sent) {
-			float val = VK_NEG_INF, r = VK_NEG_INF;
-			if (len >= 1) {
-				const float boost = p.boost ? p.boost[s_idx] : 1.0f;
-				r = raw;
-				val = (raw / inv_ref) * boost;
-			}
-			p.scores[s_idx] = val;
-			if (p.raw) p.raw[s_idx] = r;
-		}
-		wave_lds_fence();
-	}
-	}
+	constexpr int FULL_LQ = 0;
+#include "vk_score_body.hip.inc"
 }
 
 template <typename K>
-static hipError_t launch_sized(K kernel, const VkScoreParams &p, int want_blocks, size_t smem, hipStream_t stream) {
+static hipError_t launch_sized(K kernel, const VkScoreParams &p, int want_blocks, size_t smem, hipStream_t stream, int residency = 0) {
 	int occ = 0;
 	const int threads = p.group_list ? 64 : 256;
 	hipError_t e;
@@ -288,6 +35,7 @@
 	const int stream_cap = ((p.bound_bits == 0 && p.nk32 >= 5 && p.nk32 <= 7) || p.bound_bits == 6) ? 4 : 3;
 	if (occ > stream_cap && !dp_bound && !bound_pass) occ = stream_cap;
 	if (p.nk32 == 24 && p.tail == 0 && p.prec == 0 && p.layout != VK_DEV_LAYOUT_STATIC && !bound_pass) occ = 1;
+	if (residency > 0) occ = residency < real_occ ? residency : real_occ;
 	const char *ov = getenv("VK_BLOCKS_PER_CU");
 	if (ov && atoi(ov) > 0) occ = atoi(ov) < real_occ ? atoi(ov) : real_occ;
 	int dev = 0, cus = 256;
diff --git a/vectorian_amd/csrc/vk_score_body.hip.inc b/vectorian_amd/csrc/vk_score_body.hip.inc
--- /dev/null
+++ b/vectorian_amd/csrc/vk_score_body.hip.inc
@@ -0,0 +1,260 @@
+	static_assert(FULL_LQ == 0 || (GAP == 8 && FULL_LQ <= LT), "the straight-line DP is a form of GAP 8");
+	extern __shared__ float4 vk_smem4[];
+	float *smem = reinterpret_cast<float *>(vk_smem4);
+	const int lane = threadIdx.x & 63, wv = threadIdx.x >> 6;
+	const int nwaves = blockDim.x >> 6;
+	const uint8_t *qlds = reinterpret_cast<const uint8_t *>(smem);
+	if constexpr (MODE == 3 || MODE == 4) {
+		for (int i = threadIdx.x; i < NK32 * 64; i += blockDim.x)
+			vk_smem4[i] = *reinterpret_cast<const float4 *>(p.qtile + i * 16);
+		__syncthreads();
+		smem += NK32 * 256;
+	}
+	if constexpr (MODE == 7) {
+		for (int i = threadIdx.x; i < NK32 * 64 + 12; i += blockDim.x)
+			vk_smem4[i] = *reinterpret_cast<const float4 *>(p.qtile + i * 16);
+		__syncthreads();
+		smem += NK32 * 256 + VK_DEV_BOUND_CONST_BYTES / 4;
+	}
+	if constexpr (MODE == 8 || MODE == 9) {
+		for (int i = threadIdx.x; i < VK_DEV_FP6_QTILE_BYTES / 16 + 12; i += blockDim.x)
+			vk_smem4[i] = *reinterpret_cast<const float4 *>(p.qtile + i * 16);
+		__syncthreads();
+		smem += (VK_DEV_FP6_QTILE_BYTES + VK_DEV_BOUND_CONST_BYTES) / 4;
+	}
+	if constexpr (MODE == 1 || MODE == 5 || MODE == 6) {
+		if (p.q_lds > 0) {
+			for (int i = threadIdx.x; i * 16 < p.q_lds; i += blockDim.x)
+				vk_smem4[i] = i * 16 < p.tile_bytes ? *reinterpret_cast<const float4 *>(p.qtile + i * 16) : float4{0.0f, 0.0f, 0.0f, 0.0f};
+			__syncthreads();
+			smem += p.q_lds / 4;
+		}
+	}
+	float *S = smem + wv * p.lds_floats_per_wave;
+	float *Hh = S + p.s_rows_per_wave * LT + 16;
+	const int sigma = lane >> 4, v = lane & 15;
+
+	QFrag<NK32, TAIL> qf;
+	if constexpr (MODE == 0) load_qfrag<NK32, TAIL>(qf, p.qtile, lane);
+
+	DpArgs a;
+	a.locality = p.locality; a.len_t = p.len_t;
+	a.gs = p.gs; a.gt = p.gt; a.a_s = p.a_s; a.a_t = p.a_t; a.open_s = p.open_s; a.open_t = p.open_t;
+	a.ws = p.ws; a.wt = p.wt; a.wt0 = p.wt0;
+	a.rwmd_symmetric = p.rwmd_symmetric; a.rwmd_normalize_bow = p.rwmd_normalize_bow; a.wmd_bound = p.wmd_bound;
+	a.wrd_raw_total = p.wrd_raw_total;
+	const float inv_ref = p.ref_total;
+	constexpr bool TAGS = MODE != 7 && MODE != 8 && MODE != 9;
+	float twl[4] = {1.0f, 1.0f, 1.0f, 1.0f};
+	int tposl[4] = {0, 0, 0, 0};
+	if (TAGS && p.pos_s) {
+		const int cbase = (MODE == 2) ? (lane & 3) * 4 : (lane >> 4) * 4;
+#pragma unroll
+		for (int r = 0; r < 4; r++) { twl[r] = p.tw[cbase + r]; tposl[r] = p.tpos[cbase + r]; }
+	}
+
+	constexpr bool FLAT = GAP == 8 || GAP == 9;
+	static_assert(!FLAT || MODE == 7 || MODE == 8 || MODE == 9, "a flat-tailed table gives a bound, not a score");
+	constexpr int WSN = FLAT ? VK_BOUND_TAIL_K + 2 : GAP == 6 ? 65 : 33;
+	float wsr[WSN], wtr[LT];
+	if (GAP == 3 || GAP == 6 || FLAT) {
+#pragma unroll
+		for (int k = 0; k < (FLAT ? WSN - 1 : WSN); k++) wsr[k] = p.ws[k];
+		if (FLAT) wsr[WSN - 1] = p.bound_tail_cost;
+#pragma unroll
+		for (int k = 0; k < LT; k++) wtr[k] = p.wt[k];
+	}
+
+	const int n_groups = p.group_list ? p.n_list : (p.n_sent + 3) >> 2;
+	const int run = p.group_list ? 1 : VK_RUN;
+	const int n_runs = (n_groups + run - 1) / run;
+	for (int ri = blockIdx.x * nwaves + wv; ri < n_runs; ri += gridDim.x * nwaves) {
+	int prev_tile = -1, prev_row = 0;
+	for (int gg = 0; gg < run; gg++) {
+		const int gi = ri * run + gg;
+		if (gi >= n_groups) break;
+		const int grp = p.group_list ? p.group_list[gi] : gi;
+		const int s_idx = grp * 4 + sigma;
+		const int i0 = s_idx < p.n_sent ? s_idx : p.n_sent;
+		const int t_a = p.sent_start[i0], t_b = p.sent_end[i0];
+		const int len = t_b - t_a;
+		const int g_a = __builtin_amdgcn_readlane(t_a, 0);
+		const int g_b = __builtin_amdgcn_readlane(t_b, 48);
+		int maxlen = __builtin_amdgcn_readlane(len, 0);
+		maxlen = max(maxlen, __builtin_amdgcn_readlane(len, 16));
+		maxlen = max(maxlen, __builtin_amdgcn_readlane(len, 32));
+		maxlen = max(maxlen, __builtin_amdgcn_readlane(len, 48));
+		if (!p.group_list && maxlen > p.max_short_len) { prev_tile = -1; continue; }
+
+		int rowbase;
+		if (MODE == 2) {
+			const int ntok = g_b - g_a;
+			for (int it0 = 0; it0 * 16 < ntok; it0 += 4) {
+				int id[4];
+				float4 val[4];
+#pragma unroll
+				for (int q4 = 0; q4 < 4; q4++) {
+					const int tk = (it0 + q4) * 16 + (lane >> 2);
+					id[q4] = p.tok_id[g_a + (tk < ntok ? tk : 0)];
+				}
+#pragma unroll
+				for (int q4 = 0; q4 < 4; q4++)
+					val[q4] = *reinterpret_cast<const float4 *>(p.table + (int64_t)id[q4] * 16 + (lane & 3) * 4);
+#pragma unroll
+				for (int q4 = 0; q4 < 4; q4++) {
+					const int tk = (it0 + q4) * 16 + (lane >> 2);
+					if (tk < ntok) {
+						float4 vq = val[q4];
+						if (p.pos_s) {
+							const int ps = p.pos_s[g_a + tk];
+							vq.x = tag_weighted(vq.x, twl[0], ps, tposl[0], p.tw_keep, p.tw_threshold);
+							vq.y = tag_weighted(vq.y, twl[1], ps, tposl[1], p.tw_keep, p.tw_threshold);
+							vq.z = tag_weighted(vq.z, twl[2], ps, tposl[2], p.tw_keep, p.tw_threshold);
+							vq.w = tag_weighted(vq.w, twl[3], ps, tposl[3], p.tw_keep, p.tw_threshold);
+						}
+						if ((lane & 3) * 4 < LT) *reinterpret_cast<float4 *>(S + tk * LT + (lane & 3) * 4) = vq;
+					}
+				}
+			}
+			rowbase = t_a - g_a;
+		} else {
+			const int tile0 = g_a >> 4;
+			const int ntiles = ((g_b + 15) >> 4) - tile0;
+			const uint8_t *tp = p.tiles + (int64_t)tile0 * p.tile_bytes;
+			int ti0 = 0;
+			if (ntiles > 0 && tile0 == prev_tile) {
+				if (prev_row != 0) {
+					float4 keep = {0.0f, 0.0f, 0.0f, 0.0f};
+					if (lane < 4 * LT) keep = reinterpret_cast<const float4 *>(S)[prev_row * 4 * LT + lane];
+					wave_lds_fence();
+					if (lane < 4 * LT) reinterpret_cast<float4 *>(S)[lane] = keep;
+				}
+				ti0 = 1;
+				tp += p.tile_bytes;
+			}
+			if (ntiles > 0) { prev_tile = tile0 + ntiles - 1; prev_row = ntiles - 1; }
+			if constexpr (MODE == 8 || MODE == 9) {
+				constexpr int T = GAP == 6 ? 1 : GAP == 8 ? VK_FP6_TILES_TAIL : GAP == 9 ? VK_FP6_TILES_TAIL64 : VK_FP6_TILES;
+				const auto tiles = [&](auto tc, int ti) {
+					constexpr int N = decltype(tc)::value;
+					f32x4 ub[N];
+					sim_tiles_fp6<N, MODE == 9>(ub, qlds, tp, p.tile_bytes, lane, p.bound_live);
+#pragma unroll
+					for (int i = 0; i < N; i++)
+						if ((lane >> 4) * 4 < LT) *reinterpret_cast<f32x4 *>(S + ((ti + i) * 16 + (lane & 15)) * LT + (lane >> 4) * 4) = ub[i];
+					tp += (int64_t)N * p.tile_bytes;
+				};
+				int ti = ti0;
+				for (; ti + T <= ntiles; ti += T) tiles(std::integral_constant<int, T>{}, ti);
+				if constexpr (T > 1)
+					for (; ti < ntiles; ti++) tiles(std::integral_constant<int, 1>{}, ti);
+			} else
+			for (int ti = ti0; ti < ntiles; ti++) {
+				f32x4 acc;
+				if constexpr (MODE == 0) acc = sim_tile<NK32, TAIL>(qf, tp, lane);
+				else if constexpr (MODE == 3) acc = sim_tile_qlds<NK32, TAIL>(qlds, tp, lane);
+				else if constexpr (MODE == 4) acc = sim_tile_f32_qlds<NK32>(qlds, tp, lane);
+				else if constexpr (MODE == 7) acc = sim_tile_i8<NK32>(qlds, tp, lane, p.bound_live);
+				else {
+					constexpr bool DEEP = MODE == 5 || MODE == 6;
+					constexpr int PREC = MODE == 6 ? 1 : 0;
+					if (p.q_lds > 0) acc = sim_tile_generic<DEEP, PREC>(qlds, tp, p.nk32, p.tail, lane);
+					else acc = sim_tile_generic<DEEP, PREC>(p.qtile, tp, p.nk32, p.tail, lane);
+				}
+				if (TAGS && p.pos_s) {
+					const int ps = p.pos_s[(tile0 + ti) * 16 + (lane & 15)];
+#pragma unroll
+					for (int r = 0; r < 4; r++) acc[r] = tag_weighted(acc[r], twl[r], ps, tposl[r], p.tw_keep, p.tw_threshold);
+				}
+				if ((lane >> 4) * 4 < LT) *reinterpret_cast<f32x4 *>(S + (ti * 16 + (lane & 15)) * LT + (lane >> 4) * 4) = acc;
+				tp += p.tile_bytes;
+			}
+			rowbase = t_a - tile0 * 16;
+		}
+		wave_lds_fence();
+		int turns = 1;
+		bool rewrite = false;
+		if constexpr (MODE == 2 && (GAP == 4 || GAP == 7)) {
+			if (p.qid_bits) {
+				rewrite = len > 0 && static_vocab_shared(len, p.len_t, p.tok_id + t_a, p.tag_s + t_a, p.qid_bits, p.qkey) != 0;
+				if (p.slices_overlap && __builtin_amdgcn_ballot_w64(rewrite) != 0) turns = 4;
+				else if (rewrite) static_vocab_fixup<16>(S + rowbase * LT, LT, len, p.len_t, p.tok_id + t_a, p.tag_s + t_a, p.pos_s + t_a, p.table, 0,
+					p.qid_bits, p.qkey, p.tw, p.tpos, p.tw_keep, p.tw_threshold, v);
+				wave_lds_fence();
+			}
+		}
+
+		const int lenc = len > 0 ? len : 0;
+		const int rb = len > 0 ? rowbase : 0;
+		auto evaluate = [&]() -> float {
+		float raw;
+		if constexpr (GAP == 0) raw = dp_linear<LT>(S, rb, lenc, maxlen, v, a);
+		else if constexpr (GAP == 1) raw = dp_affine<LT>(S, rb, lenc, maxlen, v, a);
+		else if constexpr (GAP == 2) raw = dp_general<LT>(S, Hh, p.h_rows, rb, lenc, maxlen, lane, a);
+		else if constexpr (GAP == 3) raw = dp_general_reg<LT, 32>(S, rb, lenc, maxlen, v, a, wsr, wtr);
+		else if constexpr (GAP == 6) raw = dp_general_reg<LT, 64, MODE != 7>(S, rb, lenc, maxlen, v, a, wsr, wtr);
+		else if constexpr (GAP == 8 && FULL_LQ > 0) {
+			if (maxlen == 32 && __builtin_amdgcn_ballot_w64(len != 32) == 0) raw = dp_tail_local_full<LT, FULL_LQ, VK_BOUND_TAIL_K>(S, rowbase, v, a, wsr, wtr);
+			else raw = dp_general_tail_reg<LT, 32, VK_BOUND_TAIL_K, true, VK_DEV_LOCAL, FULL_LQ>(S, rb, lenc, maxlen, v, a, wsr, wtr);
+		}
+		else if constexpr (GAP == 8) raw = dp_general_tail_reg<LT, 32, VK_BOUND_TAIL_K>(S, rb, lenc, maxlen, v, a, wsr, wtr);
+		else if constexpr (GAP == 9) raw = dp_general_tail_reg<LT, 64, VK_BOUND_TAIL_K, MODE != 7>(S, rb, lenc, maxlen, v, a, wsr, wtr);
+		else if constexpr (GAP == 4) {
+			if (a.wmd_bound == 1) raw = wrd_bound_rows<LT>(S, rb, lenc, maxlen, v, a, nullptr, nullptr, 1.0f / (float)a.len_t);
+			else raw = rwmd_rows<LT>(S, rb, lenc, maxlen, v, a);
+		}
+		else if constexpr (GAP == 7) {
+			float *sm = nullptr;
+			if (MODE == 2) {
+				sm = Hh + sigma * p.m_rows;
+				const float wsum = p.rwmd_normalize_bow ? (float)(lenc > 0 ? lenc : 1) : 1.0f;
+				for (int u = v; u < lenc; u += 16) {
+					const int id = p.tok_id[t_a + u];
+					int cnt = 0;
+					bool first = true;
+					for (int i = 0; i < lenc; i++) {
+						const bool same = p.tok_id[t_a + i] == id && (!p.tag_s || p.tag_s[t_a + i] == p.tag_s[t_a + u]);
+						cnt += same ? 1 : 0;
+						first = first && !(same && i < u);
+					}
+					sm[u] = first ? (float)cnt / wsum : 0.0f;
+				}
+				wave_lds_fence();
+			}
+			raw = rwmd_fill_rows<LT>(S, sm, rb, lenc, maxlen, lane, a, p.qmass[v]);
+		}
+		else if constexpr (MODE == 2) raw = wrd_bound_rows<LT>(S, rb, lenc, maxlen, v, a, p.mag, p.tok_id + (len > 0 ? t_a : 0), p.qmass[v]);
+		else raw = wrd_bound_rows<LT>(S, rb, lenc, maxlen, v, a, p.mag + (len > 0 ? t_a : 0), nullptr, p.qmass[v]);
+		return raw;
+		};
+		float raw = 0.0f;
+		if constexpr (MODE == 2 && (GAP == 4 || GAP == 7)) {
+			if (turns > 1) {
+				for (int turn = 0; turn < 4; turn++) {
+					const bool mine = sigma == turn;
+					if (mine && rewrite) static_vocab_fixup<16>(S + rowbase * LT, LT, len, p.len_t, p.tok_id + t_a, p.tag_s + t_a, p.pos_s + t_a, p.table, 0,
+						p.qid_bits, p.qkey, p.tw, p.tpos, p.tw_keep, p.tw_threshold, v);
+					wave_lds_fence();
+					const float r = evaluate();
+					if (mine) raw = r;
+					wave_lds_fence();
+					if (mine && rewrite) static_vocab_fixup<16, false, true>(S + rowbase * LT, LT, len, p.len_t, p.tok_id + t_a, p.tag_s + t_a, p.pos_s + t_a, p.table, 0,
+						p.qid_bits, p.qkey, p.tw, p.tpos, p.tw_keep, p.tw_threshold, v);
+					wave_lds_fence();
+				}
+			} else raw = evaluate();
+		} else raw = evaluate();
+
+		if (v == 15 && s_idx < p.n_sent) {
+			float val = VK_NEG_INF, r = VK_NEG_INF;
+			if (len >= 1) {
+				const float boost = p.boost ? p.boost[s_idx] : 1.0f;
+				r = raw;
+				val = (raw / inv_ref) * boost;
+			}
+			p.scores[s_idx] = val;
+			if (p.raw) p.raw[s_idx] = r;
+		}
+		wave_lds_fence();
+	}
+	}
diff --git a/vectorian_amd/csrc/vk_score_m9f.hip b/vectorian_amd/csrc/vk_score_m9f.hip
--- /dev/null
+++ b/vectorian_amd/csrc/vk_score_m9f.hip
@@ -0,0 +1,29 @@
+#define VK_SCORE_VGPRS 104
+#include <cstring>
+#include "vk_score.hip.h"
+
+template <int LT, int LQ>
+__global__ __launch_bounds__(256) VK_SCORE_KERNEL_ATTR void vk_score_local_kernel(VkScoreParams p) {
+	static_assert(LT == (LQ + 3) / 4 * 4, "the strip is as wide as vk_score_kernel's for a query of LQ tokens");
+	constexpr int MODE = 9, NK32 = VK_DEV_FP6_STEPS, GAP = 8, FULL_LQ = LQ;
+	constexpr bool TAIL = false;
+#include "vk_score_body.hip.inc"
+}
+
+extern "C" int32_t vk_score_m9f_takes(const VkScoreParams *p) {
+	if (p->gap_mode != 8 || p->locality != VK_DEV_LOCAL || p->len_t < 1 || p->len_t > 16) return 0;
+	const char *dp = getenv("VK_BOUND_DP");
+	return dp && strcmp(dp, "generic") == 0 ? 0 : 1;
+}
+
+#define VK_M9F_BLOCKS_PER_CU 3
+extern "C" hipError_t vk_launch_score_m9f(const VkScoreParams *p, int32_t grid, size_t smem_bytes, hipStream_t stream) {
+	if (!vk_score_m9f_takes(p)) return hipErrorInvalidValue;
+	switch (p->len_t) {
+#define VK_M9F_CASE(LQ) case LQ: return launch_sized(vk_score_local_kernel<(LQ + 3) / 4 * 4, LQ>, *p, grid, smem_bytes, stream, VK_M9F_BLOCKS_PER_CU);
+	VK_M9F_CASE(1) VK_M9F_CASE(2) VK_M9F_CASE(3) VK_M9F_CASE(4) VK_M9F_CASE(5) VK_M9F_CASE(6) VK_M9F_CASE(7) VK_M9F_CASE(8)
+	VK_M9F_CASE(9) VK_M9F_CASE(10) VK_M9F_CASE(11) VK_M9F_CASE(12) VK_M9F_CASE(13) VK_M9F_CASE(14) VK_M9F_CASE(15) VK_M9F_CASE(16)
+#undef VK_M9F_CASE
+	default: return hipErrorInvalidValue;
+	}
+}
diff --git a/vectorian_amd/csrc/vk_score_m9t.hip b/vectorian_amd/csrc/vk_score_m9t.hip
--- a/vectorian_amd/csrc/vk_score_m9t.hip
+++ b/vectorian_amd/csrc/vk_score_m9t.hip
@@ -2,6 +2,7 @@
 #include "vk_score.hip.h"
 
 extern "C" hipError_t vk_launch_score_m9t(const VkScoreParams *p, int32_t grid, size_t smem_bytes, hipStream_t stream) {
+	if (vk_score_m9f_takes(p)) return vk_launch_score_m9f(p, grid, smem_bytes, stream);
 	switch (p->gap_mode) {
 	case 8: return launch_score_lt<9, VK_DEV_FP6_STEPS, false, 8>(*p, grid, smem_bytes, stream);
 	case 9: return launch_score_lt<9, VK_DEV_FP6_STEPS, false, 9>(*p, grid, smem_bytes, stream);
```

New measurement: 886.5 million, median of 6. +5.5%, better.
